# zsyOAOA/ResShift

Measured on NVIDIA B200. Metric: 256x256 x4 SR images/sec (15 steps), denoising hot path, higher is better.
Workload: dtype f16 (fp32 accumulate)

## Files before the change

### include/resshift_b200.h

```cpp
#ifndef RESSHIFT_B200_H
#define RESSHIFT_B200_H

#include <stddef.h>
#include <stdint.h>

#ifdef __cplusplus
extern "C" {
#endif

#define RS_MAX_LEVELS 8

typedef struct rs_unet_config {
  int32_t image_size;
  int32_t in_channels;
  int32_t model_channels;
  int32_t out_channels;
  int32_t n_levels;
  int32_t channel_mult[RS_MAX_LEVELS];
  int32_t num_res_blocks[RS_MAX_LEVELS];
  int32_t n_attn;
  int32_t attention_resolutions[RS_MAX_LEVELS];
  int32_t swin_depth;
  int32_t swin_embed_dim;
  int32_t swin_heads;
  int32_t window_size;
  float mlp_ratio;
  int32_t cond_mask;
  int32_t lq_size;
} rs_unet_config;

typedef struct rs_vq_config {
  int32_t embed_dim;
  int32_t n_embed;
  int32_t z_channels;
  int32_t in_channels;
  int32_t out_ch;
  int32_t ch;
  int32_t n_levels;
  int32_t ch_mult[RS_MAX_LEVELS];
  int32_t num_res_blocks[RS_MAX_LEVELS];
} rs_vq_config;

typedef struct rs_engine rs_engine;
typedef struct rs_plan rs_plan;
typedef struct rs_sampler rs_sampler;

int rs_version(void);
const char* rs_last_error(void);

int rs_unet_create(const rs_unet_config* cfg, rs_engine** out);
void rs_unet_destroy(rs_engine* e);
int rs_unet_param_count(const rs_engine* e);
int rs_unet_param_info(const rs_engine* e, int index, char* name, size_t name_cap, int32_t shape[4],
                       int32_t* ndim, int32_t* is_buffer);
size_t rs_unet_arena_bytes(const rs_engine* e);
int rs_unet_set_arena(rs_engine* e, void* arena_dev);
int rs_unet_load_param(rs_engine* e, const char* name, const float* src_dev, void* stream);

int rs_plan_create(rs_engine* e, int batch, int height, int width, rs_plan** out);
void rs_plan_destroy(rs_plan* p);
size_t rs_plan_workspace_bytes(const rs_plan* p);
int rs_plan_bind(rs_plan* p, void* workspace_dev);
int rs_plan_num_launches(const rs_plan* p);
int rs_plan_forward(rs_plan* p, const float* x, const float* timesteps, const float* lq, const float* mask,
                    float* out, void* stream);
int rs_plan_profile(rs_plan* p, const float* x, const float* timesteps, const float* lq, const float* mask,
                    double* ms_by_kind, double* conv_flops, int32_t* n_conv_launches, void* stream);
int rs_plan_profile_ops(rs_plan* p, const float* x, const float* timesteps, const float* lq, const float* mask,
                        double* ms, char* desc, int desc_stride, int cap, int32_t* n_ops, void* stream);
int rs_plan_probe(rs_plan* p, const char* block, float* dst, int32_t* channels, int32_t* h, int32_t* w,
                  void* stream);

int rs_sampler_create(rs_plan* p, int steps, const double* sqrt_etas_host, double kappa,
                      const int32_t* timestep_map_host, rs_sampler** out);
void rs_sampler_destroy(rs_sampler* s);
int rs_sampler_run(rs_sampler* s, const float* z_y, const float* noises, const float* lq, const float* mask,
                   float* out_latent, int use_graph, void* stream);
int rs_sampler_run_host(rs_sampler* s, const float* z_y_host, const float* noises_host, const float* lq_host,
                        const float* mask_host, float* out_latent_host, void* staging_dev, size_t staging_bytes,
                        int use_graph, void* stream);
size_t rs_sampler_staging_bytes(const rs_sampler* s);
int rs_sampler_set_taps(rs_sampler* s, float* pred_xstart_steps, float* sample_steps);

int rs_vq_create(const rs_vq_config* cfg, rs_engine** out);
int rs_vq_plan_create(rs_engine* e, int batch, int image_h, int image_w, int which, rs_plan** out);
int rs_vq_encode(rs_plan* p, const float* x, float* h_out, void* stream);
int rs_vq_decode(rs_plan* p, const float* h, float* out, int32_t* idx_out, int force_not_quantize, void* stream);
int rs_vq_profile_ops(rs_plan* p, double* ms, char* desc, int desc_stride, int cap, int32_t* n_ops, void* stream);

int rs_op_bicubic_upsample(const float* x, int N, int C, int H, int W, int sf, float* y, void* stream);
int rs_op_ingest_u8(const void* src_u8_nhwc, int N, int H, int W, int C, float* dst_nchw, void* stream);
int rs_op_emit_u8(const float* sr_nchw, const float* lq_nchw_or_null, const float* mask_or_null, int N, int H, int W,
                  int bgr, void* dst_u8_nhwc, void* stream);
int rs_op_tile_gather(const float* tiles, int N, int C, int H, int W, int th, int tw, int nty, int ntx, const int32_t* ys,
                      const int32_t* xs, float* out, void* stream);

int rs_p_sample(const float* x_t, const float* x0_pred, const float* noise, float* x_next, float coef1,
                float coef2, float std, int t_is_zero, long long numel, void* stream);

int rs_op_pack_conv_weight(const float* src_oihw, void* dst_f16, int O, int I, int KH, int KW, int Ipad, void* stream);
int rs_op_conv2d(const void* x, int N, int H, int W, int C, int ld, const void* w_packed, int Ipad, const float* bias,
                 int Cout, int ksize, int stride, const void* residual, int res_ld, void* out, int out_ld,
                 float* out_f32_nchw, int act, int bn, void* stream);
int rs_op_conv2d_stats(const void* x, int N, int H, int W, int C, int ld, const void* w_packed, int Ipad, const float* bias,
                       int Cout, int ksize, int stride, const void* residual, int res_ld, void* out, int out_ld, int act,
                       int bn, float* part, int cstride, int coff, int32_t* slots_out, float* gstat, void* counter,
                       int expected_channels, void* stream);
int rs_op_conv2d_splitk(const void* x, int N, int H, int W, int C, int ld, const void* w_packed, int Ipad, const float* bias,
                        int Cout, int ksize, int stride, const void* residual, int res_ld, void* out, int out_ld, int act,
                        float* part, int cstride, int coff, float* scratch, int32_t* splits_out, float* gstat, void* counter,
                        void* stream);
int rs_op_conv2d_timeline(const void* x, int N, int H, int W, int C, int ld, const void* w_packed, int Ipad, const float* bias,
                          int Cout, int ksize, int stride, void* out, int out_ld, int bn, int iters, void* dbg,
                          int32_t* info, float* splitk_scratch_or_null, void* stream);
int rs_op_groupnorm(const void* x, int N, int H, int W, int C, int ld, const float* gamma, const float* beta,
                    const float* film, long long film_sN, int silu, void* y, int y_ld, float* sums_scratch,
                    void* stream);
long long rs_op_groupnorm_scratch_floats(int N, int H, int W, int C);
int rs_op_groupnorm_apply(const void* x, int N, int H, int W, int C, int ld, const float* gamma, const float* beta,
                          const float* film, long long film_sN, int silu, void* y, int y_ld, const float* gstat,
                          void* stream);
int rs_op_groupnorm_apply_pairs(const void* x, int N, int H, int W, int C, int ld, const float* gamma, const float* beta,
                                const float* film, long long film_sN, int silu, void* y, int y_ld, const float* part,
                                int slots, void* stream);
int rs_op_groupnorm_finalize(const float* part, int N, int slots, int C, int rows_per_slot, float eps, float* gstat, void* stream);
int rs_op_expand_relpos(const float* table_225xh, float* dense_hx64x64, int heads, void* stream);
int rs_op_window_attention(const void* qkv, int N, int H, int W, int heads, int shift, const float* bias_dense,
                           void* out, void* stream);
int rs_op_swin_attn(const void* x, int N, int H, int W, int E, int heads, int shift, const float* gn_part, int gn_slots,
                    const float* gamma, const float* beta, const void* wqkv_packed, const float* bqkv, const float* relbias_dense,
                    const void* wproj_packed, const float* bproj, void* y, float* part_out, float* gstat_out_or_null,
                    uint32_t* counters_or_null, void* stream);
int rs_op_mlp(const void* x, int N, int H, int W, int E, int Hd, const void* w1_packed, const float* b1,
              const void* w2_packed, const float* b2, const void* residual, void* out, void* dbg_timeline_or_null,
              void* stream);
int rs_debug_tile_config(int m_tiles, int cout, int num_kblocks, int32_t* out);
int rs_debug_swin_timeline(void* dev_buf_or_null);
int rs_op_upsample2x(const void* x, int N, int H, int W, int C, void* y, void* stream);

#ifdef __cplusplus
}
#endif
#endif
```

### resshift_b200/_lib.py

```python
from __future__ import annotations

import ctypes as C
import os
from pathlib import Path

_HERE = Path(__file__).resolve().parent
LIB_PATH = Path(os.environ.get("RESSHIFT_B200_LIB", _HERE / "lib" / "librs_b200.so"))

RS_MAX_LEVELS = 8


class RsError(RuntimeError):
    pass


class UNetConfigC(C.Structure):
    _fields_ = [
        ("image_size", C.c_int32), ("in_channels", C.c_int32), ("model_channels", C.c_int32),
        ("out_channels", C.c_int32), ("n_levels", C.c_int32),
        ("channel_mult", C.c_int32 * RS_MAX_LEVELS), ("num_res_blocks", C.c_int32 * RS_MAX_LEVELS),
        ("n_attn", C.c_int32), ("attention_resolutions", C.c_int32 * RS_MAX_LEVELS),
        ("swin_depth", C.c_int32), ("swin_embed_dim", C.c_int32), ("swin_heads", C.c_int32),
        ("window_size", C.c_int32), ("mlp_ratio", C.c_float), ("cond_mask", C.c_int32), ("lq_size", C.c_int32),
    ]


class VQConfigC(C.Structure):
    _fields_ = [
        ("embed_dim", C.c_int32), ("n_embed", C.c_int32), ("z_channels", C.c_int32), ("in_channels", C.c_int32),
        ("out_ch", C.c_int32), ("ch", C.c_int32), ("n_levels", C.c_int32),
        ("ch_mult", C.c_int32 * RS_MAX_LEVELS), ("num_res_blocks", C.c_int32 * RS_MAX_LEVELS),
    ]


_P = C.c_void_p
_SIGNATURES = {
    "rs_version": (C.c_int, []),
    "rs_last_error": (C.c_char_p, []),
    "rs_unet_create": (C.c_int, [C.POINTER(UNetConfigC), C.POINTER(_P)]),
    "rs_unet_destroy": (None, [_P]),
    "rs_unet_param_count": (C.c_int, [_P]),
    "rs_unet_param_info": (C.c_int, [_P, C.c_int, C.c_char_p, C.c_size_t, C.POINTER(C.c_int32), C.POINTER(C.c_int32),
                                     C.POINTER(C.c_int32)]),
    "rs_unet_arena_bytes": (C.c_size_t, [_P]),
    "rs_unet_set_arena": (C.c_int, [_P, _P]),
    "rs_unet_load_param": (C.c_int, [_P, C.c_char_p, _P, _P]),
    "rs_plan_create": (C.c_int, [_P, C.c_int, C.c_int, C.c_int, C.POINTER(_P)]),
    "rs_plan_destroy": (None, [_P]),
    "rs_plan_workspace_bytes": (C.c_size_t, [_P]),
    "rs_plan_bind": (C.c_int, [_P, _P]),
    "rs_plan_num_launches": (C.c_int, [_P]),
    "rs_plan_forward": (C.c_int, [_P, _P, _P, _P, _P, _P, _P]),
    "rs_plan_profile": (C.c_int, [_P, _P, _P, _P, _P, C.POINTER(C.c_double), C.POINTER(C.c_double), C.POINTER(C.c_int32), _P]),
    "rs_plan_profile_ops": (C.c_int, [_P, _P, _P, _P, _P, C.POINTER(C.c_double), C.c_char_p, C.c_int, C.c_int, C.POINTER(C.c_int32), _P]),
    "rs_plan_probe": (C.c_int, [_P, C.c_char_p, _P, C.POINTER(C.c_int32), C.POINTER(C.c_int32), C.POINTER(C.c_int32), _P]),
    "rs_sampler_create": (C.c_int, [_P, C.c_int, C.POINTER(C.c_double), C.c_double, C.POINTER(C.c_int32), C.POINTER(_P)]),
    "rs_sampler_destroy": (None, [_P]),
    "rs_sampler_run": (C.c_int, [_P, _P, _P, _P, _P, _P, C.c_int, _P]),
    "rs_sampler_run_host": (C.c_int, [_P, _P, _P, _P, _P, _P, _P, C.c_size_t, C.c_int, _P]),
    "rs_sampler_staging_bytes": (C.c_size_t, [_P]),
    "rs_sampler_set_taps": (C.c_int, [_P, _P, _P]),
    "rs_p_sample": (C.c_int, [_P, _P, _P, _P, C.c_float, C.c_float, C.c_float, C.c_int, C.c_longlong, _P]),
    "rs_op_pack_conv_weight": (C.c_int, [_P, _P, C.c_int, C.c_int, C.c_int, C.c_int, C.c_int, _P]),
    "rs_op_conv2d": (C.c_int, [_P, C.c_int, C.c_int, C.c_int, C.c_int, C.c_int, _P, C.c_int, _P, C.c_int, C.c_int,
                               C.c_int, _P, C.c_int, _P, C.c_int, _P, C.c_int, C.c_int, _P]),
    "rs_op_conv2d_stats": (C.c_int, [_P, C.c_int, C.c_int, C.c_int, C.c_int, C.c_int, _P, C.c_int, _P, C.c_int, C.c_int,
                                     C.c_int, _P, C.c_int, _P, C.c_int, C.c_int, C.c_int, _P, C.c_int, C.c_int,
                                     C.POINTER(C.c_int32), _P, _P, C.c_int, _P]),
    "rs_op_conv2d_splitk": (C.c_int, [_P, C.c_int, C.c_int, C.c_int, C.c_int, C.c_int, _P, C.c_int, _P, C.c_int, C.c_int,
                                      C.c_int, _P, C.c_int, _P, C.c_int, C.c_int, _P, C.c_int, C.c_int, _P,
                                      C.POINTER(C.c_int32), _P, _P, _P]),
    "rs_op_conv2d_timeline": (C.c_int, [_P, C.c_int, C.c_int, C.c_int, C.c_int, C.c_int, _P, C.c_int, _P, C.c_int, C.c_int,
                                        C.c_int, _P, C.c_int, C.c_int, C.c_int, _P, C.POINTER(C.c_int32), _P, _P]),
    "rs_op_groupnorm": (C.c_int, [_P, C.c_int, C.c_int, C.c_int, C.c_int, C.c_int, _P, _P, _P, C.c_longlong, C.c_int,
                                  _P, C.c_int, _P, _P]),
    "rs_op_groupnorm_scratch_floats": (C.c_longlong, [C.c_int, C.c_int, C.c_int, C.c_int]),
    "rs_op_groupnorm_apply": (C.c_int, [_P, C.c_int, C.c_int, C.c_int, C.c_int, C.c_int, _P, _P, _P, C.c_longlong, C.c_int,
                                        _P, C.c_int, _P, _P]),
    "rs_op_groupnorm_finalize": (C.c_int, [_P, C.c_int, C.c_int, C.c_int, C.c_int, C.c_float, _P, _P]),
    "rs_op_groupnorm_apply_pairs": (C.c_int, [_P, C.c_int, C.c_int, C.c_int, C.c_int, C.c_int, _P, _P, _P, C.c_longlong,
                                              C.c_int, _P, C.c_int, _P, C.c_int, _P]),
    "rs_op_expand_relpos": (C.c_int, [_P, _P, C.c_int, _P]),
    "rs_op_window_attention": (C.c_int, [_P, C.c_int, C.c_int, C.c_int, C.c_int, C.c_int, _P, _P, _P]),
    "rs_op_swin_attn": (C.c_int, [_P, C.c_int, C.c_int, C.c_int, C.c_int, C.c_int, C.c_int, _P, C.c_int, _P, _P, _P, _P, _P, _P, _P,
                                  _P, _P, _P, _P, _P]),
    "rs_op_mlp": (C.c_int, [_P, C.c_int, C.c_int, C.c_int, C.c_int, C.c_int, _P, _P, _P, _P, _P, _P, _P, _P]),
    "rs_debug_tile_config": (C.c_int, [C.c_int, C.c_int, C.c_int, C.POINTER(C.c_int32)]),
    "rs_debug_swin_timeline": (C.c_int, [_P]),
    "rs_op_upsample2x": (C.c_int, [_P, C.c_int, C.c_int, C.c_int, C.c_int, _P, _P]),
    "rs_vq_create": (C.c_int, [C.POINTER(VQConfigC), C.POINTER(_P)]),
    "rs_vq_plan_create": (C.c_int, [_P, C.c_int, C.c_int, C.c_int, C.c_int, C.POINTER(_P)]),
    "rs_vq_encode": (C.c_int, [_P, _P, _P, _P]),
    "rs_vq_decode": (C.c_int, [_P, _P, _P, _P, C.c_int, _P]),
    "rs_vq_profile_ops": (C.c_int, [_P, C.POINTER(C.c_double), C.c_char_p, C.c_int, C.c_int, C.POINTER(C.c_int32), _P]),
    "rs_op_bicubic_upsample": (C.c_int, [_P, C.c_int, C.c_int, C.c_int, C.c_int, C.c_int, _P, _P]),
    "rs_op_ingest_u8": (C.c_int, [_P, C.c_int, C.c_int, C.c_int, C.c_int, _P, _P]),
    "rs_op_emit_u8": (C.c_int, [_P, _P, _P, C.c_int, C.c_int, C.c_int, C.c_int, _P, _P]),
    "rs_op_tile_gather": (C.c_int, [_P, C.c_int, C.c_int, C.c_int, C.c_int, C.c_int, C.c_int, C.c_int, C.c_int, _P, _P, _P, _P]),
}


def _load():
    if not LIB_PATH.exists():
        raise ImportError(
            f"resshift_b200: CUDA library {LIB_PATH} not found. Build it with "
            f"`python -c 'import __graft_entry__ as g; g.build()'` (nvcc, sm_100a). There is no CPU fallback.")
    lib = C.CDLL(str(LIB_PATH))
    for name, (res, args) in _SIGNATURES.items():
        fn = getattr(lib, name)
        fn.restype = res
        fn.argtypes = args
    return lib


lib = _load()


def check(rc: int) -> None:
    if rc != 0:
        msg = lib.rs_last_error()
        raise RsError(f"librs_b200 error {rc}: {msg.decode(errors='replace') if msg else '?'}")


def declared_symbols():
    return sorted(_SIGNATURES)


def ptr(t) -> int:
    return None if t is None else t.data_ptr()


def current_stream() -> int:
    import torch
    return torch.cuda.current_stream().cuda_stream


def make_config(cfg) -> UNetConfigC:
    c = UNetConfigC()
    c.image_size, c.in_channels, c.model_channels, c.out_channels = cfg.image_size, cfg.in_channels, cfg.model_channels, cfg.out_channels
    c.n_levels = len(cfg.channel_mult)
    for i, v in enumerate(cfg.channel_mult):
        c.channel_mult[i] = int(v)
    for i, v in enumerate(cfg.num_res_blocks):
        c.num_res_blocks[i] = int(v)
    c.n_attn = len(cfg.attention_resolutions)
    for i, v in enumerate(cfg.attention_resolutions):
        c.attention_resolutions[i] = int(v)
    c.swin_depth, c.swin_embed_dim, c.swin_heads = cfg.swin_depth, cfg.swin_embed_dim, cfg.swin_heads
    c.window_size, c.mlp_ratio = cfg.window_size, float(cfg.mlp_ratio)
    c.cond_mask, c.lq_size = int(cfg.cond_mask), cfg.lq_size
    return c


def make_vq_config(cfg) -> VQConfigC:
    c = VQConfigC()
    c.embed_dim, c.n_embed, c.z_channels = cfg.embed_dim, cfg.n_embed, cfg.z_channels
    c.in_channels, c.out_ch, c.ch = cfg.in_channels, cfg.out_ch, cfg.ch
    c.n_levels = len(cfg.ch_mult)
    for i, v in enumerate(cfg.ch_mult):
        c.ch_mult[i] = int(v)
    for i, v in enumerate(cfg.num_res_blocks):
        c.num_res_blocks[i] = int(v)
    return c
```

### resshift_b200/csrc/conv_gemm.cuh

```cuda
#pragma once

#include "common.cuh"
#include "gn_stats.cuh"

namespace rs {

constexpr int kConvBM = 128;
constexpr int kConvBK = 64;
constexpr int kConvEpiWarps = 8;
constexpr int kConvThreads = 64 + 32 * kConvEpiWarps;
constexpr int kConvTmaWarp = kConvEpiWarps;
constexpr int kConvMmaWarp = kConvEpiWarps + 1;
constexpr int kMaxTaps = 9;
constexpr int kMaxSrc = 4;

enum ConvAct : int { ACT_NONE = 0, ACT_GELU = 1, ACT_SILU = 2 };

struct ConvParams {
  CUtensorMap tmA[kMaxSrc];
  CUtensorMap tmB;
  int num_taps;
  int tap_src[kMaxTaps];
  int tap_dh[kMaxTaps];
  int tap_dw[kMaxTaps];
  int kchunks;
  int tail_k16;
  int w_tap_stride;
  int bw, bh, bn;
  int tiles_w, tiles_h, tiles_n;
  int Wout, Hout, Nimg;
  int BN, n_tiles, Cout;
  int stages;
  int tmem_cols;
  int cg;
  int splitk;
  float* partial;
  int splitk_cluster;
  int msub;
  const float* bias;
  const __half* residual;
  long long res_sN, res_sH, res_sW;
  __half* out;
  long long out_sN, out_sH, out_sW;
  float* out_f32_nchw;
  int act;
  unsigned long long* dbg;
  CUtensorMap tmOut, tmRes;
  int tma_out;
  int tma_res;
  int epi_bc;
  GnSink sink[2];
  int gn_slots;
  int persist;
  int num_units;
};

#ifdef __CUDACC__

template <int kCG>
__global__ void __launch_bounds__(kConvThreads, 2) conv_gemm_sm100_kernel(const __grid_constant__ ConvParams p) {
  extern __shared__ __align__(1024) uint8_t smem_raw[];
  uint8_t* smem = reinterpret_cast<uint8_t*>((reinterpret_cast<uintptr_t>(smem_raw) + 1023) & ~uintptr_t(1023));
  const int a_bytes = kConvBM * kConvBK * 2;
  const int b_rows = kCG == 2 ? p.BN / 2 : p.BN;
  const int b_bytes = b_rows * kConvBK * 2;
  const int stage_bytes = p.msub * a_bytes + b_bytes;
  uint64_t* full_bar = reinterpret_cast<uint64_t*>(smem + (size_t)p.stages * stage_bytes);
  uint64_t* empty_bar = full_bar + p.stages;
  uint64_t* tmem_full_bar = empty_bar + p.stages;
  uint64_t* res_bar = tmem_full_bar + 1;
  uint32_t* tmem_slot = reinterpret_cast<uint32_t*>(res_bar + 1);
  float* s_bias = reinterpret_cast<float*>(smem + (size_t)p.stages * stage_bytes + 256);

  const int warp = threadIdx.x >> 5;
  const int lane = threadIdx.x & 31;
  unsigned long long* dbg = p.dbg ? p.dbg + (size_t)blockIdx.x * 8 : nullptr;
  if (dbg && threadIdx.x == 0) {
    uint32_t smid;
    asm volatile("mov.u32 %0, %%smid;" : "=r"(smid));
    dbg[0] = global_timer_ns(); dbg[7] = smid;
  }

  const uint32_t crank = kCG == 2 ? cluster_ctarank() : 0;
  const uint32_t rank = crank & 1;
  const uint32_t lead = crank & ~1u;
  const uint16_t pair_mask = (uint16_t)(3u << lead);
  int unit = kCG == 2 ? (blockIdx.x >> 1) : blockIdx.x;
  const int split = unit % p.splitk;
  unit /= p.splitk;
  const int n_tile = unit % p.n_tiles;
  const int mt0 = kCG == 2 ? (unit / p.n_tiles) * 2 + (int)rank : (unit / p.n_tiles) * p.msub;
  const int total_kb = p.num_taps * p.kchunks;
  const int kb_begin = (int)((long long)total_kb * split / p.splitk);
  const int kb_end = (int)((long long)total_kb * (split + 1) / p.splitk);
  const int num_kb = kb_end - kb_begin;
  auto tile_origin = [&](int sub, int& tw_, int& th_, int& w0_, int& h0_, int& n0_) {
    int mt = mt0 + sub;
    tw_ = mt % p.tiles_w; mt /= p.tiles_w;
    th_ = mt % p.tiles_h; mt /= p.tiles_h;
    w0_ = tw_ * p.bw; h0_ = th_ * p.bh; n0_ = mt * p.bn;
  };

  if (warp == kConvTmaWarp && lane == 0) {
    for (int s = 0; s < kMaxSrc; ++s) tma_prefetch_desc(&p.tmA[s]);
    tma_prefetch_desc(&p.tmB);
    if (p.tma_out) tma_prefetch_desc(&p.tmOut);
    if (p.tma_res) tma_prefetch_desc(&p.tmRes);
    for (int s = 0; s < p.stages; ++s) {
      mbar_init(&full_bar[s], 1);
      mbar_init(&empty_bar[s], 1);
    }
    mbar_init(tmem_full_bar, 1);
    mbar_init(res_bar, 1);
    mbar_fence_init();
  }
  if (warp == kConvMmaWarp) {
    if constexpr (kCG == 2) { tmem_alloc_dyn_cg2(tmem_slot, (uint32_t)p.tmem_cols); tmem_relinquish_cg2(); }
    else { tmem_alloc_dyn(tmem_slot, (uint32_t)p.tmem_cols); tmem_relinquish(); }
  }
  tc_fence_before();
  if constexpr (kCG == 2) cluster_sync_all(); else __syncthreads();
  tc_fence_after();
  const uint32_t tmem_base = *tmem_slot;
  pdl_trigger();
  pdl_wait();
  if (dbg && threadIdx.x == 0) dbg[1] = global_timer_ns();

  if (warp == kConvTmaWarp) {
    const bool el = elect_one();
    int stage = 0;
    uint32_t phase = 0;
    int tws[2], ths[2], w0s[2], h0s[2], n0s[2];
    for (int sub = 0; sub < p.msub; ++sub) tile_origin(sub, tws[sub], ths[sub], w0s[sub], h0s[sub], n0s[sub]);
    int tap = kb_begin / p.kchunks;
    int kc = kb_begin - tap * p.kchunks;
    const uint32_t tx_bytes = (uint32_t)(kCG == 2 ? 2 * stage_bytes : stage_bytes);
    for (int kb = 0; kb < num_kb; ++kb) {
      mbar_wait(&empty_bar[stage], phase ^ 1);
      uint8_t* sa = smem + (size_t)stage * stage_bytes;
      uint8_t* sb = sa + p.msub * a_bytes;
      const CUtensorMap* ma = &p.tmA[p.tap_src[tap]];
      const int dw = p.tap_dw[tap], dh = p.tap_dh[tap];
      const int kcol = kc * kConvBK, wcol = tap * p.w_tap_stride + kc * kConvBK;
      if constexpr (kCG == 2) {
        const uint32_t lead_bar = mapa_u32(smem_u32(&full_bar[stage]), lead);
        if (el) {
          if (rank == 0) mbar_arrive_expect_tx(&full_bar[stage], tx_bytes);
          tma_load_4d_cg2(sa, ma, lead_bar, kcol, w0s[0] + dw, h0s[0] + dh, n0s[0]);
          tma_load_2d_cg2(sb, &p.tmB, lead_bar, wcol, n_tile * p.BN + (int)rank * b_rows);
        }
      } else {
        if (el) {
          mbar_arrive_expect_tx(&full_bar[stage], tx_bytes);
          for (int sub = 0; sub < p.msub; ++sub)
            tma_load_4d(sa + sub * a_bytes, ma, &full_bar[stage], kcol, w0s[sub] + dw, h0s[sub] + dh, n0s[sub]);
          tma_load_2d(sb, &p.tmB, &full_bar[stage], wcol, n_tile * p.BN);
        }
      }
      if (++kc == p.kchunks) { kc = 0; ++tap; }
      if (++stage == p.stages) { stage = 0; phase ^= 1; }
    }
  } else if (warp == kConvMmaWarp && rank == 0) {
    const bool el = elect_one();
    const uint32_t idesc = umma_idesc_f16(kCG == 2 ? 2 * kConvBM : kConvBM, p.BN);
    const uint32_t smem0 = smem_u32(smem);
    const uint32_t b_off = (uint32_t)(p.msub * a_bytes);
    int stage = 0;
    uint32_t phase = 0;
    int kc = kb_begin % p.kchunks;
    for (int kb = 0; kb < num_kb; ++kb) {
      mbar_wait(&full_bar[stage], phase);
      tc_fence_after();
      if (dbg && el && kb == 0) dbg[2] = global_timer_ns();
      const uint32_t sa = smem0 + (uint32_t)stage * (uint32_t)stage_bytes;
      const uint64_t adesc = umma_desc_sw128(sa);
      const uint64_t bdesc = umma_desc_sw128(sa + b_off);
      const uint32_t acc0 = kb != 0 ? 1u : 0u;
      const int ksteps = (kc == p.kchunks - 1) ? p.tail_k16 : kConvBK / 16;
      if (++kc == p.kchunks) kc = 0;
      if constexpr (kCG == 2) {
        if (el) {
          umma_f16_cg2(tmem_base, adesc, bdesc, idesc, acc0);
#pragma unroll
          for (int k = 1; k < kConvBK / 16; ++k) if (k < ksteps) umma_f16_cg2(tmem_base, adesc + 2 * k, bdesc + 2 * k, idesc, 1u);
          umma_commit_cg2(&empty_bar[stage], pair_mask);
          if (kb == num_kb - 1) umma_commit_cg2(tmem_full_bar, pair_mask);
        }
      } else {
        if (el) {
          umma_f16(tmem_base, adesc, bdesc, idesc, acc0);
#pragma unroll
          for (int k = 1; k < kConvBK / 16; ++k) if (k < ksteps) umma_f16(tmem_base, adesc + 2 * k, bdesc + 2 * k, idesc, 1u);
          if (p.msub == 2) {
            const uint64_t adesc1 = umma_desc_sw128(sa + a_bytes);
            umma_f16(tmem_base + p.BN, adesc1, bdesc, idesc, acc0);
#pragma unroll
            for (int k = 1; k < kConvBK / 16; ++k) if (k < ksteps) umma_f16(tmem_base + p.BN, adesc1 + 2 * k, bdesc + 2 * k, idesc, 1u);
          }
          umma_commit(&empty_bar[stage]);
          if (kb == num_kb - 1) umma_commit(tmem_full_bar);
        }
      }
      if (++stage == p.stages) { stage = 0; phase ^= 1; }
    }
    if (dbg && el) dbg[3] = global_timer_ns();
// ... 64 lines not shown
          for (int sub = 0; sub < p.msub; ++sub) {
            int tw, th, w0, h0, n0;
            tile_origin(sub, tw, th, w0, h0, n0);
            for (int b = 0; b < nblk; ++b)
              tma_load_4d(smem + (size_t)sub * sub_bytes + (size_t)b * blk_bytes, &p.tmRes, res_bar, col0 + b * bc, w0, h0, n0);
          }
        }
        mbar_wait(res_bar, 0);
      }
      const bool want_stats = p.sink[0].part != nullptr;
      for (int sub = 0; sub < p.msub; ++sub) {
        int tw, th, w0, h0, n0;
        tile_origin(sub, tw, th, w0, h0, n0);
        const uint32_t trow = tmem_base + (static_cast<uint32_t>(quad * 32) << 16) + sub * p.BN;
        uint8_t* sblk = smem + (size_t)sub * sub_bytes;
        uint32_t vn[16];
        if (cpar * 16 < p.BN) tmem_ld16(trow + cpar * 16, vn);
        for (int c = cpar * 16; c < p.BN; c += 32) {
          tmem_ld_wait16(vn);
          float f[16];
#pragma unroll
          for (int j = 0; j < 16; ++j) f[j] = __uint_as_float(vn[j]);
          if (c + 32 < p.BN) tmem_ld16(trow + c + 32, vn);
          {
            const float4* bp = reinterpret_cast<const float4*>(s_bias + c);
#pragma unroll
            for (int j = 0; j < 4; ++j) {
              const float4 b4 = bp[j];
              f[4 * j] += b4.x; f[4 * j + 1] += b4.y; f[4 * j + 2] += b4.z; f[4 * j + 3] += b4.w;
            }
          }
          if (p.act == ACT_GELU) {
#pragma unroll
            for (int j = 0; j < 16; ++j) f[j] = gelu_erf_f(f[j]);
          } else if (p.act == ACT_SILU) {
#pragma unroll
            for (int j = 0; j < 16; ++j) f[j] = silu_f(f[j]);
          }
          uint8_t* brow = sblk + (size_t)(c >> bshift) * blk_bytes + r * (2 * bc);
          const int u0 = (c & (bc - 1)) >> 3;
          uint4* a0 = reinterpret_cast<uint4*>(brow + (((u0) ^ swz) << 4));
          uint4* a1 = reinterpret_cast<uint4*>(brow + (((u0 + 1) ^ swz) << 4));
          if (p.tma_res) {
            const uint4 r0 = *a0, r1 = *a1;
            const __half2* h0p = reinterpret_cast<const __half2*>(&r0);
            const __half2* h1p = reinterpret_cast<const __half2*>(&r1);
#pragma unroll
            for (int j = 0; j < 4; ++j) {
              const float2 x0 = __half22float2(h0p[j]);
              const float2 x1 = __half22float2(h1p[j]);
              f[2 * j] += x0.x; f[2 * j + 1] += x0.y;
              f[8 + 2 * j] += x1.x; f[8 + 2 * j + 1] += x1.y;
            }
          }
          uint4 o0, o1;
          __half2* q0 = reinterpret_cast<__half2*>(&o0);
          __half2* q1 = reinterpret_cast<__half2*>(&o1);
#pragma unroll
          for (int j = 0; j < 4; ++j) {
            q0[j] = __floats2half2_rn(f[2 * j], f[2 * j + 1]);
            q1[j] = __floats2half2_rn(f[8 + 2 * j], f[8 + 2 * j + 1]);
          }
          *a0 = o0; *a1 = o1;
          if (want_stats) warp_chunk_stats(o0, o1, lane, wsum_all + ((size_t)(sub * 4 + quad) * p.BN + c) * 2);
        }
      }
      fence_proxy_async_smem();
      named_bar_sync(1, 32 * kConvEpiWarps);
      if (dbg && etid == 0) dbg[6] = global_timer_ns();
      if (etid == 0) {
        for (int sub = 0; sub < p.msub; ++sub) {
          int tw, th, w0, h0, n0;
          tile_origin(sub, tw, th, w0, h0, n0);
          for (int b = 0; b < nblk; ++b)
            if (col0 + b * bc < p.Cout)
              tma_store_4d(&p.tmOut, smem + (size_t)sub * sub_bytes + (size_t)b * blk_bytes, col0 + b * bc, w0, h0, n0);
        }
        tma_store_commit();
      }
      if (want_stats) {
        int* s_flag = reinterpret_cast<int*>(wsum_all + (size_t)p.msub * 8 * p.BN);
        for (int sub = 0; sub < p.msub; ++sub) {
          int tw, th, w0, h0, n0;
          tile_origin(sub, tw, th, w0, h0, n0);
          const int ncols = min(p.BN, p.Cout - col0);
          const int slot = th * p.tiles_w + tw;
          if (n0 < p.Nimg)
            write_quad_pairs(wsum_all + (size_t)sub * 8 * p.BN, p.BN, ncols, col0, p.bn, n0, p.Nimg, slot, p.gn_slots, p.sink[0], p.sink[1],
                             etid, 32 * kConvEpiWarps);
          if (p.sink[0].gstat || p.sink[1].gstat) {
            const GnSink* const sk[4] = {&p.sink[0], &p.sink[0], p.sink[1].part ? &p.sink[1] : nullptr, p.sink[1].part ? &p.sink[1] : nullptr};
            const int n1 = (p.bn == 2 && n0 + 1 < p.Nimg) ? n0 + 1 : -1;
            const int im[4] = {n0 < p.Nimg ? n0 : -1, n0 < p.Nimg ? n1 : -1, n0 < p.Nimg ? n0 : -1, n0 < p.Nimg ? n1 : -1};
            const unsigned int ad[4] = {(unsigned)ncols, (unsigned)ncols, (unsigned)ncols, (unsigned)ncols};
            gn_arrive<4>(sk, im, ad, p.gn_slots, 128.0f / (float)p.bn, etid, 32 * kConvEpiWarps, 1, s_flag);
          }
        }
      }
      if (etid == 0) tma_store_wait_read();
    } else {
      for (int sub = 0; sub < p.msub; ++sub) {
        int tw, th, w0, h0, n0;
        tile_origin(sub, tw, th, w0, h0, n0);
        const int w = w0 + lw, h = h0 + lh, n = n0 + ln;
        const bool row_ok = (w < p.Wout) && (h < p.Hout) && (n < p.Nimg);
        const uint32_t trow = tmem_base + (static_cast<uint32_t>(quad * 32) << 16) + sub * p.BN;
        __half* orow = p.out ? p.out + n * p.out_sN + h * p.out_sH + w * p.out_sW : nullptr;
        const __half* rrow = p.residual ? p.residual + n * p.res_sN + h * p.res_sH + w * p.res_sW : nullptr;
        for (int c = cpar * 16; c < p.BN; c += 32) {
          uint32_t v[16];
          __syncwarp();
          tmem_ld16(trow + c, v);
          tmem_ld_wait();
          const int col = col0 + c;
          if (!row_ok || col >= p.Cout) continue;
          float f[16];
#pragma unroll
          for (int j = 0; j < 16; ++j) f[j] = __uint_as_float(v[j]);
          if (p.bias) {
#pragma unroll
            for (int j = 0; j < 16; ++j)
              if (col + j < p.Cout) f[j] += __ldg(p.bias + col + j);
          }
          if (p.act == ACT_GELU) {
#pragma unroll
            for (int j = 0; j < 16; ++j) f[j] = gelu_erf_f(f[j]);
          } else if (p.act == ACT_SILU) {
#pragma unroll
            for (int j = 0; j < 16; ++j) f[j] = silu_f(f[j]);
          }
          if (rrow)
            for (int j = 0; j < 16 && col + j < p.Cout; ++j) f[j] += __half2float(rrow[col + j]);
          if (p.out_f32_nchw)
            for (int j = 0; j < 16 && col + j < p.Cout; ++j)
              p.out_f32_nchw[(((long long)n * p.Cout + (col + j)) * p.Hout + h) * p.Wout + w] = f[j];
          if (orow)
            for (int j = 0; j < 16 && col + j < p.Cout; ++j) orow[col + j] = __float2half_rn(f[j]);
        }
      }
    }
  }

  if constexpr (kCG == 2) {
    if (p.splitk > 1 && p.splitk_cluster) {
      cluster_sync_all();
      if (warp < kConvEpiWarps) {
        const int etid = threadIdx.x;
        const int S = p.splitk, cw = p.BN / S, upr = cw >> 3;
        const int pitch = p.BN * 4 + 16;
        const int cbase = split * cw;
        const int col0 = n_tile * p.BN;
        __half* s_out = reinterpret_cast<__half*>(smem + (size_t)kConvBM * pitch);
        float* s_col = reinterpret_cast<float*>(s_out + (size_t)kConvBM * cw);
        int tw, th, w0, h0, n0;
        tile_origin(0, tw, th, w0, h0, n0);
        const uint32_t dump0 = smem_u32(smem);
        for (int u = etid; u < kConvBM * upr; u += 32 * kConvEpiWarps) {
          const int rr = u / upr, cu = u - rr * upr;
          const int ct = cbase + cu * 8;
          float acc[8];
#pragma unroll
          for (int j = 0; j < 8; ++j) acc[j] = 0.f;
          for (int sp = 0; sp < S; ++sp) {
            const uint32_t a = mapa_u32(dump0 + (uint32_t)(rr * pitch + ct * 4), (uint32_t)(sp * 2) + rank);
            const float4 x0 = ld_shared_cluster_f4(a), x1 = ld_shared_cluster_f4(a + 16);
            acc[0] += x0.x; acc[1] += x0.y; acc[2] += x0.z; acc[3] += x0.w;
            acc[4] += x1.x; acc[5] += x1.y; acc[6] += x1.z; acc[7] += x1.w;
          }
          const int lw = rr % p.bw, lh = (rr / p.bw) % p.bh, ln = rr / (p.bw * p.bh);
          const int w = w0 + lw, h = h0 + lh, n = n0 + ln;
          const int col = col0 + ct;
          const bool ok = (w < p.Wout) && (h < p.Hout) && (n < p.Nimg) && (col < p.Cout);
          uint4 o = make_uint4(0, 0, 0, 0);
          if (ok) {
            if (p.bias) {
#pragma unroll
              for (int j = 0; j < 8; ++j) acc[j] += __ldg(p.bias + col + j);
            }
            if (p.act == ACT_GELU) {
#pragma unroll
              for (int j = 0; j < 8; ++j) acc[j] = gelu_erf_f(acc[j]);
            } else if (p.act == ACT_SILU) {
#pragma unroll
              for (int j = 0; j < 8; ++j) acc[j] = silu_f(acc[j]);
            }
            if (p.residual) {
              const uint4 rv = *reinterpret_cast<const uint4*>(p.residual + n * p.res_sN + h * p.res_sH + w * p.res_sW + col);
              const __half2* rh = reinterpret_cast<const __half2*>(&rv);
#pragma unroll
              for (int j = 0; j < 4; ++j) { const float2 f = __half22float2(rh[j]); acc[2 * j] += f.x; acc[2 * j + 1] += f.y; }
            }
            __half2* oh = reinterpret_cast<__half2*>(&o);
#pragma unroll
            for (int j = 0; j < 4; ++j) oh[j] = __floats2half2_rn(acc[2 * j], acc[2 * j + 1]);
            *reinterpret_cast<uint4*>(p.out + n * p.out_sN + h * p.out_sH + w * p.out_sW + col) = o;
          }
          *reinterpret_cast<uint4*>(s_out + (size_t)rr * cw + cu * 8) = o;
        }
        if (p.sink[0].part != nullptr) {
          named_bar_sync(1, 32 * kConvEpiWarps);
          for (int t = etid; t < 2 * cw; t += 32 * kConvEpiWarps) {
            const int half = t / cw, c = t - half * cw;
            const __half* col = s_out + (size_t)(half * 64) * cw + c;
            const float pv = __half2float(col[0]);
            float s1 = 0.f, s2 = 0.f;
            for (int rr = 1; rr < 64; ++rr) {
              const float d = __half2float(col[(size_t)rr * cw]) - pv;
              s1 += d; s2 = fmaf(d, d, s2);
            }
            s_col[(half * cw + c) * 2] = pv + s1 * (1.0f / 64.0f);
            s_col[(half * cw + c) * 2 + 1] = fmaxf(s2 - s1 * s1 * (1.0f / 64.0f), 0.f);
          }
          named_bar_sync(1, 32 * kConvEpiWarps);
          const int slot = th * p.tiles_w + tw;
          const int ncols = max(0, min(cw, p.Cout - (col0 + cbase)));
          if (n0 < p.Nimg)
            write_tile_pairs(s_col, cw, ncols, col0 + cbase, p.bn, n0, p.Nimg, slot, p.gn_slots, p.sink[0], p.sink[1], etid, 32 * kConvEpiWarps);
          if (p.sink[0].gstat || p.sink[1].gstat) {
            int* s_flag = reinterpret_cast<int*>(s_col + 4 * cw);
            const GnSink* const sk[4] = {&p.sink[0], &p.sink[0], p.sink[1].part ? &p.sink[1] : nullptr, p.sink[1].part ? &p.sink[1] : nullptr};
            const int n1 = (p.bn == 2 && n0 + 1 < p.Nimg) ? n0 + 1 : -1;
            const int im[4] = {n0 < p.Nimg ? n0 : -1, n0 < p.Nimg ? n1 : -1, n0 < p.Nimg ? n0 : -1, n0 < p.Nimg ? n1 : -1};
            const unsigned int ad[4] = {(unsigned)ncols, (unsigned)ncols, (unsigned)ncols, (unsigned)ncols};
            gn_arrive<4>(sk, im, ad, p.gn_slots, 128.0f / (float)p.bn, etid, 32 * kConvEpiWarps, 1, s_flag);
          }
        }
      }
    }
  }

  tc_fence_before();
  if constexpr (kCG == 2) cluster_sync_all(); else __syncthreads();
  if (dbg && threadIdx.x == 0) dbg[5] = global_timer_ns();
  if (warp == kConvMmaWarp) {
    tc_fence_after();
    if constexpr (kCG == 2) tmem_dealloc_dyn_cg2(tmem_base, (uint32_t)p.tmem_cols);
    else tmem_dealloc_dyn(tmem_base, (uint32_t)p.tmem_cols);
  }
}

struct ConvSimtSrc {
  const __half* ptr[kMaxSrc];
  long long sN[kMaxSrc], sH[kMaxSrc], sW[kMaxSrc];
  int H[kMaxSrc], W[kMaxSrc];
  int C;
  const __half* wt;
};

__global__ void conv_simt_kernel(const __grid_constant__ ConvParams p, const __grid_constant__ ConvSimtSrc s) {
  pdl_trigger();
  pdl_wait();
  const long long pix = (long long)blockIdx.x * (blockDim.x >> 5) + (threadIdx.x >> 5);
  const int lane = threadIdx.x & 31;
  const long long npix = (long long)p.Nimg * p.Hout * p.Wout;
  if (pix >= npix) return;
  const int w = (int)(pix % p.Wout);
  const int h = (int)((pix / p.Wout) % p.Hout);
  const int n = (int)(pix / ((long long)p.Wout * p.Hout));
  const int ktot = p.num_taps * p.w_tap_stride;
  for (int co = lane; co < p.Cout; co += 32) {
    float acc = 0.f;
    for (int t = 0; t < p.num_taps; ++t) {
      const int src = p.tap_src[t];
      const int hh = h + p.tap_dh[t], ww = w + p.tap_dw[t];
      if (hh < 0 || ww < 0 || hh >= s.H[src] || ww >= s.W[src]) continue;
      const __half* a = s.ptr[src] + n * s.sN[src] + hh * s.sH[src] + ww * s.sW[src];
      const __half* wr = s.wt + (long long)co * ktot + t * p.w_tap_stride;
      for (int c = 0; c < s.C; c += 2) {
        const float2 av = __half22float2(*reinterpret_cast<const __half2*>(a + c));
        const float2 wv = __half22float2(*reinterpret_cast<const __half2*>(wr + c));
        acc = fmaf(av.x, wv.x, acc);
        acc = fmaf(av.y, wv.y, acc);
      }
    }
    if (p.bias) acc += p.bias[co];
    if (p.act == ACT_GELU) acc = gelu_erf_f(acc);
    else if (p.act == ACT_SILU) acc = silu_f(acc);
    if (p.residual) acc += __half2float(p.residual[n * p.res_sN + h * p.res_sH + w * p.res_sW + co]);
    if (p.out_f32_nchw) p.out_f32_nchw[(((long long)n * p.Cout + co) * p.Hout + h) * p.Wout + w] = acc;
    if (p.out) p.out[n * p.out_sN + h * p.out_sH + w * p.out_sW + co] = __float2half_rn(acc);
  }
}

#endif

}
```

### resshift_b200/csrc/engine.cu

```cuda
#include <map>
#include <memory>
#include <string>
#include <vector>

#include "../../include/resshift_b200.h"
#include "launch.cuh"
#include "vq_kernels.cuh"

namespace rs {

static thread_local std::string g_last_error;
void set_error(const std::string& msg) { g_last_error = msg; }
int fail(int code, const std::string& msg) { g_last_error = msg; return code; }

static inline size_t align_up(size_t v, size_t a) { return (v + a - 1) / a * a; }

enum Role { R_CONV3 = 0, R_CONV1, R_LINEAR, R_BIAS, R_GN_W, R_GN_B, R_RELPOS, R_BUF_RELIDX, R_BUF_MASK, R_F32  };

struct Param {
  std::string name;
  std::vector<int> shape;
  int role;
  size_t off = 0;
  size_t bytes = 0;
// ... 113 lines not shown
      add_conv(e, p, L.a, L.b, 3);
    } else if (L.kind == 1) {
      add_gn(e, p + ".in_layers.0", L.a);
      add_conv(e, p + ".in_layers.2", L.a, L.b, 3);
      add_linear(e, p + ".emb_layers.1", e.time_dim(), 2 * L.b);
      add_gn(e, p + ".out_layers.0", L.b);
      add_conv(e, p + ".out_layers.3", L.b, L.b, 3);
      if (L.a != L.b) add_conv(e, p + ".skip_connection", L.a, L.b, 1);
    } else if (L.kind == 2) {
      const int E = c.swin_embed_dim, res = L.b;
      const int win = res <= c.window_size ? res : c.window_size;
      const int shift = res <= c.window_size ? 0 : c.window_size / 2;
      const int hidden = (int)(E * c.mlp_ratio);
      add_conv(e, p + ".patch_embed.proj", L.a, E, 1);
      add_conv(e, p + ".patch_unembed.proj", E, L.a, 1);
      for (int i = 0; i < c.swin_depth; ++i) {
        const std::string b = p + ".blocks." + std::to_string(i);
        if (i % 2 == 1 && shift > 0) {
          const int nw = (res / win) * (res / win);
          add_param(e, b + ".attn_mask", {nw, win * win, win * win}, R_BUF_MASK);
        }
        add_gn(e, b + ".norm1", E);
        add_param(e, b + ".attn.relative_position_bias_table", {(2 * win - 1) * (2 * win - 1), c.swin_heads}, R_RELPOS);
        add_param(e, b + ".attn.relative_position_index", {win * win, win * win}, R_BUF_RELIDX);
        add_linear(e, b + ".attn.qkv", E, 3 * E);
        add_linear(e, b + ".attn.proj", E, E);
        add_gn(e, b + ".norm2", E);
        add_conv(e, b + ".mlp.fc1", E, hidden, 1);
        add_conv(e, b + ".mlp.fc2", hidden, E, 1);
      }
    } else if (L.kind == 3) {
      add_conv(e, p + ".op", L.a, L.a, 3);
    } else if (L.kind == 4) {
      add_conv(e, p + ".conv", L.a, L.a, 3);
    }
  }
}

int build_inventory(rs_engine& e) {
  const rs_unet_config& c = e.cfg;
  add_linear(e, "time_embed.0", c.model_channels, e.time_dim());
  add_linear(e, "time_embed.2", e.time_dim(), e.time_dim());
  int fc = e.lq_in_ch(), bc = 16;
  for (int st = 0; st < e.fe_stages(); ++st) {
    add_conv(e, "feature_extractor." + std::to_string(3 * st), fc, bc, 3);
    add_conv(e, "feature_extractor." + std::to_string(3 * st + 2) + ".op", bc, 2 * bc, 3);
    bc *= 2; fc = bc;
  }
  Topology t = build_topology(e);
  for (size_t i = 0; i < t.input_blocks.size(); ++i) add_layers(e, "input_blocks." + std::to_string(i), t.input_blocks[i]);
  add_layers(e, "middle_block", t.middle);
  for (size_t i = 0; i < t.output_blocks.size(); ++i) add_layers(e, "output_blocks." + std::to_string(i), t.output_blocks[i]);
  add_gn(e, "out.0", c.channel_mult[0] * c.model_channels);
  add_conv(e, "out.2", c.channel_mult[0] * c.model_channels, c.out_channels, 3);

  size_t off = 0;
  const int K = e.time_dim();
  e.film_w_off = off;
  int rows = 0;
  for (Param& p : e.params) {
    if (p.role == R_LINEAR && p.name.find(".emb_layers.1.weight") != std::string::npos) {
      p.ipad = K; p.off = off; p.bytes = (size_t)p.shape[0] * K * 2;
      e.film_row_of[p.name.substr(0, p.name.size() - std::string(".emb_layers.1.weight").size())] = rows;
      rows += p.shape[0];
      off += p.bytes;
    }
  }
  e.film_rows = rows;
  off = align_up(off, 256);
  e.film_b_off = off;
  for (Param& p : e.params) {
    if (p.role == R_BIAS && p.name.find(".emb_layers.1.bias") != std::string::npos) {
      p.off = off; p.bytes = (size_t)p.shape[0] * 4; off += p.bytes;
    }
  }
  off = align_up(off, 256);
  for (Param& p : e.params) {
    if (p.bytes) continue;
    switch (p.role) {
      case R_CONV3: case R_CONV1:
        p.ipad = (p.shape[1] + 7) / 8 * 8;
        p.bytes = (size_t)p.shape[0] * p.shape[2] * p.shape[3] * p.ipad * 2; break;
      case R_LINEAR:
        p.ipad = (p.shape[1] + 7) / 8 * 8;
        p.bytes = (size_t)p.shape[0] * p.ipad * 2; break;
      case R_BIAS: case R_GN_W: case R_GN_B:
        p.bytes = (size_t)p.shape[0] * 4; break;
      case R_RELPOS:
        p.bytes = (size_t)c.swin_heads * 64 * 64 * 4; break;
      default: p.bytes = 0; break;
    }
    if (p.bytes) { p.off = off; off = align_up(off + p.bytes, 256); }
  }
  e.arena_bytes = align_up(off, 256);
  return 0;
}

}

namespace {

enum OpKind { OP_CONV, OP_GN, OP_ATTN, OP_UPSAMPLE, OP_MLP, OP_SOFTMAX, OP_FORK, OP_JOIN, OP_SWIN_ATTN };

struct Tensor {
  size_t bytes = 0;
  int first = 1 << 30, last = -1;
  size_t off = 0;
  bool persistent = false;
};

struct Op {
  OpKind kind;
  ConvDesc conv;
  GnDesc gn;
  View a_in, a_out; const float* a_bias = nullptr; int a_shift = 0;
  View u_in, u_out;
  View s_view; float s_scale = 1.f;
  View w_view; bool w_is_view = false;
  std::string in_param;
  MlpDesc mlp;
  SwinAttnDesc swin;
  std::string blk_name;
  std::string w2_name, b2_name;
  std::string w_name, b_name, g_name;
  size_t stats_off = 0;
  int gn_index = -1;
  bool to_f32 = false;
  int split_tens = -1;
  int stream = 0;
  struct StatDst { int list; int op; int coff; int img_off; };
  std::vector<StatDst> stat_dst;
};

}

struct rs_plan {
  rs_engine* e = nullptr;
  int B = 0, H = 0, W = 0, lqH = 0, lqW = 0;
  std::vector<Tensor> tensors;
  std::vector<Op> fe_ops, ops;
  std::map<std::string, View> block_out;
  size_t off_emb_sin = 0, off_emb_mid = 0, off_emb_vec = 0, off_film = 0, off_tsteps = 0, off_tables = 0;
  size_t off_stats = 0, stats_bytes = 0, off_state = 0, off_temps = 0, temps_bytes = 0;
  size_t off_gstat = 0, off_counters = 0;
  int n_gn = 0;
  size_t workspace_bytes = 0;
  int max_rows = 0;
  uint8_t* ws = nullptr;
  View xin, lq_feat, fe_in;
  int cin_pad = 0, fe_cpad = 0;
  float* out_f32 = nullptr;
  bool bound = false;
  int launches = 0;
  int branches = 1;
  std::vector<cudaStream_t> side;
  std::vector<cudaEvent_t> ev;
  std::vector<std::pair<int, int>> sections;
  ~rs_plan() {
    for (cudaStream_t s : side) cudaStreamDestroy(s);
    for (cudaEvent_t e : ev) cudaEventDestroy(e);
  }
  int vq_which = -1;
  int imgH = 0, imgW = 0;
  const void* table_owner = nullptr;
  unsigned long long table_epoch = ~0ull;

  int new_tensor(size_t bytes, bool persistent = false) {
    Tensor t; t.bytes = align_up(bytes, 256); t.persistent = persistent;
    tensors.push_back(t);
    return (int)tensors.size() - 1;
  }
  View make_view(int N, int Hh, int Ww, int C, bool persistent = false) {
    View v; v.N = N; v.H = Hh; v.W = Ww; v.C = C; v.ld = C; v.off = 0;
    v.tens = new_tensor((size_t)N * Hh * Ww * C * 2, persistent);
    return v;
  }
  static View slice(const View& base, int c0, int C) {
    View v = base; v.off = base.off + c0; v.c0 = base.c0 + c0; v.C = C; return v;
  }
  static View batch(const View& base, int n0, int n) {
    View v = base; v.off = base.off + (long long)n0 * base.sN(); v.n0 = base.n0 + n0; v.N = n; return v;
  }
  void touch(const View& v, int opi) {
    if (v.tens < 0) return;
    Tensor& t = tensors[v.tens];
    t.first = std::min(t.first, opi); t.last = std::max(t.last, opi);
  }
};

namespace {

struct Builder {
  rs_plan& P;
  rs_engine& E;
  std::vector<Op>* cur;
  size_t stats_off = 0;
  int n_gn = 0;
  struct Writer { int c0; int C; int n0; int N; int list; int op; int win_slots; };
  std::map<int, std::vector<Writer>> writers;
  int cur_stream = 0;
  int cur_batch0 = 0;
  static bool overlaps(const Writer& w, const View& v, int C) {
    return w.c0 < v.c0 + C && v.c0 < w.c0 + w.C && w.n0 < v.n0 + v.N && v.n0 < w.n0 + w.N;
  }
  static bool inside(const Writer& w, const View& v) {
    return w.c0 >= v.c0 && w.c0 + w.C <= v.c0 + v.C && w.n0 >= v.n0 && w.n0 + w.N <= v.n0 + v.N;
  }
  void note_writer(const View& out, int C, int win_slots = 0) {
    auto& ws = writers[out.tens];
    ws.erase(std::remove_if(ws.begin(), ws.end(), [&](const Writer& w) { return overlaps(w, out, C); }), ws.end());
    ws.push_back({out.c0, C, out.n0, out.N, list_id(), (int)cur->size() - 1, win_slots});
  }
  std::vector<Writer> covering_writers(const View& in) {
    bool fusable = false;
    conv_tile_slots(in.H, in.W, &fusable);
    std::vector<Writer> prod;
    if (fuse_stats && fusable) {
      long long covered = 0;
      auto it = writers.find(in.tens);
      if (it != writers.end())
        for (const Writer& w : it->second)
          if (inside(w, in)) { prod.push_back(w); covered += (long long)w.C * w.N; }
      bool ok = covered == (long long)in.C * in.N;
      for (const Writer& w : prod) ok = ok && list(w.list)[w.op].stat_dst.size() < 2 && w.win_slots == prod[0].win_slots;
      if (!ok) prod.clear();
    }
    return prod;
  }
  const bool fuse_mlp = env_int("RS_MLP_FUSE", 1) && !env_is("RS_CONV_IMPL", "simt");
  const bool fuse_mlp_norm = env_int("RS_MLP_NORM_FUSE", 0) != 0;
  const bool fuse_swin_attn = env_int("RS_SWIN_FUSE", 1) != 0 && !env_is("RS_CONV_IMPL", "simt") && !env_is("RS_ATTN_IMPL", "simt");
  const int fuse_swin_min_pairs = env_int("RS_SWIN_FUSE_MIN_PAIRS", 96);
  const bool fuse_stats = env_int("RS_GN_FUSE", 1) && !env_is("RS_CONV_EPI", "direct") && !env_is("RS_CONV_IMPL", "simt");
  Builder(rs_plan& p) : P(p), E(*p.e), cur(&p.ops) {}
  int list_id() const { return cur == &P.fe_ops ? 0 : 1; }
  std::vector<Op>& list(int id) { return id == 0 ? P.fe_ops : P.ops; }

  int opi() const { return (int)(P.fe_ops.size() + P.ops.size()); }

  void conv(const View& in, const std::string& name, int ksize, int stride, int cout, const View* out,
            const View* res, int act, bool out_f32 = false, int pad_lo = 1) {
    Op op; op.kind = OP_CONV;
    op.conv.in = in; op.conv.ksize = ksize; op.conv.stride = stride; op.conv.Cout = cout; op.conv.act = act;
    op.conv.pad_lo = pad_lo;
    if (out) { op.conv.out = *out; op.conv.has_out = true; } else op.conv.has_out = false;
    if (res) { op.conv.res = *res; op.conv.has_res = true; }
    op.w_name = name + ".weight"; op.b_name = name + ".bias";
    op.to_f32 = out_f32;
    if (out && !out_f32 && env_int("RS_CONV_SPLITK", 0) != 1) {
      const TileConfig tc = conv_preview_config(in.N, in.H, in.W, in.C, cout, ksize, stride, true);
      if (tc.splitk > 1) op.conv.allow_split = true;
      if (tc.splitk > 1 && !tc.cluster_split) {
        const size_t bytes = (size_t)tc.splitk * in.N * (in.H / stride) * (in.W / stride) * cout * sizeof(float);
        op.split_tens = P.new_tensor(bytes);
        Tensor& tz = P.tensors[op.split_tens];
        tz.first = tz.last = opi();
      }
    }
    const int i = opi();
    P.touch(in, i); if (out) P.touch(*out, i); if (res) P.touch(*res, i);
    op.stream = cur_stream;
    cur->push_back(op);
    if (out && !out_f32 && out->tens >= 0) note_writer(*out, cout);
  }
  void gn(const View& in, const std::string& name, const View& out, int silu, int film_off, float eps = 1e-5f) {
    Op op; op.kind = OP_GN;
    op.gn.in = in; op.gn.out = out; op.gn.silu = silu; op.gn.film_off = film_off; op.gn.eps = eps;
    op.gn.film_n0 = cur_batch0;
    op.g_name = name;
    std::vector<Writer> prod = covering_writers(in);
    op.gn.win_slots = !prod.empty() && prod[0].win_slots;
    const int tile_slots = op.gn.win_slots ? (in.H / 8) * (in.W / 8) : conv_tile_slots(in.H, in.W);
    int chunks, rows;
    gn_chunks(in.H * in.W, in.N, &chunks, &rows);
    op.gn.fused = !prod.empty();
    op.gn.slots = op.gn.fused ? tile_slots : chunks;
    op.stats_off = stats_off;
    op.gn_index = n_gn++;
    stats_off += align_up((size_t)in.N * op.gn.slots * in.C * 2 * sizeof(float), 256);
    const int i = opi();
    P.touch(in, i); P.touch(out, i);
    op.stream = cur_stream;
    cur->push_back(op);
    for (const Writer& w : prod)
      list(w.list)[w.op].stat_dst.push_back({list_id(), (int)cur->size() - 1, w.c0 - in.c0, w.n0 - in.n0});
  }
  void attn(const View& qkv, const View& out, const std::string& blk, int shift) {
    Op op; op.kind = OP_ATTN; op.a_in = qkv; op.a_out = out; op.a_shift = shift;
    op.w_name = blk + ".attn.relative_position_bias_table";
    const int i = opi();
    P.touch(qkv, i); P.touch(out, i);
    op.stream = cur_stream;
    cur->push_back(op);
  }
  bool mlp(const View& in, const std::string& name, int E, int Hd, const View& out, const View& res,
           const std::string& norm_name = std::string()) {
    Op op; op.kind = OP_MLP;
    op.mlp.in = in; op.mlp.out = out; op.mlp.res = res; op.mlp.has_res = true; op.mlp.E = E; op.mlp.Hd = Hd;
    op.w_name = name + ".fc1.weight"; op.b_name = name + ".fc1.bias";
    op.w2_name = name + ".fc2.weight"; op.b2_name = name + ".fc2.bias";
    std::vector<Writer> prod;
    if (!norm_name.empty()) {
      prod = covering_writers(in);
      if (prod.empty() || Hd < 4 * E) return false;
      op.g_name = norm_name;
      op.gn.win_slots = prod[0].win_slots;
      op.gn.in = in; op.gn.fused = true; op.gn.slots = op.gn.win_slots ? (in.H / 8) * (in.W / 8) : conv_tile_slots(in.H, in.W);
      op.stats_off = stats_off;
      op.gn_index = n_gn++;
      stats_off += align_up((size_t)in.N * op.gn.slots * in.C * 2 * sizeof(float), 256);
    }
    const int i = opi();
    P.touch(in, i); P.touch(out, i); P.touch(res, i);
    op.stream = cur_stream;
    cur->push_back(op);
    for (const Writer& w : prod)
      list(w.list)[w.op].stat_dst.push_back({list_id(), (int)cur->size() - 1, w.c0 - in.c0, w.n0 - in.n0});
    if (out.tens >= 0) note_writer(out, E);
    return true;
  }
  bool swin_attn(const View& x, const std::string& blk, int heads, int shift) {
    std::vector<Writer> prod = covering_writers(x);
    if (prod.empty()) return false;
    Op op; op.kind = OP_SWIN_ATTN;
    op.swin.x = x; op.swin.y = x; op.swin.heads = heads; op.swin.shift = shift;
    op.blk_name = blk;
    op.g_name = blk + ".norm1";
    op.gn.win_slots = prod[0].win_slots;
    op.gn.in = x; op.gn.fused = true; op.gn.slots = op.gn.win_slots ? (x.H / 8) * (x.W / 8) : conv_tile_slots(x.H, x.W);
    op.stats_off = stats_off;
    op.gn_index = n_gn++;
    stats_off += align_up((size_t)x.N * op.gn.slots * x.C * 2 * sizeof(float), 256);
    const int i = opi();
    P.touch(x, i);
    op.stream = cur_stream;
    cur->push_back(op);
    for (const Writer& w : prod)
      list(w.list)[w.op].stat_dst.push_back({list_id(), (int)cur->size() - 1, w.c0 - x.c0, w.n0 - x.n0});
    if (x.tens >= 0) note_writer(x, x.C, 1);
    return true;
  }
  void upsample(const View& in, const View& out) {
    Op op; op.kind = OP_UPSAMPLE; op.u_in = in; op.u_out = out;
    const int i = opi();
    P.touch(in, i); P.touch(out, i);
    op.stream = cur_stream;
    cur->push_back(op);
  }
  void marker(OpKind k) { Op op; op.kind = k; cur->push_back(op); }

  void res_block(const View& x, const std::string& p, int cout, const View& out) {
    View t1 = P.make_view(x.N, x.H, x.W, x.C);
    gn(x, p + ".in_layers.0", t1, 1, -1);
    View h1 = P.make_view(x.N, x.H, x.W, cout);
    conv(t1, p + ".in_layers.2", 3, 1, cout, &h1, nullptr, ACT_NONE);
    View t2 = P.make_view(x.N, x.H, x.W, cout);
    gn(h1, p + ".out_layers.0", t2, 1, E.film_row_of.at(p));
    if (x.C != cout) {
      conv(x, p + ".skip_connection", 1, 1, cout, &out, nullptr, ACT_NONE);
      conv(t2, p + ".out_layers.3", 3, 1, cout, &out, &out, ACT_NONE);
    } else {
      conv(t2, p + ".out_layers.3", 3, 1, cout, &out, &x, ACT_NONE);
    }
  }
  int basic_layer(const View& x, const std::string& p, int ctor_res, const View& out) {
    const rs_unet_config& c = E.cfg;
    const int Ed = c.swin_embed_dim, hidden = (int)(Ed * c.mlp_ratio);
    const int win = ctor_res <= c.window_size ? ctor_res : c.window_size;
    RS_CHECK(win == 8 && x.H % 8 == 0 && x.W % 8 == 0, "the window-attention kernel covers 8x8 windows only");
    const int shift_odd = ctor_res <= c.window_size ? 0 : c.window_size / 2;
    View e = P.make_view(x.N, x.H, x.W, Ed);
    conv(x, p + ".patch_embed.proj", 1, 1, Ed, &e, nullptr, ACT_NONE);
    for (int i = 0; i < c.swin_depth; ++i) {
      const std::string b = p + ".blocks." + std::to_string(i);
      const int win_pairs = (x.N * (x.H / 8) * (x.W / 8) + 1) / 2;
      if (!(fuse_swin_attn && win_pairs >= fuse_swin_min_pairs && swin_attn_supported(Ed, c.swin_heads, x.H, x.W) &&
            swin_attn(e, b, c.swin_heads, (i % 2) ? shift_odd : 0))) {
        View n1 = P.make_view(x.N, x.H, x.W, Ed);
        gn(e, b + ".norm1", n1, 0, -1);
        View qkv = P.make_view(x.N, x.H, x.W, 3 * Ed);
        conv(n1, b + ".attn.qkv", 1, 1, 3 * Ed, &qkv, nullptr, ACT_NONE);
        View a = P.make_view(x.N, x.H, x.W, Ed);
        attn(qkv, a, b, (i % 2) ? shift_odd : 0);
        conv(a, b + ".attn.proj", 1, 1, Ed, &e, &e, ACT_NONE);
      }
      const bool mlp_ok = fuse_mlp && mlp_supported(Ed, hidden, x.H, x.W, x.N);
      if (mlp_ok && fuse_mlp_norm && mlp(e, b + ".mlp", Ed, hidden, e, e, b + ".norm2")) continue;
      View n2 = P.make_view(x.N, x.H, x.W, Ed);
      gn(e, b + ".norm2", n2, 0, -1);
      if (mlp_ok) {
        mlp(n2, b + ".mlp", Ed, hidden, e, e);
      } else {
        View f = P.make_view(x.N, x.H, x.W, hidden);
        conv(n2, b + ".mlp.fc1", 1, 1, hidden, &f, nullptr, ACT_GELU);
        conv(f, b + ".mlp.fc2", 1, 1, Ed, &e, &e, ACT_NONE);
      }
    }
    conv(e, p + ".patch_unembed.proj", 1, 1, x.C, &out, nullptr, ACT_NONE);
    return 0;
  }

  int run_block(View h, const std::string& prefix, const std::vector<Layer>& layers, const View& dest, View* result) {
    for (size_t j = 0; j < layers.size(); ++j) {
      const Layer& L = layers[j];
      const std::string p = prefix + "." + std::to_string(j);
      const bool last = (j + 1 == layers.size());
      View out;
      if (L.kind == 0) {
        out = last ? dest : P.make_view(h.N, h.H, h.W, L.b);
        conv(h, p, 3, 1, L.b, &out, nullptr, ACT_NONE);
      } else if (L.kind == 1) {
        out = last ? dest : P.make_view(h.N, h.H, h.W, L.b);
        res_block(h, p, L.b, out);
      } else if (L.kind == 2) {
        out = last ? dest : P.make_view(h.N, h.H, h.W, h.C);
        int rc = basic_layer(h, p, L.b, out); if (rc) return rc;
      } else if (L.kind == 3) {
        out = dest;
        conv(h, p + ".op", 3, 2, L.a, &out, nullptr, ACT_NONE);
      } else {
        View u = P.make_view(h.N, 2 * h.H, 2 * h.W, h.C);
        upsample(h, u);
        out = dest;
        conv(u, p + ".conv", 3, 1, L.a, &out, nullptr, ACT_NONE);
      }
      h = out;
    }
    *result = h;
    return 0;
  }
};

int finish_layout(rs_plan& P, Builder& b, size_t state_bytes, bool unet) {
  rs_engine& E = *P.e;
  const rs_unet_config& c = E.cfg;
  const int B = P.B;
  P.max_rows = std::max(B, 64);
  size_t off = 0;
  auto region = [&](size_t bytes) { size_t o = off; off = align_up(off + bytes, 256); return o; };
  if (unet) {
    P.off_tables = region(4 * 1024 * sizeof(float));
    P.off_tsteps = region((size_t)P.max_rows * sizeof(float));
    P.off_emb_sin = region((size_t)P.max_rows * c.model_channels * sizeof(float));
    P.off_emb_mid = region((size_t)P.max_rows * E.time_dim() * sizeof(float));
    P.off_emb_vec = region((size_t)P.max_rows * E.time_dim() * sizeof(float));
    P.off_film = region((size_t)P.max_rows * E.film_rows * sizeof(float));
  }
  P.stats_bytes = b.stats_off;
  P.off_stats = region(P.stats_bytes);
  P.n_gn = b.n_gn;
  P.off_gstat = region((size_t)P.n_gn * B * 32 * 2 * sizeof(float));
  P.off_counters = region((size_t)P.n_gn * B * sizeof(unsigned int));
  const size_t lat = state_bytes;
  P.off_state = region(2 * align_up(lat, 256));
  for (const auto& sec : P.sections)
    for (Tensor& tz : P.tensors) {
      if (tz.last < 0) continue;
      if (tz.first >= sec.first && tz.first <= sec.second) tz.first = sec.first;
      if (tz.last >= sec.first && tz.last <= sec.second) tz.last = sec.second;
    }
  if (env_int("RS_NO_REUSE", 0)) for (Tensor& tz : P.tensors) tz.persistent = true;
  for (Tensor& tz : P.tensors) if (tz.persistent) tz.off = region(tz.bytes);
  P.off_temps = off;
  {
    struct Live { size_t off, bytes; int last; };
    std::vector<Live> live;
    std::vector<int> order;
    for (int i = 0; i < (int)P.tensors.size(); ++i) if (!P.tensors[i].persistent && P.tensors[i].last >= 0) order.push_back(i);
    std::stable_sort(order.begin(), order.end(), [&](int a, int bb) { return P.tensors[a].first < P.tensors[bb].first; });
    size_t high = 0;
    for (int id : order) {
      Tensor& tz = P.tensors[id];
      live.erase(std::remove_if(live.begin(), live.end(), [&](const Live& l) { return l.last < tz.first; }), live.end());
      std::sort(live.begin(), live.end(), [](const Live& a, const Live& bb) { return a.off < bb.off; });
      size_t pos = 0;
      for (const Live& l : live) {
        if (pos + tz.bytes <= l.off) break;
        pos = std::max(pos, l.off + l.bytes);
      }
      tz.off = P.off_temps + pos;
      live.push_back({pos, tz.bytes, tz.last});
      high = std::max(high, pos + tz.bytes);
    }
    P.temps_bytes = high;
  }
  P.workspace_bytes = align_up(P.off_temps + P.temps_bytes, 256);
  return 0;
}

int build_plan(rs_plan& P) {
  rs_engine& E = *P.e;
  const rs_unet_config& c = E.cfg;
  Topology topo = build_topology(E);
  Builder b(P);
  const int B = P.B;

  const int fes = E.fe_stages();
  P.lqH = P.H << fes; P.lqW = P.W << fes;
  if (fes > 0) {
    b.cur = &P.fe_ops;
    P.fe_cpad = 8;
    P.fe_in = P.make_view(B, P.lqH, P.lqW, P.fe_cpad, true);
    View cur = P.fe_in;
    int bc = 16;
    for (int st = 0; st < fes; ++st) {
      View a = P.make_view(B, cur.H, cur.W, bc, true);
      b.conv(cur, "feature_extractor." + std::to_string(3 * st), 3, 1, bc, &a, nullptr, ACT_SILU);
      View d = P.make_view(B, cur.H / 2, cur.W / 2, 2 * bc, true);
      b.conv(a, "feature_extractor." + std::to_string(3 * st + 2) + ".op", 3, 2, 2 * bc, &d, nullptr, ACT_NONE);
      cur = d; bc *= 2;
// ... 3 lines not shown
  }

  const int cin = c.in_channels + E.lq_feat_ch();
  P.cin_pad = (cin + 7) / 8 * 8;
  P.xin = P.make_view(B, P.H, P.W, P.cin_pad, true);

  const int n_in = (int)topo.input_blocks.size();
  const int n_out = (int)topo.output_blocks.size();
  RS_CHECK(n_in == n_out, "encoder/decoder block counts differ");
  std::vector<int> in_h(n_in), in_w(n_in);
  {
    int hh = P.H, ww = P.W;
    for (int i = 0; i < n_in; ++i) {
      for (const Layer& L : topo.input_blocks[i]) if (L.kind == 3) { hh /= 2; ww /= 2; }
      in_h[i] = hh; in_w[i] = ww;
    }
  }
  std::vector<View> cat(n_out);
  for (int j = 0; j < n_out; ++j) {
    const int k = n_in - 1 - j;
    const int ctot = topo.output_blocks[j][0].a;
    cat[j] = P.make_view(B, in_h[k], in_w[k], ctot);
  }
  {
    int nb = env_int("RS_LOWRES_STREAMS", 1);
    if (nb < 1) nb = 1;
    while (nb > 1 && (B % nb != 0 || B / nb < 1)) --nb;
    P.branches = nb;
  }
  const long long low_tiles = env_int("RS_LOWRES_TILES", 64);
  auto is_low = [&](int hh, int ww) { return (long long)B * hh * ww / 128 <= low_tiles; };
  bool in_sec = false;
  int sec_first = 0;
  auto leave = [&]() {
    if (!in_sec) return;
    const int last = b.opi() - 1;
    b.marker(OP_JOIN);
    P.sections.push_back({sec_first, last});
    in_sec = false;
  };
  auto run = [&](const View& hin, const std::string& prefix, const std::vector<Layer>& layers, const View& dest, View* hout) -> int {
    bool low = P.branches > 1 && is_low(hin.H, hin.W);
    if (P.branches > 1 && !low && layers.size() == 1 && layers[0].kind == 3) low = is_low(hin.H / 2, hin.W / 2);
    if (!low) {
      leave();
      return b.run_block(hin, prefix, layers, dest, hout);
    }
    if (!in_sec) { b.marker(OP_FORK); sec_first = b.opi(); in_sec = true; }
    const int per = B / P.branches;
    for (int k = 0; k < P.branches; ++k) {
      View tmp;
      b.cur_stream = k; b.cur_batch0 = k * per;
      int rc = b.run_block(rs_plan::batch(hin, k * per, per), prefix, layers, rs_plan::batch(dest, k * per, per), &tmp);
      b.cur_stream = 0; b.cur_batch0 = 0;
      if (rc) return rc;
    }
    *hout = dest;
    return 0;
  };
  View h = P.xin;
  for (int i = 0; i < n_in; ++i) {
    const int j = n_in - 1 - i;
    const int ich = topo.in_block_ch[i];
    View dest = rs_plan::slice(cat[j], cat[j].C - ich, ich);
    View hin = h;
    int rc = run(hin, "input_blocks." + std::to_string(i), topo.input_blocks[i], dest, &h);
    if (rc) return rc;
    P.block_out["input_blocks." + std::to_string(i)] = h;
  }
  {
    View dest = rs_plan::slice(cat[0], 0, cat[0].C - topo.in_block_ch[n_in - 1]);
    int rc = run(h, "middle_block", topo.middle, dest, &h); if (rc) return rc;
    P.block_out["middle_block"] = h;
  }
  View final_h;
  for (int j = 0; j < n_out; ++j) {
    View dest;
    if (j + 1 < n_out) {
      const int ich_next = topo.in_block_ch[n_in - 2 - j];
      dest = rs_plan::slice(cat[j + 1], 0, cat[j + 1].C - ich_next);
    } else {
      const Layer& L0 = topo.output_blocks[j][0];
      dest = P.make_view(B, cat[j].H, cat[j].W, L0.b);
    }
    int rc = run(cat[j], "output_blocks." + std::to_string(j), topo.output_blocks[j], dest, &h);
    if (rc) return rc;
    P.block_out["output_blocks." + std::to_string(j)] = h;
    final_h = h;
  }
  leave();
  View t = P.make_view(B, final_h.H, final_h.W, final_h.C);
  b.gn(final_h, "out.0", t, 1, -1);
  b.conv(t, "out.2", 3, 1, c.out_channels, nullptr, nullptr, ACT_NONE, true);

  return finish_layout(P, b, (size_t)B * std::max(c.in_channels, c.out_channels) * P.H * P.W * sizeof(float), true);
}

void resolve(rs_plan& P, View& v) {
  if (v.tens >= 0) v.ptr = reinterpret_cast<__half*>(P.ws + P.tensors[v.tens].off) + v.off;
}

bool gn_finalizes(const Op& g) {
  static const int thr = env_int("RS_GN_FINALIZE_SLOTS", 64);
  return g.gn.slots > thr && !g.gn.win_slots;
}
bool gn_producer_finalizes(const Op& g) {
  static const int on = env_int("RS_GN_PRODUCER_FINALIZE", 0);
  static const int swin_fin = env_int("RS_SWIN_FINALIZE", 0);
  if (g.gn.win_slots) return swin_fin != 0 && swin_attn_uses_tc();
  return gn_finalizes(g) && (on != 0 || !g.gn.fused);
}
GnSink make_sink(rs_plan& P, const Op& g, int coff, int img_off = 0, bool consumer = false) {
  GnSink s{};
  s.part = reinterpret_cast<float*>(P.ws + P.off_stats + g.stats_off) + (size_t)img_off * g.gn.slots * g.gn.in.C * 2;
  if (gn_producer_finalizes(g) || (consumer && gn_finalizes(g))) {
    s.gstat = reinterpret_cast<float*>(P.ws + P.off_gstat) + (size_t)g.gn_index * P.B * 64 + (size_t)img_off * 64;
    s.counter = reinterpret_cast<unsigned int*>(P.ws + P.off_counters) + (size_t)g.gn_index * P.B + img_off;
  }
  s.cstride = g.gn.in.C; s.coff = coff; s.expected = (unsigned)(g.gn.slots * g.gn.in.C); s.eps = g.gn.eps;
  return s;
}

int bind_ops(rs_plan& P, std::vector<Op>& ops) {
  rs_engine& E = *P.e;
  for (Op& op : ops) {
    if (op.kind == OP_CONV) {
      for (int i = 0; i < 2; ++i) {
        op.conv.sink[i] = GnSink{};
        if (i < (int)op.stat_dst.size()) {
          const Op::StatDst& sd = op.stat_dst[i];
          op.conv.sink[i] = make_sink(P, (sd.list == 0 ? P.fe_ops : P.ops)[sd.op], sd.coff, sd.img_off);
        }
      }
      ConvDesc& d = op.conv;
      resolve(P, d.in); if (d.has_out) resolve(P, d.out); if (d.has_res) resolve(P, d.res);
      if (!op.in_param.empty()) {
        const Param* wp = E.find(op.in_param);
        RS_CHECK(wp != nullptr && wp->ipad == d.in.ld, "missing / mismatching parameter " + op.in_param);
        d.in.ptr = E.at<__half>(op.in_param);
      }
      if (op.w_is_view) {
        resolve(P, op.w_view);
        d.wt = op.w_view.ptr; d.ipad = op.w_view.ld;
        d.bias = op.b_name.empty() ? nullptr : E.at<float>(op.b_name);
      } else {
        const Param* w = E.find(op.w_name);
        RS_CHECK(w != nullptr, "missing parameter " + op.w_name);
        d.wt = E.at<__half>(op.w_name); d.ipad = w->ipad; d.bias = E.at<float>(op.b_name);
      }
      d.out_f32 = op.to_f32 ? P.out_f32 : nullptr;
      d.partial = op.split_tens >= 0 ? reinterpret_cast<float*>(P.ws + P.tensors[op.split_tens].off) : nullptr;
      if (d.in.C < d.ipad && d.in.ld >= d.ipad && d.in.tens == P.xin.tens) d.in.C = d.ipad;
      if (d.in.C < d.ipad && P.fe_in.tens >= 0 && d.in.tens == P.fe_in.tens) d.in.C = d.ipad;
      int rc = conv_finalize(d); if (rc) return rc;
      P.launches += (d.prm.splitk > 1 && !d.prm.splitk_cluster) ? 2 : 1;
    } else if (op.kind == OP_GN) {
      resolve(P, op.gn.in); resolve(P, op.gn.out);
      op.gn.gamma = E.at<float>(op.g_name + ".weight"); op.gn.beta = E.at<float>(op.g_name + ".bias");
      RS_CHECK(op.gn.gamma && op.gn.beta, "missing GroupNorm parameters " + op.g_name);
      {
        const GnSink sk = make_sink(P, op, 0, 0, true);
        op.gn.part = sk.part; op.gn.gstat = sk.gstat; op.gn.counter = sk.counter;
        op.gn.finalize_kernel = op.gn.fused && gn_finalizes(op) && !gn_producer_finalizes(op);
      }
      P.launches += (op.gn.fused ? 1 : 2) + (op.gn.finalize_kernel ? 1 : 0);
    } else if (op.kind == OP_MLP) {
      MlpDesc& m = op.mlp;
      resolve(P, m.in); resolve(P, m.out); resolve(P, m.res);
      m.w1 = E.at<__half>(op.w_name); m.b1 = E.at<float>(op.b_name);
      m.w2 = E.at<__half>(op.w2_name); m.b2 = E.at<float>(op.b2_name);
      RS_CHECK(m.w1 && m.w2 && m.b1 && m.b2, "missing MLP parameters " + op.w_name);
      const Param* w1p = E.find(op.w_name); const Param* w2p = E.find(op.w2_name);
      RS_CHECK(w1p->ipad == m.E && w2p->ipad == m.Hd, "MLP weight padding");
      if (!op.g_name.empty()) {
        const GnSink sk = make_sink(P, op, 0);
        m.gn_in_gstat = sk.gstat; m.gn_in_part = sk.part; m.gn_in_slots = op.gn.slots;
        m.gn_in_gamma = E.at<float>(op.g_name + ".weight"); m.gn_in_beta = E.at<float>(op.g_name + ".bias");
        RS_CHECK(m.gn_in_gamma && m.gn_in_beta, "missing GroupNorm parameters " + op.g_name);
      }
      for (int i = 0; i < 2; ++i) {
        m.sink[i] = GnSink{};
        if (i < (int)op.stat_dst.size()) {
          const Op::StatDst& sd = op.stat_dst[i];
          m.sink[i] = make_sink(P, (sd.list == 0 ? P.fe_ops : P.ops)[sd.op], sd.coff, sd.img_off);
        }
      }
      int rc = mlp_finalize(m); if (rc) return rc;
      ++P.launches;
    } else if (op.kind == OP_ATTN) {
      resolve(P, op.a_in); resolve(P, op.a_out);
      op.a_bias = E.at<float>(op.w_name);
      RS_CHECK(op.a_bias != nullptr, "missing " + op.w_name);
      ++P.launches;
    } else if (op.kind == OP_SWIN_ATTN) {
      SwinAttnDesc& w = op.swin;
      resolve(P, w.x); resolve(P, w.y);
      const std::string& b = op.blk_name;
      const Param* wq = E.find(b + ".attn.qkv.weight"); const Param* wp = E.find(b + ".attn.proj.weight");
      RS_CHECK(wq && wp, "missing attention parameters of " + b);
      w.wqkv = E.at<__half>(b + ".attn.qkv.weight"); w.wqkv_ld = wq->ipad; w.bqkv = E.at<float>(b + ".attn.qkv.bias");
      w.wproj = E.at<__half>(b + ".attn.proj.weight"); w.wproj_ld = wp->ipad; w.bproj = E.at<float>(b + ".attn.proj.bias");
      w.relbias = E.at<float>(b + ".attn.relative_position_bias_table");
      w.gamma = E.at<float>(b + ".norm1.weight"); w.beta = E.at<float>(b + ".norm1.bias");
      RS_CHECK(w.bqkv && w.bproj && w.relbias && w.gamma && w.beta, "missing attention parameters of " + b);
      {
        const GnSink sk = make_sink(P, op, 0);
        w.gn_part = sk.part; w.gn_slots = op.gn.slots; w.gn_gstat = sk.gstat;
      }
      for (int i = 0; i < 2; ++i) {
        w.sink[i] = GnSink{};
        if (i < (int)op.stat_dst.size()) {
          const Op::StatDst& sd = op.stat_dst[i];
          w.sink[i] = make_sink(P, (sd.list == 0 ? P.fe_ops : P.ops)[sd.op], sd.coff, sd.img_off);
        }
      }
      int rc = swin_attn_finalize(w); if (rc) return rc;
      ++P.launches;
    } else if (op.kind == OP_FORK || op.kind == OP_JOIN) {
    } else if (op.kind == OP_SOFTMAX) {
      resolve(P, op.s_view);
      RS_CHECK(op.s_view.C % 8 == 0 && op.s_view.C <= 8192 && op.s_view.ld % 8 == 0, "softmax row length");
      ++P.launches;
    } else {
      resolve(P, op.u_in); resolve(P, op.u_out);
      ++P.launches;
    }
  }
  return 0;
}

struct Prof {
  std::vector<cudaEvent_t> ev;
  std::vector<int> kind;
  int used = 0;
  cudaEvent_t get() {
    if (used == (int)ev.size()) { cudaEvent_t e; cudaEventCreate(&e); ev.push_back(e); }
    return ev[used++];
  }
  ~Prof() { for (cudaEvent_t e : ev) cudaEventDestroy(e); }
};

inline bool op_skipped(const Op& op) {
  static const int skip = env_int("RS_SKIP_KINDS", 0);
  if (!skip) return false;
  switch (op.kind) {
    case OP_CONV: return (skip >> (op.conv.ksize == 3 ? 0 : 1)) & 1;
    case OP_GN: return (skip >> 2) & 1;
    case OP_ATTN: return (skip >> 3) & 1;
    case OP_UPSAMPLE: return (skip >> 4) & 1;
    case OP_MLP: return (skip >> 5) & 1;
    case OP_SWIN_ATTN: return (skip >> 3) & 1;
    case OP_SOFTMAX: case OP_FORK: case OP_JOIN: return false;
  }
  return false;
}

int run_ops(rs_plan& P, const std::vector<Op>& ops, const float* film_base, long long film_sN, cudaStream_t st0,
            Prof* prof = nullptr) {
  const bool multi = prof == nullptr && !P.side.empty();
  for (const Op& op : ops) {
    int rc = 0;
    if (op.kind == OP_FORK || op.kind == OP_JOIN) {
      if (multi) {
        if (op.kind == OP_FORK) {
          RS_CUDA_OK(cudaEventRecord(P.ev[0], st0));
          for (cudaStream_t s : P.side) RS_CUDA_OK(cudaStreamWaitEvent(s, P.ev[0], 0));
        } else {
          for (size_t k = 0; k < P.side.size(); ++k) {
            RS_CUDA_OK(cudaEventRecord(P.ev[k + 1], P.side[k]));
            RS_CUDA_OK(cudaStreamWaitEvent(st0, P.ev[k + 1], 0));
          }
        }
      }
      if (prof) { cudaEventRecord(prof->get(), st0); prof->kind.push_back((int)OP_UPSAMPLE); cudaEventRecord(prof->get(), st0); }
      continue;
    }
    cudaStream_t st = (multi && op.stream > 0 && op.stream <= (int)P.side.size()) ? P.side[op.stream - 1] : st0;
    if (op_skipped(op)) { if (prof) { cudaEventRecord(prof->get(), st); prof->kind.push_back((int)op.kind); cudaEventRecord(prof->get(), st); } continue; }
    if (prof) { cudaEventRecord(prof->get(), st); prof->kind.push_back((int)op.kind); }
    switch (op.kind) {
      case OP_CONV: rc = conv_launch(op.conv, st); break;
      case OP_GN: {
        GnDesc g = op.gn;
        if (g.film_off >= 0) { g.film = film_base + g.film_off + (long long)g.film_n0 * film_sN; g.film_sN = film_sN; }
        rc = gn_launch(g, st);
        break;
      }
      case OP_MLP: rc = mlp_launch(op.mlp, st); break;
      case OP_SWIN_ATTN: rc = swin_attn_launch(op.swin, st); break;
      case OP_ATTN:
        rc = attn_launch(op.a_in, op.a_out, op.a_bias, P.e->cfg.swin_heads, P.e->cfg.swin_embed_dim, op.a_shift, st);
        break;
      case OP_SOFTMAX: {
        SoftmaxParams sp{op.s_view.ptr, (long long)op.s_view.ld, op.s_view.N * op.s_view.H * op.s_view.W, op.s_view.C, op.s_scale};
        (void)launch_k(softmax_rows_kernel, dim3((unsigned)sp.rows), dim3(256), (size_t)0, st, sp);
        if (cudaGetLastError() != cudaSuccess) rc = fail(-2, "softmax launch failed");
        break;
      }
      case OP_UPSAMPLE: {
        UpsampleParams u{op.u_in.ptr, op.u_in.sN(), op.u_in.ld, op.u_out.ptr, op.u_in.N, op.u_in.H, op.u_in.W, op.u_in.C};
        const long long total = (long long)u.N * 4 * u.H * u.W * (u.C / 8);
        (void)launch_k(upsample2x_kernel, dim3((unsigned)std::min<long long>((total + 255) / 256, 148 * 16)), dim3(256), (size_t)(0), st, u);
        if (cudaGetLastError() != cudaSuccess) rc = fail(-2, "upsample launch failed");
        break;
      }
    }
    if (prof) cudaEventRecord(prof->get(), st);
    if (rc) return rc;
  }
  return 0;
}

int run_embedding(rs_plan& P, const float* tsteps, int rows, cudaStream_t st) {
  rs_engine& E = *P.e;
  const int mc = E.cfg.model_channels, K = E.time_dim();
  float* sinb = reinterpret_cast<float*>(P.ws + P.off_emb_sin);
  float* mid = reinterpret_cast<float*>(P.ws + P.off_emb_mid);
  float* vec = reinterpret_cast<float*>(P.ws + P.off_emb_vec);
  float* film = reinterpret_cast<float*>(P.ws + P.off_film);
  const int half = mc / 2;
  (void)launch_k(timestep_embedding_kernel, dim3((rows * half + 127) / 128), dim3(128), (size_t)(0), st, tsteps, sinb, rows, mc);
  auto lin = [&](const float* x, const __half* W, const float* bias, float* out, int Kin, int O, int si, int so) {
    const long long warps = (long long)rows * O;
    (void)launch_k(linear_small_kernel, dim3((unsigned)((warps * 32 + 255) / 256)), dim3(256), (size_t)(0), st, x, W, bias, out, rows, Kin, O, si, so);
  };
  const Param* w0 = E.find("time_embed.0.weight");
  RS_CHECK(w0 && w0->ipad == mc, "time_embed.0 layout");
  lin(sinb, E.at<__half>("time_embed.0.weight"), E.at<float>("time_embed.0.bias"), mid, mc, K, 0, 1);
  lin(mid, E.at<__half>("time_embed.2.weight"), E.at<float>("time_embed.2.bias"), vec, K, K, 0, 0);
  lin(vec, reinterpret_cast<__half*>(E.arena + E.film_w_off), reinterpret_cast<float*>(E.arena + E.film_b_off), film,
      K, E.film_rows, 1, 0);
  RS_CUDA_OK(cudaGetLastError());
  return 0;
}

int pack_lq_and_input(rs_plan& P, const float* x, const float* lq, const float* mask, const float* scale_tab,
                      int scale_idx, cudaStream_t st) {
  rs_engine& E = *P.e;
  const rs_unet_config& c = E.cfg;
  const long long npix = (long long)P.B * P.H * P.W;
  PackInputParams pp{};
  pp.x = x; pp.Cx = c.in_channels; pp.scale_tab = scale_tab; pp.scale_idx = scale_idx;
  pp.out = P.xin.ptr; pp.Cpad = P.cin_pad; pp.N = P.B; pp.HW = P.H * P.W;
  pp.zero_ptr = reinterpret_cast<unsigned int*>(P.ws + P.off_counters); pp.zero_n = P.n_gn * P.B;
  if (E.fe_stages() > 0) {
    RS_CHECK(!c.cond_mask || mask != nullptr, "this model is mask-conditioned: mask must be given");
    PackImageParams ip{lq, 3, c.cond_mask ? mask : nullptr, c.cond_mask ? 1 : 0, P.fe_in.ptr, P.fe_cpad, P.B, P.lqH * P.lqW};
    const long long lpix = (long long)P.B * P.lqH * P.lqW;
    (void)launch_k(pack_image_kernel, dim3((unsigned)((lpix + 255) / 256)), dim3(256), (size_t)(0), st, ip);
    int rc = run_ops(P, P.fe_ops, nullptr, 0, st); if (rc) return rc;
    pp.lq_nhwc = P.lq_feat.ptr; pp.lq_ld = P.lq_feat.ld; pp.Cl = P.lq_feat.C;
  } else {
    RS_CHECK(!c.cond_mask, "cond_mask with lq_size == image_size is not covered");
    pp.lq_nchw = lq; pp.Cl = 3;
  }
  (void)launch_k(pack_input_kernel, dim3((unsigned)((npix + 255) / 256)), dim3(256), (size_t)(0), st, pp);
  RS_CUDA_OK(cudaGetLastError());
  return 0;
}

}

extern "C" {

int rs_version(void) { return 100; }
const char* rs_last_error(void) { return g_last_error.c_str(); }

int rs_unet_create(const rs_unet_config* cfg, rs_engine** out) {
  RS_CHECK(cfg && out, "null argument");
  RS_CHECK(cfg->n_levels >= 1 && cfg->n_levels <= RS_MAX_LEVELS, "n_levels");
  RS_CHECK(cfg->swin_embed_dim == cfg->swin_heads * 32, "head_dim must be 32 (num_head_channels: 32 in every shipped yaml)");
  RS_CHECK(cfg->model_channels % 32 == 0 && cfg->swin_embed_dim % 32 == 0, "GroupNorm32 needs channels % 32 == 0");
  RS_CHECK(cfg->lq_size >= cfg->image_size, "lq_size < image_size is not covered");
  auto e = std::make_unique<rs_engine>();
  e->cfg = *cfg;
  int rc = build_inventory(*e); if (rc) return rc;
  *out = e.release();
  return 0;
}
void rs_unet_destroy(rs_engine* e) { delete e; }
int rs_unet_param_count(const rs_engine* e) { return e ? (int)e->params.size() : 0; }
int rs_unet_param_info(const rs_engine* e, int index, char* name, size_t name_cap, int32_t shape[4], int32_t* ndim,
                       int32_t* is_buffer) {
  RS_CHECK(e && index >= 0 && index < (int)e->params.size(), "index out of range");
  const Param& p = e->params[index];
  if (name && name_cap) { std::strncpy(name, p.name.c_str(), name_cap - 1); name[name_cap - 1] = 0; }
  for (int i = 0; i < 4; ++i) shape[i] = i < (int)p.shape.size() ? p.shape[i] : 1;
  if (ndim) *ndim = (int)p.shape.size();
  if (is_buffer) *is_buffer = (p.role == R_BUF_RELIDX || p.role == R_BUF_MASK) ? 1 : 0;
  return 0;
}
size_t rs_unet_arena_bytes(const rs_engine* e) { return e ? e->arena_bytes : 0; }
int rs_unet_set_arena(rs_engine* e, void* arena_dev) {
  RS_CHECK(e && arena_dev && (reinterpret_cast<uintptr_t>(arena_dev) & 255) == 0, "arena must be 256-byte aligned");
  e->arena = static_cast<uint8_t*>(arena_dev);
  return 0;
}
int rs_unet_load_param(rs_engine* e, const char* name, const float* src, void* stream) {
  RS_CHECK(e && name && src, "null argument");
  RS_CHECK(e->arena != nullptr, "rs_unet_set_arena first");
  const Param* p = e->find(name);
  RS_CHECK(p != nullptr, std::string("unknown parameter ") + name);
  cudaStream_t st = static_cast<cudaStream_t>(stream);
  ++e->weights_epoch;
  if (p->bytes == 0) return 0;
  if (p->role == R_CONV3 || p->role == R_CONV1 || p->role == R_LINEAR) {
    const int O = p->shape[0], I = p->shape[1];
    const int KH = p->shape.size() == 4 ? p->shape[2] : 1, KW = p->shape.size() == 4 ? p->shape[3] : 1;
    const long long total = (long long)O * KH * KW * p->ipad;
    (void)launch_k(pack_conv_weight_kernel, dim3((unsigned)std::min<long long>((total + 255) / 256, 4096)), dim3(256), (size_t)(0), st, 
        src, reinterpret_cast<__half*>(e->arena + p->off), O, I, KH, KW, p->ipad);
  } else if (p->role == R_RELPOS) {
    RS_CHECK(p->shape[0] == 225, "relative position table must be 15x15 (window 8)");
    (void)launch_k(expand_relpos_kernel, dim3((e->cfg.swin_heads * 4096 + 255) / 256), dim3(256), (size_t)(0), st,
        src, reinterpret_cast<float*>(e->arena + p->off), e->cfg.swin_heads);
  } else {
    long long n = 1;
    for (int v : p->shape) n *= v;
    (void)launch_k(copy_f32_kernel, dim3((unsigned)((n + 255) / 256)), dim3(256), (size_t)(0), st, src, reinterpret_cast<float*>(e->arena + p->off), n);
  }
  RS_CUDA_OK(cudaGetLastError());
  return 0;
}

int rs_plan_create(rs_engine* e, int batch, int height, int width, rs_plan** out) {
  RS_CHECK(e && out && batch > 0, "bad argument");
  RS_CHECK(e->kind == 0, "this engine is a VQ-GAN first stage: use rs_vq_plan_create");
  const int down = 1 << (e->cfg.n_levels - 1);
  RS_CHECK(height % (8 * down) == 0 && width % (8 * down) == 0,
           "latent H and W must be multiples of window_size * 2^(levels-1) (64 for the shipped configs)");
  auto p = std::make_unique<rs_plan>();
  p->e = e; p->B = batch; p->H = height; p->W = width;
  int rc = build_plan(*p); if (rc) return rc;
  *out = p.release();
  return 0;
}
void rs_plan_destroy(rs_plan* p) { delete p; }
size_t rs_plan_workspace_bytes(const rs_plan* p) { return p ? p->workspace_bytes : 0; }
int rs_plan_num_launches(const rs_plan* p) { return p ? p->launches : 0; }

int rs_plan_bind(rs_plan* p, void* workspace_dev) {
  RS_CHECK(p && workspace_dev && (reinterpret_cast<uintptr_t>(workspace_dev) & 255) == 0, "workspace must be 256-byte aligned");
  RS_CHECK(p->e->arena != nullptr, "rs_unet_set_arena before binding a plan");
  p->ws = static_cast<uint8_t*>(workspace_dev);
  if (p->vq_which >= 0) {
    p->out_f32 = reinterpret_cast<float*>(p->ws + p->off_state);
  } else {
    const size_t lat = align_up((size_t)p->B * std::max(p->e->cfg.in_channels, p->e->cfg.out_channels) * p->H * p->W * 4, 256);
    p->out_f32 = reinterpret_cast<float*>(p->ws + p->off_state + lat);
  }
  resolve(*p, p->xin);
  if (p->fe_in.tens >= 0) { resolve(*p, p->fe_in); resolve(*p, p->lq_feat); }
  for (auto& kv : p->block_out) resolve(*p, kv.second);
  p->launches = 0;
  if (p->branches > 1 && p->side.empty() && !p->sections.empty()) {
    for (int k = 1; k < p->branches; ++k) {
      cudaStream_t s = nullptr;
      RS_CUDA_OK(cudaStreamCreateWithFlags(&s, cudaStreamNonBlocking));
      p->side.push_back(s);
    }
    for (int k = 0; k < p->branches; ++k) {
      cudaEvent_t e = nullptr;
      RS_CUDA_OK(cudaEventCreateWithFlags(&e, cudaEventDisableTiming));
      p->ev.push_back(e);
    }
  }
  int rc = conv_init(); if (rc) return rc;
  rc = bind_ops(*p, p->fe_ops); if (rc) return rc;
  rc = bind_ops(*p, p->ops); if (rc) return rc;
  p->launches += p->vq_which >= 0 ? 3 : 6;
  p->bound = true;
  return 0;
}

int rs_plan_forward(rs_plan* p, const float* x, const float* timesteps, const float* lq, const float* mask, float* out,
                    void* stream) {
  RS_CHECK(p && p->bound, "plan is not bound");
  RS_CHECK(p->vq_which < 0, "this is a VQ-GAN plan: use rs_vq_encode / rs_vq_decode");
  RS_CHECK(x && timesteps && lq && out, "null tensor");
  cudaStream_t st = static_cast<cudaStream_t>(stream);
  p->table_owner = nullptr;
  int rc = run_embedding(*p, timesteps, p->B, st); if (rc) return rc;
  rc = pack_lq_and_input(*p, x, lq, mask, nullptr, 0, st); if (rc) return rc;
  const float* film = reinterpret_cast<const float*>(p->ws + p->off_film);
  rc = run_ops(*p, p->ops, film, p->e->film_rows, st); if (rc) return rc;
  const long long n = (long long)p->B * p->e->cfg.out_channels * p->H * p->W;
  (void)launch_k(copy_f32_kernel, dim3((unsigned)((n + 255) / 256)), dim3(256), (size_t)(0), st, p->out_f32, out, n);
  RS_CUDA_OK(cudaGetLastError());
  return 0;
}

int rs_plan_profile(rs_plan* p, const float* x, const float* timesteps, const float* lq, const float* mask,
                    double* ms_by_kind, double* conv_flops, int32_t* n_conv_launches, void* stream) {
  RS_CHECK(p && p->bound && ms_by_kind && p->vq_which < 0, "bad argument (needs a bound denoiser plan)");
  cudaStream_t st = static_cast<cudaStream_t>(stream);
  p->table_owner = nullptr;
  int rc = run_embedding(*p, timesteps, p->B, st); if (rc) return rc;
  rc = pack_lq_and_input(*p, x, lq, mask, nullptr, 0, st); if (rc) return rc;
  Prof prof;
  const float* film = reinterpret_cast<const float*>(p->ws + p->off_film);
  rc = run_ops(*p, p->ops, film, p->e->film_rows, st, &prof); if (rc) return rc;
  RS_CUDA_OK(cudaStreamSynchronize(st));
  for (int k = 0; k < 4; ++k) ms_by_kind[k] = 0.0;
  for (size_t i = 0; i < prof.kind.size(); ++i) {
    float ms = 0.f;
    cudaEventElapsedTime(&ms, prof.ev[2 * i], prof.ev[2 * i + 1]);
    const int kd = prof.kind[i];
    ms_by_kind[(kd == (int)OP_MLP || kd == (int)OP_SWIN_ATTN) ? 0 : kd] += ms;
  }
  double fl = 0.0; int nc = 0;
  for (const Op& op : p->ops) if (op.kind == OP_MLP) {
    fl += 4.0 * (double)op.mlp.in.N * op.mlp.in.H * op.mlp.in.W * op.mlp.E * (double)op.mlp.Hd;
    ++nc;
  } else if (op.kind == OP_CONV) {
    const ConvParams& c = op.conv.prm;
    const int cin_real = op.conv.in.tens == p->xin.tens ? p->e->cfg.in_channels + p->e->lq_feat_ch() : op.conv.in.C;
    fl += 2.0 * (double)c.Nimg * c.Hout * c.Wout * c.Cout * (double)c.num_taps * cin_real;
    ++nc;
  } else if (op.kind == OP_SWIN_ATTN) {
    const double M = (double)op.swin.x.N * op.swin.x.H * op.swin.x.W, Ed = (double)op.swin.x.C;
    fl += M * (8.0 * Ed * Ed + 256.0 * Ed);
    ++nc;
  }
  if (conv_flops) *conv_flops = fl;
  if (n_conv_launches) *n_conv_launches = nc;
  return 0;
}

static void collect_profile(const rs_plan& P, const Prof& prof, double* ms, char* desc, int desc_stride, int cap, int32_t* n_ops) {
  const rs_plan* p = &P;
  const int n = std::min<int>((int)p->ops.size(), cap);
  *n_ops = n;
  for (int i = 0; i < n; ++i) {
    float t = 0.f;
    cudaEventElapsedTime(&t, prof.ev[2 * i], prof.ev[2 * i + 1]);
    ms[i] = t;
    const Op& op = p->ops[i];
    char* d = desc + (size_t)i * desc_stride;
    if (op.kind == OP_CONV) {
      const ConvParams& c = op.conv.prm;
      snprintf(d, desc_stride, "conv%dx%d s%d %dx%d Cin=%d Cout=%d grid=%d BN=%d st=%d %s", op.conv.ksize, op.conv.ksize,
               op.conv.stride, c.Hout, c.Wout, op.conv.in.C, c.Cout, op.conv.grid, c.BN, c.stages, op.w_name.c_str());
    } else if (op.kind == OP_GN) {
      snprintf(d, desc_stride, "gn %dx%d C=%d fused=%d %s", op.gn.in.H, op.gn.in.W, op.gn.in.C, (int)op.gn.fused, op.g_name.c_str());
    } else if (op.kind == OP_MLP) {
      snprintf(d, desc_stride, "mlp %dx%d E=%d Hd=%d grid=%d", op.mlp.in.H, op.mlp.in.W, op.mlp.E, op.mlp.Hd, op.mlp.grid);
    } else if (op.kind == OP_ATTN) {
      snprintf(d, desc_stride, "attn %dx%d shift=%d", op.a_in.H, op.a_in.W, op.a_shift);
    } else if (op.kind == OP_SWIN_ATTN) {
      snprintf(d, desc_stride, "swin_attn %dx%d shift=%d grid=%d", op.swin.x.H, op.swin.x.W, op.swin.shift, op.swin.grid);
    } else if (op.kind == OP_FORK || op.kind == OP_JOIN) {
      snprintf(d, desc_stride, "%s", op.kind == OP_FORK ? "fork" : "join");
    } else if (op.kind == OP_SOFTMAX) {
      snprintf(d, desc_stride, "softmax %d", op.s_view.C);
    } else {
      snprintf(d, desc_stride, "upsample %dx%d C=%d", op.u_in.H, op.u_in.W, op.u_in.C);
    }
  }
}

int rs_plan_profile_ops(rs_plan* p, const float* x, const float* timesteps, const float* lq, const float* mask,
                        double* ms, char* desc, int desc_stride, int cap, int32_t* n_ops, void* stream) {
  RS_CHECK(p && p->bound && ms && desc && n_ops, "bad argument");
  cudaStream_t st = static_cast<cudaStream_t>(stream);
  p->table_owner = nullptr;
  int rc = run_embedding(*p, timesteps, p->B, st); if (rc) return rc;
  rc = pack_lq_and_input(*p, x, lq, mask, nullptr, 0, st); if (rc) return rc;
  Prof prof;
  const float* film = reinterpret_cast<const float*>(p->ws + p->off_film);
  rc = run_ops(*p, p->ops, film, p->e->film_rows, st, &prof); if (rc) return rc;
  RS_CUDA_OK(cudaStreamSynchronize(st));
  collect_profile(*p, prof, ms, desc, desc_stride, cap, n_ops);
  return 0;
}

__global__ void probe_kernel(const __half* src, long long sN, int ld, float* dst, int N, int HW, int C) {
  pdl_trigger();
  pdl_wait();
  const long long i = (long long)blockIdx.x * blockDim.x + threadIdx.x;
  if (i >= (long long)N * C * HW) return;
  const int hw = (int)(i % HW); const int c = (int)((i / HW) % C); const int n = (int)(i / ((long long)HW * C));
  dst[i] = __half2float(src[n * sN + (long long)hw * ld + c]);
}

int rs_plan_probe(rs_plan* p, const char* block, float* dst, int32_t* channels, int32_t* h, int32_t* w, void* stream) {
  RS_CHECK(p && p->bound && block, "bad argument");
  auto it = p->block_out.find(block);
  RS_CHECK(it != p->block_out.end(), std::string("unknown block ") + block);
  const View& v = it->second;
  if (channels) *channels = v.C; if (h) *h = v.H; if (w) *w = v.W;
  if (dst) {
    const long long n = (long long)v.N * v.C * v.H * v.W;
    (void)launch_k(probe_kernel, dim3((unsigned)((n + 255) / 256)), dim3(256), (size_t)(0), static_cast<cudaStream_t>(stream), v.ptr, v.sN(), v.ld, dst, v.N, v.H * v.W, v.C);
    RS_CUDA_OK(cudaGetLastError());
  }
  return 0;
}

}

struct rs_sampler {
  rs_plan* p = nullptr;
  int T = 0;
  double kappa = 0;
  std::vector<float> coef1, coef2, stdv, in_scale, tsteps;
  float prior_coef = 0;
  float* tap_pred = nullptr; float* tap_sample = nullptr;
  cudaGraphExec_t graph = nullptr;
  cudaStream_t cap_stream = nullptr;
  const void* g_zy = nullptr; const void* g_noise = nullptr; const void* g_lq = nullptr; const void* g_mask = nullptr;
  void* g_out = nullptr;
};

namespace {

int sampler_enqueue(rs_sampler& S, const float* z_y, const float* noises, const float* lq, const float* mask,
                    float* out_latent, cudaStream_t st) {
  rs_plan& P = *S.p;
  const rs_unet_config& c = P.e->cfg;
  RS_CHECK(c.in_channels == c.out_channels, "predict_type xstart needs out_channels == in_channels");
  const long long numel = (long long)P.B * c.in_channels * P.H * P.W;
  const size_t lat = align_up((size_t)numel * 4, 256);
  float* x_t = reinterpret_cast<float*>(P.ws + P.off_state);
  float* tab = reinterpret_cast<float*>(P.ws + P.off_tables);
  const float* coef1 = tab, *coef2 = tab + 1024, *stdv = tab + 2048, *in_scale = tab + 3072;
  (void)lat;
  (void)launch_k(prior_sample_kernel, dim3((unsigned)((numel + 255) / 256)), dim3(256), (size_t)(0), st, z_y, noises, x_t, S.prior_coef, numel);
  int rc = pack_lq_and_input(P, x_t, lq, mask, in_scale, S.T - 1, st); if (rc) return rc;
  const float* film_all = reinterpret_cast<const float*>(P.ws + P.off_film);
  for (int k = 0; k < S.T; ++k) {
    const int t = S.T - 1 - k;
    rc = run_ops(P, P.ops, film_all + (long long)t * P.e->film_rows, 0, st); if (rc) return rc;
    PSampleParams pp{};
    pp.x_t = x_t; pp.x0 = P.out_f32; pp.noise = noises + (long long)(k + 1) * numel;
    pp.x_next = (t == 0) ? out_latent : x_t;
    pp.coef1 = coef1; pp.coef2 = coef2; pp.stdv = stdv; pp.in_scale = in_scale; pp.t = t;
    pp.N = P.B; pp.C = c.in_channels; pp.HW = P.H * P.W;
    pp.next_in = P.xin.ptr; pp.next_cpad = P.cin_pad;
    pp.zero_ptr = reinterpret_cast<unsigned int*>(P.ws + P.off_counters); pp.zero_n = P.n_gn * P.B;
    if (S.tap_pred) RS_CUDA_OK(cudaMemcpyAsync(S.tap_pred + (long long)k * numel, P.out_f32, numel * 4, cudaMemcpyDeviceToDevice, st));
    (void)launch_k(p_sample_kernel, dim3((unsigned)((numel + 255) / 256)), dim3(256), (size_t)(0), st, pp);
    if (S.tap_sample) RS_CUDA_OK(cudaMemcpyAsync(S.tap_sample + (long long)k * numel, pp.x_next, numel * 4, cudaMemcpyDeviceToDevice, st));
  }
  RS_CUDA_OK(cudaGetLastError());
  return 0;
}

int sampler_prepare(rs_sampler& S, cudaStream_t st) {
  rs_plan& P = *S.p;
  if (P.table_owner == &S && P.table_epoch == P.e->weights_epoch) return 0;
  float* tab = reinterpret_cast<float*>(P.ws + P.off_tables);
  RS_CUDA_OK(cudaMemcpyAsync(tab, S.coef1.data(), S.T * 4, cudaMemcpyHostToDevice, st));
  RS_CUDA_OK(cudaMemcpyAsync(tab + 1024, S.coef2.data(), S.T * 4, cudaMemcpyHostToDevice, st));
  RS_CUDA_OK(cudaMemcpyAsync(tab + 2048, S.stdv.data(), S.T * 4, cudaMemcpyHostToDevice, st));
  RS_CUDA_OK(cudaMemcpyAsync(tab + 3072, S.in_scale.data(), S.T * 4, cudaMemcpyHostToDevice, st));
  float* ts = reinterpret_cast<float*>(P.ws + P.off_tsteps);
  RS_CUDA_OK(cudaMemcpyAsync(ts, S.tsteps.data(), S.T * 4, cudaMemcpyHostToDevice, st));
  int rc = run_embedding(P, ts, S.T, st); if (rc) return rc;
  RS_CUDA_OK(cudaStreamSynchronize(st));
  P.table_owner = &S; P.table_epoch = P.e->weights_epoch;
  return 0;
}

}

extern "C" {

int rs_sampler_create(rs_plan* p, int steps, const double* sqrt_etas, double kappa, const int32_t* tmap, rs_sampler** out) {
  RS_CHECK(p && p->bound && sqrt_etas && out, "bad argument (plan must be bound)");
  RS_CHECK(p->vq_which < 0, "samplers are built on denoiser plans");
  RS_CHECK(steps >= 2 && steps <= p->max_rows && steps <= 1024, "steps out of range for this plan");
  auto s = std::make_unique<rs_sampler>();
  s->p = p; s->T = steps; s->kappa = kappa;
  std::vector<double> etas(steps), prev(steps), alpha(steps), pv(steps);
  for (int i = 0; i < steps; ++i) etas[i] = sqrt_etas[i] * sqrt_etas[i];
  for (int i = 0; i < steps; ++i) { prev[i] = i ? etas[i - 1] : 0.0; alpha[i] = etas[i] - prev[i]; pv[i] = kappa * kappa * prev[i] / etas[i] * alpha[i]; }
  s->coef1.resize(steps); s->coef2.resize(steps); s->stdv.resize(steps); s->in_scale.resize(steps); s->tsteps.resize(steps);
  for (int i = 0; i < steps; ++i) {
    const double pvc = pv[i == 0 ? 1 : i];
    s->coef1[i] = (float)(prev[i] / etas[i]);
    s->coef2[i] = (float)(alpha[i] / etas[i]);
    const float logv = (float)std::log(pvc);
    s->stdv[i] = std::exp(0.5f * logv);
    const float e32 = (float)etas[i];
    s->in_scale[i] = 1.0f / std::sqrt(e32 * (float)(kappa * kappa) + 1.0f);
    s->tsteps[i] = (float)(tmap ? tmap[i] : i);
  }
  s->prior_coef = (float)(kappa * sqrt_etas[steps - 1]);
  *out = s.release();
  return 0;
}
void rs_sampler_destroy(rs_sampler* s) {
  if (s && s->p && s->p->table_owner == s) s->p->table_owner = nullptr;
  if (s && s->graph) cudaGraphExecDestroy(s->graph);
  if (s && s->cap_stream) cudaStreamDestroy(s->cap_stream);
// ... 95 lines not shown
```

### resshift_b200/csrc/gn_stats.cuh

```cuda
#pragma once

#include "common.cuh"

namespace rs {

struct GnSink {
  float* part;
  float* gstat;
  unsigned int* counter;
  int cstride;
  int coff;
  unsigned int expected;
  float eps;
};

#ifdef __CUDACC__

__device__ __forceinline__ float2 ldcg_f2(const float* p) {
  float2 v;
  asm volatile("ld.global.cg.v2.f32 {%0, %1}, [%2];" : "=f"(v.x), "=f"(v.y) : "l"(p) : "memory");
  return v;
}

__device__ __forceinline__ unsigned int atom_add_acq_rel_gpu(unsigned int* p, unsigned int v) {
// ... 55 lines not shown
    }
    const int g = g0 + q * gstep;
    const float invK = 1.0f / (float)K;
    const float dm = a * invK;
    const float m2 = fmaxf(b - ns * (float)K * dm * dm, 0.f);
    const float var = m2 * invK / ns;
    if (lane == 0 && g < 32) {
      gstat[((size_t)n * 32 + g) * 2] = pivot[q] + dm;
      gstat[((size_t)n * 32 + g) * 2 + 1] = rsqrtf(var + eps);
    }
  }
}

template <int kMax>
__device__ __forceinline__ void gn_arrive(const GnSink* const (&sink)[kMax], const int (&img)[kMax], const unsigned int (&add)[kMax],
                                          int slots, float ns, int tid, int nthreads, int bar_id, int* s_flag ) {
  named_bar_sync(bar_id, nthreads);
  if (tid < kMax) {
    int last = 0;
    if (sink[tid] != nullptr && img[tid] >= 0 && sink[tid]->gstat != nullptr) {
      const unsigned int old = atom_add_acq_rel_gpu(sink[tid]->counter + img[tid], add[tid]);
      last = (old + add[tid] == sink[tid]->expected) ? 1 : 0;
    }
    s_flag[tid] = last;
  }
  named_bar_sync(bar_id, nthreads);
  const int warp = tid >> 5, lane = tid & 31, nwarps = nthreads >> 5;
#pragma unroll
  for (int i = 0; i < kMax; ++i) {
    if (!s_flag[i]) continue;
    const GnSink& s = *sink[i];
    const int cpg = s.cstride / 32;
    for (int g = warp; g < 32; g += 4 * nwarps) gn_finalize_groups<4>(s.part, img[i], slots, s.cstride, g, nwarps, cpg, ns, s.eps, s.gstat, lane);
  }
  named_bar_sync(bar_id, nthreads);
}

constexpr int kGnListCap = 64;
struct GnArriveList {
  int cnt;
  int over;
  short sink[kGnListCap];
  short img[kGnListCap];
  unsigned int add[kGnListCap];
  int flag[kGnListCap];
};
__device__ __forceinline__ void gn_list_add(GnArriveList* L, int d, int img, unsigned int add) {
  for (int j = 0; j < L->cnt; ++j)
    if (L->sink[j] == d && L->img[j] == img) { L->add[j] += add; return; }
  const int j = L->cnt++;
  L->sink[j] = (short)d; L->img[j] = (short)img; L->add[j] = add;
}
__device__ __forceinline__ void gn_list_arrive(GnArriveList* L, const GnSink& s0, const GnSink& s1, int slots, float ns, int tid,
                                               int nthreads, int bar_id) {
  named_bar_sync(bar_id, nthreads);
  const int cnt = L->cnt;
  for (int j = tid; j < cnt; j += nthreads) {
    const GnSink& s = L->sink[j] == 0 ? s0 : s1;
    const unsigned int old = atom_add_acq_rel_gpu(s.counter + L->img[j], L->add[j]);
    L->flag[j] = (old + L->add[j] == s.expected) ? 1 : 0;
  }
  named_bar_sync(bar_id, nthreads);
  const int warp = tid >> 5, lane = tid & 31, nwarps = nthreads >> 5;
  for (int j = 0; j < cnt; ++j) {
    if (!L->flag[j]) continue;
    const GnSink& s = L->sink[j] == 0 ? s0 : s1;
    const int cpg = s.cstride / 32;
    for (int g = warp; g < 32; g += 4 * nwarps) gn_finalize_groups<4>(s.part, L->img[j], slots, s.cstride, g, nwarps, cpg, ns, s.eps, s.gstat, lane);
  }
  named_bar_sync(bar_id, nthreads);
  if (tid == 0) L->cnt = 0;
}

template <typename Ld>
__device__ __forceinline__ void pivot_stats2(Ld ld, int rows, float2& mean, float2& m2) {
  const float2 p = ld(0);
  float2 s1 = make_float2(0.f, 0.f), s2 = make_float2(0.f, 0.f);
  for (int r = 1; r < rows; ++r) {
    const float2 v = ld(r);
    const float dx = v.x - p.x, dy = v.y - p.y;
    s1.x += dx; s1.y += dy;
    s2.x = fmaf(dx, dx, s2.x); s2.y = fmaf(dy, dy, s2.y);
  }
  const float inv = 1.0f / (float)rows;
  mean = make_float2(p.x + s1.x * inv, p.y + s1.y * inv);
  m2 = make_float2(fmaxf(s2.x - s1.x * s1.x * inv, 0.f), fmaxf(s2.y - s1.y * s1.y * inv, 0.f));
}

__device__ __forceinline__ void warp_chunk_stats(const uint4& o0, const uint4& o1, int lane, float* dst) {
  float sv[16], sq[16];
  const __half2* q0 = reinterpret_cast<const __half2*>(&o0);
  const __half2* q1 = reinterpret_cast<const __half2*>(&o1);
#pragma unroll
  for (int j = 0; j < 4; ++j) {
    const float2 x0 = __half22float2(q0[j]);
    const float2 x1 = __half22float2(q1[j]);
    sv[2 * j] = x0.x; sv[2 * j + 1] = x0.y; sv[8 + 2 * j] = x1.x; sv[8 + 2 * j + 1] = x1.y;
  }
#pragma unroll
  for (int j = 0; j < 16; ++j) sq[j] = sv[j] * sv[j];
#pragma unroll
  for (int half = 8, bit = 16; half >= 1; half >>= 1, bit >>= 1) {
    const bool upper = (lane & bit) != 0;
#pragma unroll
    for (int j = 0; j < half; ++j) {
      const float send_s = upper ? sv[j] : sv[j + half];
      const float keep_s = upper ? sv[j + half] : sv[j];
      sv[j] = keep_s + __shfl_xor_sync(0xffffffffu, send_s, bit);
      const float send_q = upper ? sq[j] : sq[j + half];
      const float keep_q = upper ? sq[j + half] : sq[j];
      sq[j] = keep_q + __shfl_xor_sync(0xffffffffu, send_q, bit);
    }
  }
  sv[0] += __shfl_xor_sync(0xffffffffu, sv[0], 1);
  sq[0] += __shfl_xor_sync(0xffffffffu, sq[0], 1);
  if ((lane & 1) == 0) {
    const int cidx = ((lane >> 4) & 1) * 8 + ((lane >> 3) & 1) * 4 + ((lane >> 2) & 1) * 2 + ((lane >> 1) & 1);
    const float mean = sv[0] * (1.0f / 32.0f);
    dst[cidx * 2] = mean;
    dst[cidx * 2 + 1] = fmaxf(sq[0] - sv[0] * mean, 0.f);
  }
}

__device__ __forceinline__ void write_quad_pairs(const float* wq, int BN, int ncols, int col0, int bn, int n0, int Nimg, int slot,
                                                 int slots, const GnSink& s0, const GnSink& s1, int tid, int nthreads) {
  for (int cc = tid; cc < ncols; cc += nthreads) {
    float m[4], q[4];
#pragma unroll
    for (int k = 0; k < 4; ++k) { m[k] = wq[((size_t)k * BN + cc) * 2]; q[k] = wq[((size_t)k * BN + cc) * 2 + 1]; }
    float ma, qa, mb, qb;
    chan_merge_equal(32.f, m[0], q[0], m[1], q[1], ma, qa);
    chan_merge_equal(32.f, m[2], q[2], m[3], q[3], mb, qb);
#pragma unroll
    for (int d = 0; d < 2; ++d) {
      const GnSink& s = d == 0 ? s0 : s1;
      if (!s.part) continue;
      const size_t ch = (size_t)s.coff + col0 + cc;
      float* dst = s.part + (((size_t)n0 * slots + slot) * s.cstride + ch) * 2;
      if (bn == 1) {
        float mm, qq;
        chan_merge_equal(64.f, ma, qa, mb, qb, mm, qq);
        dst[0] = mm; dst[1] = qq;
      } else {
        dst[0] = ma; dst[1] = qa;
        if (n0 + 1 < Nimg) {
          float* dst1 = s.part + (((size_t)(n0 + 1) * slots + slot) * s.cstride + ch) * 2;
          dst1[0] = mb; dst1[1] = qb;
        }
      }
    }
  }
}

__device__ __forceinline__ void write_tile_pairs(const float* wstat, int BN, int ncols, int col0, int bn, int n0, int Nimg, int slot,
                                                 int slots, const GnSink& s0, const GnSink& s1, int tid, int nthreads) {
  for (int cc = tid; cc < ncols; cc += nthreads) {
    const float m0 = wstat[((size_t)0 * BN + cc) * 2], q0 = wstat[((size_t)0 * BN + cc) * 2 + 1];
    const float m1 = wstat[((size_t)1 * BN + cc) * 2], q1 = wstat[((size_t)1 * BN + cc) * 2 + 1];
#pragma unroll
    for (int d = 0; d < 2; ++d) {
      const GnSink& s = d == 0 ? s0 : s1;
      if (!s.part) continue;
      const size_t ch = (size_t)s.coff + col0 + cc;
      float* dst = s.part + (((size_t)n0 * slots + slot) * s.cstride + ch) * 2;
      if (bn == 1) {
        float m, q;
        chan_merge_equal(64.f, m0, q0, m1, q1, m, q);
        dst[0] = m; dst[1] = q;
      } else {
        dst[0] = m0; dst[1] = q0;
        if (n0 + 1 < Nimg) {
          float* dst1 = s.part + (((size_t)(n0 + 1) * slots + slot) * s.cstride + ch) * 2;
          dst1[0] = m1; dst1[1] = q1;
        }
      }
    }
  }
}

__device__ __forceinline__ float2 gn_channel_from_pairs(const float* part_nc , int slots, int C, float ns) {
  const float pivot = reinterpret_cast<const float2*>(part_nc)->x;
  float s1 = 0.f, s2 = 0.f;
  int sl = 0;
  for (; sl + 16 <= slots; sl += 16) {
    float2 e[16];
#pragma unroll
    for (int u = 0; u < 16; ++u) e[u] = *reinterpret_cast<const float2*>(part_nc + (size_t)(sl + u) * C * 2);
#pragma unroll
    for (int u = 0; u < 16; ++u) { const float d = e[u].x - pivot; s1 += d; s2 += fmaf(ns * d, d, e[u].y); }
  }
  for (; sl + 4 <= slots; sl += 4) {
    float2 e[4];
#pragma unroll
    for (int u = 0; u < 4; ++u) e[u] = *reinterpret_cast<const float2*>(part_nc + (size_t)(sl + u) * C * 2);
#pragma unroll
    for (int u = 0; u < 4; ++u) { const float d = e[u].x - pivot; s1 += d; s2 += fmaf(ns * d, d, e[u].y); }
  }
  for (; sl < slots; ++sl) {
    const float2 e = *reinterpret_cast<const float2*>(part_nc + (size_t)sl * C * 2);
    const float d = e.x - pivot; s1 += d; s2 += fmaf(ns * d, d, e.y);
  }
  const float dm = s1 / (float)slots;
  return make_float2(pivot + dm, fmaxf(s2 - ns * (float)slots * dm * dm, 0.f));
}
__device__ __forceinline__ float2 gn_group_from_channels(const float* ch_pairs , int cpg, float cnt, float eps) {
  const float pivot = ch_pairs[0];
  float s1 = 0.f, s2 = 0.f;
  for (int j = 0; j < cpg; ++j) { const float d = ch_pairs[2 * j] - pivot; s1 += d; s2 += fmaf(cnt * d, d, ch_pairs[2 * j + 1]); }
  const float dm = s1 / (float)cpg;
  const float m2 = fmaxf(s2 - cnt * (float)cpg * dm * dm, 0.f);
  return make_float2(pivot + dm, rsqrtf(m2 / (cnt * (float)cpg) + eps));
}

#endif
}
```

### resshift_b200/csrc/launch.cuh

```cuda
#pragma once

#include <algorithm>
#include <cstdlib>
#include <cmath>
#include <cstring>
#include <utility>
#include <vector>

#include "common.cuh"
#include "conv_gemm.cuh"
#include "conv_persist.cuh"
#include "elementwise.cuh"
#include "mlp_fused.cuh"
#include "norm_act.cuh"
#include "window_attn.cuh"
#include "swin_attn_fused.cuh"
#include "swin_attn_tc.cuh"

namespace rs {

typedef CUresult (*PFN_encodeTiled)(CUtensorMap*, CUtensorMapDataType, cuuint32_t, void*, const cuuint64_t*,
                                    const cuuint64_t*, const cuuint32_t*, const cuuint32_t*, CUtensorMapInterleave,
                                    CUtensorMapSwizzle, CUtensorMapL2promotion, CUtensorMapFloatOOBfill);

inline PFN_encodeTiled get_encode_tiled() {
  static PFN_encodeTiled fn = nullptr;
  if (!fn) {
    void* p = nullptr;
    cudaDriverEntryPointQueryResult q;
    if (cudaGetDriverEntryPoint("cuTensorMapEncodeTiled", &p, cudaEnableDefault, &q) == cudaSuccess &&
        q == cudaDriverEntryPointSuccess)
      fn = reinterpret_cast<PFN_encodeTiled>(p);
  }
  return fn;
}

struct View {
  __half* ptr = nullptr;
  int tens = -1;
  long long off = 0;
  int c0 = 0, n0 = 0;
  int N = 0, H = 0, W = 0, C = 0, ld = 0;
  long long sW() const { return ld; }
  long long sH() const { return (long long)W * ld; }
  long long sN() const { return (long long)H * W * ld; }
};

inline int encode_act_map(CUtensorMap* m, const __half* base, int C, int W, int H, int N, long long sW,
                          long long sH, long long sN, int bw, int bh, int bn, int box_c = kConvBK) {
  PFN_encodeTiled enc = get_encode_tiled();
  RS_CHECK(enc != nullptr, "cuTensorMapEncodeTiled entry point not available (no CUDA driver?)");
  cuuint64_t dims[4] = {(cuuint64_t)C, (cuuint64_t)W, (cuuint64_t)H, (cuuint64_t)N};
  cuuint64_t strides[3] = {(cuuint64_t)sW * 2, (cuuint64_t)sH * 2, (cuuint64_t)sN * 2};
  cuuint32_t box[4] = {(cuuint32_t)box_c, (cuuint32_t)bw, (cuuint32_t)bh, (cuuint32_t)bn};
  const CUtensorMapSwizzle swz = box_c == 64 ? CU_TENSOR_MAP_SWIZZLE_128B
                                 : (box_c == 32 ? CU_TENSOR_MAP_SWIZZLE_64B : CU_TENSOR_MAP_SWIZZLE_32B);
  RS_CHECK(box_c == 64 || box_c == 32 || box_c == 16, "activation box width");
  cuuint32_t estr[4] = {1, 1, 1, 1};
  RS_CHECK((reinterpret_cast<uintptr_t>(base) & 15) == 0, "activation base must be 16-byte aligned");
  RS_CHECK(sW % 8 == 0 && sH % 8 == 0 && sN % 8 == 0, "activation strides must be multiples of 16 bytes");
  CUresult r = enc(m, CU_TENSOR_MAP_DATA_TYPE_FLOAT16, 4, const_cast<__half*>(base), dims, strides, box, estr,
                   CU_TENSOR_MAP_INTERLEAVE_NONE, swz, CU_TENSOR_MAP_L2_PROMOTION_L2_128B,
                   CU_TENSOR_MAP_FLOAT_OOB_FILL_NONE);
  RS_CHECK(r == CUDA_SUCCESS, "cuTensorMapEncodeTiled(activation) failed with CUresult " + std::to_string((int)r));
  return 0;
}
inline int encode_weight_map(CUtensorMap* m, const __half* base, int Ktot, int Cout, int BN) {
  PFN_encodeTiled enc = get_encode_tiled();
  RS_CHECK(enc != nullptr, "cuTensorMapEncodeTiled entry point not available (no CUDA driver?)");
  cuuint64_t dims[2] = {(cuuint64_t)Ktot, (cuuint64_t)Cout};
  cuuint64_t strides[1] = {(cuuint64_t)Ktot * 2};
  cuuint32_t box[2] = {(cuuint32_t)kConvBK, (cuuint32_t)BN};
  cuuint32_t estr[2] = {1, 1};
  RS_CHECK((reinterpret_cast<uintptr_t>(base) & 15) == 0 && Ktot % 8 == 0, "weight matrix must be 16-byte aligned");
  CUresult r = enc(m, CU_TENSOR_MAP_DATA_TYPE_FLOAT16, 2, const_cast<__half*>(base), dims, strides, box, estr,
                   CU_TENSOR_MAP_INTERLEAVE_NONE, CU_TENSOR_MAP_SWIZZLE_128B, CU_TENSOR_MAP_L2_PROMOTION_L2_256B,
                   CU_TENSOR_MAP_FLOAT_OOB_FILL_NONE);
  RS_CHECK(r == CUDA_SUCCESS, "cuTensorMapEncodeTiled(weights) failed with CUresult " + std::to_string((int)r));
  return 0;
}

inline int env_int(const char* name, int dflt) {
  const char* v = std::getenv(name);
  return v ? std::atoi(v) : dflt;
}
inline bool env_is(const char* name, const char* val) {
  const char* v = std::getenv(name);
  return v && std::strcmp(v, val) == 0;
}

template <typename... KArgs, typename... Args>
inline cudaError_t launch_kc(void (*kernel)(KArgs...), dim3 grid, dim3 block, size_t smem, cudaStream_t st,
                             int cluster_x, Args&&... args) {
  static const int use_pdl = env_int("RS_PDL", 1);
  cudaLaunchConfig_t cfg{};
  cfg.gridDim = grid; cfg.blockDim = block; cfg.dynamicSmemBytes = smem; cfg.stream = st;
  cudaLaunchAttribute attr[2];
  int n = 0;
  if (use_pdl) {
    attr[n].id = cudaLaunchAttributeProgrammaticStreamSerialization;
    attr[n].val.programmaticStreamSerializationAllowed = 1;
    ++n;
  }
  if (cluster_x > 1) {
    attr[n].id = cudaLaunchAttributeClusterDimension;
    attr[n].val.clusterDim.x = cluster_x; attr[n].val.clusterDim.y = 1; attr[n].val.clusterDim.z = 1;
    ++n;
  }
  cfg.attrs = attr; cfg.numAttrs = n;
  return cudaLaunchKernelEx(&cfg, kernel, std::forward<Args>(args)...);
}
template <typename... KArgs, typename... Args>
inline cudaError_t launch_k(void (*kernel)(KArgs...), dim3 grid, dim3 block, size_t smem, cudaStream_t st,
                            Args&&... args) {
  return launch_kc(kernel, grid, block, smem, st, 1, std::forward<Args>(args)...);
}

inline int pow2_floor_div(int x, int cap) {
  int p = 1;
  while (p * 2 <= cap && x % (p * 2) == 0) p *= 2;
  return p;
}

struct ConvDesc {
  View in;
  int ksize = 1, stride = 1;
  int pad_lo = 1;
  const __half* wt = nullptr;
  int ipad = 0;
  const float* bias = nullptr;
  int Cout = 0;
  View out;
  bool has_out = true;
  View res; bool has_res = false;
  float* out_f32 = nullptr;
  int act = ACT_NONE;
  int bn_override = 0;
  unsigned long long* dbg = nullptr;
  float* partial = nullptr;
  bool allow_split = false;
  SplitKReduceParams red;
  int red_grid_x = 0, red_grid_z = 1; size_t red_smem = 0;
  GnSink sink[2] = {};
  ConvParams prm;
  ConvSimtSrc simt;
  int grid = 0; size_t smem = 0;
};

struct TileConfig { int BN = 0, msub = 1, stages = 2, occ = 1, cg = 1, splitk = 1, persist = 0, cluster_split = 0; double est_cycles = 1e30; };

inline TileConfig pick_tile_config(int m_tiles, int cout16, int num_kb, int f_bn, bool allow_split = false, bool allow_persist = false,
                                   bool allow_cluster_split = false) {
  const int f_msub = env_int("RS_CONV_MSUB", 0), f_occ = env_int("RS_CONV_OCC", 0), f_stages = env_int("RS_CONV_STAGES", 0);
  const int f_cg = env_int("RS_CONV_CG", 0);
  TileConfig best, bestp;
  double best_real = 1e30;
  for (int cand = std::min(cout16, 256); cand >= 16; cand -= 16) {
    if (f_bn ? (cand != std::min(f_bn, std::min(cout16, 256))) : (cout16 % cand != 0)) continue;
    const int n_tiles = (cout16 + cand - 1) / cand;
    for (int cg = 1; cg <= 2; ++cg) {
      if (f_cg && cg != f_cg && !(f_cg == 2 && m_tiles < 2)) continue;
      if (cg == 2 && (cand % 16 != 0 || m_tiles < 2)) continue;
      if (allow_persist && 2 * cand <= 512) {
        const long long units_p = (long long)((m_tiles + cg - 1) / cg) * n_tiles;
        const int workers = cg == 2 ? 74 : 148;
        const int sbytes_p = kConvBM * kConvBK * 2 + (cand / cg) * kConvBK * 2;
        const size_t extra = (size_t)2 * cand * kConvBM * 2 + (size_t)cand * 40 + 1280 + sizeof(GnArriveList);
        const int st_p = (int)std::min<size_t>(8, ((size_t)227 * 1024 - extra) / (size_t)sbytes_p);
        if ((m_tiles + cg - 1) / cg >= 2 * workers && st_p >= 2) {
          const double kb_p = std::max(std::max(2.0 * cand, 2.0 * sbytes_p / 128.0), 2600.0 / st_p);
          const double epi_p = 5000.0 + 3.0 * cand;
          const double rounds = std::ceil((double)units_p / workers);
          const double total = rounds * std::max(num_kb * kb_p, epi_p) + epi_p + 3000.0;
          if (total < bestp.est_cycles) {
            bestp.est_cycles = total; bestp.BN = cand; bestp.msub = 1; bestp.stages = std::min(st_p, std::max(2, num_kb));
            bestp.occ = 1; bestp.cg = cg; bestp.splitk = 1; bestp.persist = 1;
          }
        }
      }
      for (int ms = 1; ms <= 2; ++ms) {
        if (ms == 2 && (f_msub != 2 || cg == 2 || m_tiles % 2 || 2 * cand > 512)) continue;
        const int sbytes = ms * kConvBM * kConvBK * 2 + (cand / cg) * kConvBK * 2;
        for (int occ = 1; occ <= 2; ++occ) {
          if (f_occ && occ != f_occ) continue;
          if (occ == 2 && ms * cand > 256) continue;
          const int budget = (occ == 2 ? 111 : 222) * 1024 - 2048;
          int st = std::min(std::min(8, std::max(2, num_kb)), budget / sbytes);
          {
            const int st_need = (int)(((size_t)ms * ((size_t)cand * kConvBM * 2 + (size_t)4 * cand * 2 * sizeof(float)) + 16 + sbytes - 1) / sbytes);
            if (st_need > budget / sbytes) continue;
            st = std::max(st, st_need);
          }
          if (f_stages) st = f_stages;
          if (st < 2 || (size_t)st * sbytes + 2304 > (size_t)(occ == 2 ? 113 : 227) * 1024) continue;
          const double smem_cycles = (sbytes + ms * (kConvBM * kConvBK * 2.0 + (cand / cg) * kConvBK * 2.0)) / 128.0;
          const double load_lat = m_tiles >= 64 ? 3000.0 : 7500.0;
          const double kb_cycles = std::max(occ * std::max(ms * 2.0 * cand, smem_cycles), load_lat / st);
          const double epi = 18.0 * cand * ms + 3000.0 + (cg == 2 ? 2500.0 : 0.0);
          const long long units = (long long)((m_tiles + cg * ms - 1) / (cg * ms)) * n_tiles;
          const double slots = (cg == 2 ? 74.0 : 148.0) * occ;
          const int f_split = env_int("RS_CONV_SPLITK", 0);
          const int kSplits[6] = {1, 2, 3, 4, 6, 8};
          const char* f_mode = std::getenv("RS_CONV_SPLITK_MODE");
          for (int mode = 0; mode < 2; ++mode)
          for (int si = 0; si < 6; ++si) {
            const int S = kSplits[si];
            if (mode == 1 && (S != 2 || !allow_cluster_split || cg != 2 || occ != 1 || (cand / S) % 8 != 0)) continue;
            if (mode == 1 && f_mode && std::strcmp(f_mode, "global") == 0) continue;
            if (mode == 0 && S > 1 && f_mode && std::strcmp(f_mode, "cluster") == 0) continue;
            if (mode == 1 && (size_t)kConvBM * (cand * 4 + 16) + (size_t)kConvBM * (cand / S) * 2 + (size_t)4 * (cand / S) * 4 + 16 > (size_t)st * sbytes) continue;
            if (S > 1 && ((mode == 0 && !allow_split) || ms != 1 || num_kb / S < 6)) continue;
            if (f_split && (allow_split || allow_cluster_split) && ms == 1 && num_kb / f_split >= 6 && S != f_split) continue;
            const double waves = std::ceil((double)units * S / slots);
            const double kbs = std::ceil((double)num_kb / S);
            const double round = kbs * kb_cycles + (occ == 2 ? 0.5 * epi : epi);
            const double part_bytes = 4.0 * m_tiles * 128.0 * cout16 * S;
            const double total = waves * round + (S == 1 ? 0.0 : mode == 1 ? 6000.0 : 19000.0 + 2.0 * part_bytes / 2048.0);
            if (total < best.est_cycles) {
              best.est_cycles = total; best.BN = cand; best.msub = ms;
              best.stages = std::max(std::min(st, (int)std::max(2.0, kbs)), std::min(st, (int)(((size_t)ms * ((size_t)cand * kConvBM * 2 + (size_t)4 * cand * 2 * sizeof(float)) + 16 + sbytes - 1) / sbytes)));
              best.occ = occ; best.cg = cg; best.splitk = S; best.persist = 0; best.cluster_split = (S > 1 && mode == 1) ? 1 : 0;
              best_real = waves * (kbs * kb_cycles + epi + 5000.0) + (S == 1 ? 0.0 : mode == 1 ? 6000.0 : 19000.0 + 2.0 * part_bytes / 2048.0);
            }
          }
        }
      }
    }
  }
  if (bestp.BN && 0.85 * bestp.est_cycles < best_real) return bestp;
  return best;
}

inline TileConfig conv_preview_config(int N, int Hin, int Win, int Cin, int Cout, int ksize, int stride, bool allow_split) {
  const int Hout = Hin / stride, Wout = Win / stride;
  const int bw = pow2_floor_div(Wout, kConvBM);
  const int bh = pow2_floor_div(Hout, kConvBM / bw);
  const int bn = kConvBM / (bw * bh);
  const int m_tiles = (Wout / bw) * (Hout / bh) * ((N + bn - 1) / bn);
  const bool contiguous = (bw == Wout) || (bh == 1);
  const int num_kb = ksize * ksize * ((Cin + kConvBK - 1) / kConvBK);
  const bool sp = allow_split && contiguous && bn <= 2;
  return pick_tile_config(m_tiles, (Cout + 15) / 16 * 16, num_kb, env_int("RS_CONV_BN", 0), sp, false, sp && Cout % 8 == 0);
}

inline int conv_finalize(ConvDesc& d) {
  ConvParams& p = d.prm;
  std::memset(&p, 0, sizeof(p));
  const int Hin = d.in.H, Win = d.in.W;
  RS_CHECK(d.ksize == 1 || d.ksize == 3, "kernel size must be 1 or 3");
  RS_CHECK(d.stride == 1 || (d.stride == 2 && d.ksize == 3 && Hin % 2 == 0 && Win % 2 == 0), "unsupported stride");
  const int Hout = Hin / d.stride, Wout = Win / d.stride, N = d.in.N;
  p.Hout = Hout; p.Wout = Wout; p.Nimg = N; p.Cout = d.Cout;
  p.num_taps = d.ksize * d.ksize;
  p.kchunks = (d.in.C + kConvBK - 1) / kConvBK;
  {
    const int tail = d.in.C - (p.kchunks - 1) * kConvBK;
    p.tail_k16 = env_int("RS_CONV_TAILSKIP", 1) ? (tail + 15) / 16 : kConvBK / 16;
  }
  p.w_tap_stride = d.ipad;
  RS_CHECK(d.ipad % 8 == 0 && d.ipad >= d.in.C, "weight channel padding");
  p.bw = pow2_floor_div(Wout, kConvBM);
  p.bh = pow2_floor_div(Hout, kConvBM / p.bw);
  p.bn = kConvBM / (p.bw * p.bh);
  p.tiles_w = Wout / p.bw; p.tiles_h = Hout / p.bh; p.tiles_n = (N + p.bn - 1) / p.bn;
  const int m_tiles = p.tiles_w * p.tiles_h * p.tiles_n;
  const int cout16 = (d.Cout + 15) / 16 * 16;
  const int num_kb = p.num_taps * p.kchunks;
  const bool contiguous_tiles = (p.bw == Wout) || (p.bh == 1);
  const bool can_split = d.allow_split && d.partial != nullptr && contiguous_tiles && p.bn <= 2 && d.has_out && !d.out_f32;
  const int want_persist = env_int("RS_CONV_PERSIST", -1);
  const bool persist_ok = d.has_out && !d.out_f32 && want_persist != 0 && !env_is("RS_CONV_EPI", "direct") &&
                          !env_is("RS_CONV_IMPL", "simt") && env_int("RS_CONV_MSUB", 0) != 2 &&
                          (!(d.sink[0].part || d.sink[1].part) || 2 * N <= kGnListCap);
  const bool can_cluster_split = d.allow_split && contiguous_tiles && p.bn <= 2 && d.has_out && !d.out_f32 && d.Cout % 8 == 0;
  const TileConfig tc = pick_tile_config(m_tiles, cout16, num_kb, d.bn_override ? d.bn_override : env_int("RS_CONV_BN", 0), can_split,
                                         persist_ok && want_persist != 1, can_cluster_split);
  const int BN = tc.BN, msub = tc.msub, stages = tc.stages, cg = tc.cg;
  p.cg = cg;
  p.splitk = tc.splitk; p.partial = d.partial; p.splitk_cluster = tc.cluster_split;
  RS_CHECK(BN >= 16 && BN <= 256 && BN % 16 == 0, "no valid tile configuration");
  p.BN = BN; p.n_tiles = (cout16 + BN - 1) / BN;
  p.msub = msub;
  int cols = 32; while (cols < msub * BN) cols *= 2;
  p.tmem_cols = cols;
  const int stage_bytes = msub * kConvBM * kConvBK * 2 + (BN / cg) * kConvBK * 2;
  p.stages = stages;
  d.smem = (size_t)stages * stage_bytes + 1024 + 256 + 1024;
  RS_CHECK(d.smem <= 227 * 1024, "shared memory budget exceeded");
  d.grid = (cg == 2 ? ((m_tiles + 1) / 2) * p.n_tiles * 2 : (m_tiles / msub) * p.n_tiles) * p.splitk;
  if (d.stride == 1) {
    int t = 0;
    for (int ky = 0; ky < d.ksize; ++ky)
      for (int kx = 0; kx < d.ksize; ++kx, ++t) {
        p.tap_src[t] = 0; p.tap_dh[t] = ky - d.ksize / 2; p.tap_dw[t] = kx - d.ksize / 2;
      }
  } else {
    int t = 0;
    for (int ky = 0; ky < 3; ++ky)
      for (int kx = 0; kx < 3; ++kx, ++t) {
        if (d.pad_lo == 1) {
          const int hp = (ky == 1) ? 0 : 1, wp = (kx == 1) ? 0 : 1;
          p.tap_src[t] = hp * 2 + wp; p.tap_dh[t] = (ky == 0) ? -1 : 0; p.tap_dw[t] = (kx == 0) ? -1 : 0;
        } else {
          const int hp = (ky == 1) ? 1 : 0, wp = (kx == 1) ? 1 : 0;
          p.tap_src[t] = hp * 2 + wp; p.tap_dh[t] = (ky == 2) ? 1 : 0; p.tap_dw[t] = (kx == 2) ? 1 : 0;
        }
      }
  }
  p.bias = d.bias; p.act = d.act;
  if (d.has_res) {
    RS_CHECK(d.res.H == Hout && d.res.W == Wout && d.res.N == N && d.res.C >= d.Cout, "residual geometry");
    p.residual = d.res.ptr; p.res_sN = d.res.sN(); p.res_sH = d.res.sH(); p.res_sW = d.res.sW();
  }
  if (d.has_out) {
    RS_CHECK(d.out.H == Hout && d.out.W == Wout && d.out.N == N, "output geometry");
    p.out = d.out.ptr; p.out_sN = d.out.sN(); p.out_sH = d.out.sH(); p.out_sW = d.out.sW();
    RS_CHECK(d.out.ld % 8 == 0 && (reinterpret_cast<uintptr_t>(d.out.ptr) & 15) == 0, "output alignment");
  }
  p.out_f32_nchw = d.out_f32;
  p.dbg = d.dbg;
  p.tma_out = (d.has_out && !d.out_f32 && p.splitk == 1 && !env_is("RS_CONV_EPI", "direct") && !env_is("RS_CONV_IMPL", "simt")) ? 1 : 0;
  p.tma_res = (p.tma_out && d.has_res) ? 1 : 0;
  p.epi_bc = (BN % 64 == 0) ? 64 : (BN % 32 == 0 ? 32 : 16);
  if (p.tma_out) {
    int rc = encode_act_map(&p.tmOut, d.out.ptr, d.Cout, Wout, Hout, N, d.out.sW(), d.out.sH(), d.out.sN(), p.bw, p.bh, p.bn, p.epi_bc);
    if (rc) return rc;
    if (p.tma_res) {
      rc = encode_act_map(&p.tmRes, d.res.ptr, d.Cout, Wout, Hout, N, d.res.sW(), d.res.sH(), d.res.sN(), p.bw, p.bh, p.bn, p.epi_bc);
      if (rc) return rc;
    }
    const size_t need = (size_t)msub * ((size_t)BN * kConvBM * 2 + (size_t)4 * BN * 2 * sizeof(float)) + 16;
    RS_CHECK(tc.persist || need <= (size_t)stages * stage_bytes, "epilogue staging does not fit in the pipeline shared memory");
  }
  {
    const int units = (cg == 2 ? (m_tiles + 1) / 2 : m_tiles) * p.n_tiles;
    const int workers = cg == 2 ? 74 : 148;
    const bool eligible = persist_ok && p.tma_out && p.splitk == 1 && msub == 1 && 2 * BN <= 512;
    p.persist = (eligible && (tc.persist || want_persist == 1)) ? 1 : 0;
    RS_CHECK(!tc.persist || p.persist, "persistent configuration chosen for an ineligible layer");
    p.num_units = units;
    if (p.persist) {
      const size_t extra = (size_t)2 * BN * kConvBM * 2 + (size_t)4 * BN * 2 * sizeof(float) + (size_t)2 * BN * sizeof(float) + 256 + 1024 + sizeof(GnArriveList);
      const int st = (int)std::min<size_t>(8, ((size_t)227 * 1024 - extra) / (size_t)stage_bytes);
      RS_CHECK(st >= 2, "persistent conv: shared memory budget");
      p.stages = std::min(st, std::max(2, num_kb));
      d.smem = (size_t)p.stages * stage_bytes + extra;
      int cols2 = 32; while (cols2 < 2 * BN) cols2 *= 2;
      p.tmem_cols = cols2;
      d.grid = cg * std::min(units, workers);
    }
  }
  p.gn_slots = p.tiles_w * p.tiles_h;
  RS_CHECK(!(d.sink[0].part || d.sink[1].part) || p.bn <= 2, "fused GroupNorm statistics need tiles of at most two images");
  auto fill_sinks = [&](GnSink* dst) {
    int k = 0;
    for (int i = 0; i < 2; ++i) {
      dst[i] = GnSink{};
      if (!d.sink[i].part) continue;
      dst[k] = d.sink[i];
      if (dst[k].expected == 0) dst[k].expected = (unsigned)(p.gn_slots * dst[k].cstride);
      if (dst[k].eps == 0.f) dst[k].eps = 1e-5f;
      ++k;
    }
  };
  {
    GnSink none[2] = {};
    if (p.tma_out) fill_sinks(p.sink); else { p.sink[0] = none[0]; p.sink[1] = none[1]; }
  }
  if (p.splitk > 1 && p.splitk_cluster) {
    fill_sinks(p.sink);
    RS_CHECK(cg == 2 && d.Cout % 8 == 0 && (BN / p.splitk) % 8 == 0, "cluster split-K configuration");
  } else if (p.splitk > 1) {
    SplitKReduceParams& r = d.red;
    std::memset(&r, 0, sizeof(r));
    r.partial = d.partial; r.S = p.splitk; r.N = N; r.HW = Hout * Wout; r.C = d.Cout;
    r.bias = d.bias; r.act = d.act;
    if (d.has_res) { r.residual = d.res.ptr; r.res_sN = d.res.sN(); r.res_ld = d.res.ld; }
    r.out = d.out.ptr; r.out_sN = d.out.sN(); r.out_ld = d.out.ld;
    r.rows_per_slot = p.bw * p.bh; r.slots = p.tiles_w * p.tiles_h;
    fill_sinks(r.sink);
    RS_CHECK(d.Cout % 8 == 0 && d.Cout <= 2048, "split-K reduce needs Cout % 8 == 0");
    p.bias = nullptr; p.residual = nullptr; p.act = ACT_NONE; p.sink[0] = GnSink{}; p.sink[1] = GnSink{};
    d.red_grid_x = r.slots;
    int cpc = d.Cout;
    while (cpc > 64 && cpc % 16 == 0 && (long long)r.slots * N * (d.Cout / cpc) < 2 * 148) cpc /= 2;
    r.cols_per_cta = cpc;
    d.red_grid_z = (d.Cout + cpc - 1) / cpc;
    const int lanes = 256 / std::max(1, cpc / 8);
    d.red_smem = (size_t)std::max(1, lanes) * cpc * 3 * sizeof(float) + 16;
  }
  ConvSimtSrc& s = d.simt;
  std::memset(&s, 0, sizeof(s));
  s.C = d.in.C; s.wt = d.wt;
  const int nsrc = d.stride == 1 ? 1 : 4;
  for (int i = 0; i < kMaxSrc; ++i) {
    const int j = i < nsrc ? i : 0;
    const int hp = d.stride == 2 ? (j >> 1) : 0, wp = d.stride == 2 ? (j & 1) : 0;
    const __half* base = d.in.ptr + (long long)hp * d.in.sH() + (long long)wp * d.in.sW();
    const long long sW = d.in.sW() * d.stride, sH = d.in.sH() * d.stride, sN = d.in.sN();
    s.ptr[i] = base; s.sN[i] = sN; s.sH[i] = sH; s.sW[i] = sW; s.H[i] = Hout; s.W[i] = Wout;
    if (!env_is("RS_CONV_IMPL", "simt")) {
      int rc = encode_act_map(&p.tmA[i], base, d.in.C, Wout, Hout, N, sW, sH, sN, p.bw, p.bh, p.bn);
      if (rc) return rc;
    }
  }
  if (!env_is("RS_CONV_IMPL", "simt")) {
    int rc = encode_weight_map(&p.tmB, d.wt, p.num_taps * d.ipad, d.Cout, BN / cg);
    if (rc) return rc;
  }
  return 0;
}

inline int conv_init() {
  static bool attr_set = false;
  if (!attr_set) {
    RS_CUDA_OK(cudaFuncSetAttribute(conv_gemm_sm100_kernel<1>, cudaFuncAttributeMaxDynamicSharedMemorySize, 227 * 1024));
    RS_CUDA_OK(cudaFuncSetAttribute(conv_gemm_sm100_kernel<2>, cudaFuncAttributeMaxDynamicSharedMemorySize, 227 * 1024));
    RS_CUDA_OK(cudaFuncSetAttribute(conv_gemm_persist_sm100_kernel<1>, cudaFuncAttributeMaxDynamicSharedMemorySize, 227 * 1024));
    RS_CUDA_OK(cudaFuncSetAttribute(conv_gemm_persist_sm100_kernel<2>, cudaFuncAttributeMaxDynamicSharedMemorySize, 227 * 1024));
    RS_CUDA_OK(cudaFuncSetAttribute(window_attn_kernel, cudaFuncAttributeMaxDynamicSharedMemorySize, 160 * 1024));
    RS_CUDA_OK(cudaFuncSetAttribute(mlp_fused_sm100_kernel, cudaFuncAttributeMaxDynamicSharedMemorySize, 227 * 1024));
    RS_CUDA_OK(cudaFuncSetAttribute(swin_attn_fused_kernel<192>, cudaFuncAttributeMaxDynamicSharedMemorySize, (int)SwinSmem<192>::total));
    RS_CUDA_OK(cudaFuncSetAttribute(swin_attn_fused_kernel<64>, cudaFuncAttributeMaxDynamicSharedMemorySize, (int)SwinSmem<64>::total));
    RS_CUDA_OK(cudaFuncSetAttribute(swin_attn_tc_kernel<192>, cudaFuncAttributeMaxDynamicSharedMemorySize, (int)SwinTcSmem<192>::total));
    RS_CUDA_OK(cudaFuncSetAttribute(swin_attn_tc_kernel<64>, cudaFuncAttributeMaxDynamicSharedMemorySize, (int)SwinTcSmem<64>::total));
    attr_set = true;
  }
  return 0;
}

inline int conv_launch(const ConvDesc& d, cudaStream_t st) {
  if (env_is("RS_CONV_IMPL", "simt")) {
    const long long npix = (long long)d.prm.Nimg * d.prm.Hout * d.prm.Wout;
    const int warps = 8;
    (void)launch_k(conv_simt_kernel, dim3((unsigned)((npix + warps - 1) / warps)), dim3(warps * 32), (size_t)(0), st, d.prm, d.simt);
  } else {
    if (d.prm.persist && d.prm.cg == 2)
      (void)launch_kc(conv_gemm_persist_sm100_kernel<2>, dim3(d.grid), dim3(kConvThreads), (size_t)(d.smem), st, 2, d.prm);
    else if (d.prm.persist)
      (void)launch_kc(conv_gemm_persist_sm100_kernel<1>, dim3(d.grid), dim3(kConvThreads), (size_t)(d.smem), st, 1, d.prm);
    else if (d.prm.cg == 2)
      (void)launch_kc(conv_gemm_sm100_kernel<2>, dim3(d.grid), dim3(kConvThreads), (size_t)(d.smem), st,
                      d.prm.splitk_cluster ? 2 * d.prm.splitk : 2, d.prm);
    else
      (void)launch_kc(conv_gemm_sm100_kernel<1>, dim3(d.grid), dim3(kConvThreads), (size_t)(d.smem), st, 1, d.prm);
    if (d.prm.splitk > 1 && !d.prm.splitk_cluster)
      (void)launch_k(splitk_reduce_kernel, dim3(d.red_grid_x, d.prm.Nimg, d.red_grid_z), dim3(256), d.red_smem, st, d.red);
  }
  RS_CUDA_OK(cudaGetLastError());
  return 0;
}

inline int conv_tile_slots(int H, int W, bool* fusable = nullptr) {
  const int bw = pow2_floor_div(W, kConvBM);
  const int bh = pow2_floor_div(H, kConvBM / bw);
  if (fusable) *fusable = (kConvBM / (bw * bh)) <= 2;
  return (W / bw) * (H / bh);
}

struct GnDesc {
  View in, out;
  const float* gamma = nullptr; const float* beta = nullptr;
  const float* film = nullptr; long long film_sN = 0;
  int film_off = -1;
  int film_n0 = 0;
  int silu = 0;
  float* part = nullptr;
  float* gstat = nullptr;
  unsigned int* counter = nullptr;
  float eps = 1e-5f;
  int slots = 0;
  bool fused = false;
  bool win_slots = false;
  bool finalize_kernel = false;
};

inline void gn_chunks(int HW, int N, int* chunks, int* rows) {
  int c = std::max(1, std::min((HW + 31) / 32, (148 * 4 + N - 1) / N));
  while (c > 1 && HW % c != 0) --c;
  *chunks = c; *rows = HW / c;
}

inline int gn_launch(const GnDesc& g, cudaStream_t st) {
  const int C = g.in.C, HW = g.in.H * g.in.W, N = g.in.N;
  RS_CHECK(C % 32 == 0 && C % 8 == 0 && C <= 2048, "GroupNorm channel count");
  RS_CHECK(g.in.ld % 8 == 0 && g.out.ld % 8 == 0, "GroupNorm view alignment");
  int chunks, rows;
  gn_chunks(HW, N, &chunks, &rows);
  int slots = g.slots;
  RS_CHECK(g.gstat != nullptr || g.part != nullptr, "GroupNorm needs a statistics buffer");
  if (!g.fused) {
    slots = chunks;
    const int lanes = 256 / (C / 8);
    RS_CHECK(g.part != nullptr && (g.gstat == nullptr || g.counter != nullptr), "GroupNorm statistics buffers");
    GnStatsParams sp{};
    sp.x = g.in.ptr; sp.sN = g.in.sN(); sp.ld = g.in.ld; sp.C = C; sp.HW = HW; sp.N = N;
    sp.sink.part = g.part; sp.sink.gstat = g.gstat; sp.sink.counter = g.counter; sp.sink.cstride = C; sp.sink.coff = 0;
    sp.sink.expected = (unsigned)(slots * C); sp.sink.eps = g.eps;
    sp.slots = slots; sp.rows_per_slot = rows;
    (void)launch_k(gn_stats_kernel, dim3(chunks, N), dim3(256), (size_t)lanes * C * 3 * sizeof(float) + 16, st, sp);
    RS_CUDA_OK(cudaGetLastError());
  }
  if (g.fused && g.finalize_kernel) {
    RS_CHECK(g.part != nullptr && g.gstat != nullptr && slots > 0 && HW % slots == 0, "GroupNorm finalisation buffers");
    GnFinalizeParams fp{g.part, g.gstat, slots, C, (float)(HW / slots), g.eps};
    (void)launch_k(gn_finalize_kernel, dim3(32, N), dim3(256), (size_t)0, st, fp);
    RS_CUDA_OK(cudaGetLastError());
  }
  int actas = std::max(1, std::min((HW + 15) / 16, (148 * 4 + N - 1) / N));
  const int arows = (HW + actas - 1) / actas;
  actas = (HW + arows - 1) / arows;
  int csplit = 1;
  {
    const int cpg = C / 32;
    int unit = cpg; while (unit % 8) unit += cpg;
    for (int cs = 2; actas * N * csplit < 222 && cs <= C / unit; ++cs)
      if (C % cs == 0 && (C / cs) % unit == 0) csplit = cs;
  }
  GnApplyParams ap{g.in.ptr, g.in.sN(), g.in.ld, g.out.ptr, g.out.sN(), g.out.ld, C, HW, N, g.gstat, g.part, slots, g.eps,
                   g.gamma, g.beta, g.film, g.film_sN, g.silu, arows, C / csplit};
  (void)launch_k(gn_apply_kernel, dim3(actas, N, csplit), dim3(256), (size_t)(4 * (C / csplit) + 64) * sizeof(float), st, ap);
  RS_CUDA_OK(cudaGetLastError());
  return 0;
}

// ... 191 lines not shown
```

### resshift_b200/csrc/norm_act.cuh

```cuda
#pragma once

#include "common.cuh"
#include "gn_stats.cuh"

namespace rs {

struct GnStatsParams {
  const __half* x;
  long long sN;
  int ld, C, HW, N;
  GnSink sink;
  int slots;
  int rows_per_slot;
};

struct GnApplyParams {
  const __half* x; long long x_sN; int x_ld;
  __half* y; long long y_sN; int y_ld;
  int C, HW, N;
  const float* gstat;
  const float* part;
  int slots;
  float eps;
  const float* gamma;
// ... 35 lines not shown
      } else {
#pragma unroll
        for (int j = 0; j < 8; ++j) { const float d = st[j] - pv[j]; s1[j] += d; s2[j] = fmaf(d, d, s2[j]); }
      }
      ++cnt;
    };
    int r = r0 + rl;
    for (; r + 3 * lanes < r1; r += 4 * lanes) {
      uint4 raw[4];
#pragma unroll
      for (int u = 0; u < 4; ++u) raw[u] = *reinterpret_cast<const uint4*>(base + (long long)(r + u * lanes) * p.ld);
#pragma unroll
      for (int u = 0; u < 4; ++u) acc(raw[u]);
    }
    for (; r < r1; r += lanes) acc(*reinterpret_cast<const uint4*>(base + (long long)r * p.ld));
    float* dst = s_red + ((size_t)rl * p.C + vec * 8) * 3;
    const float inv = cnt ? 1.0f / (float)cnt : 0.f;
#pragma unroll
    for (int j = 0; j < 8; ++j) {
      dst[3 * j] = (float)cnt;
      dst[3 * j + 1] = pv[j] + s1[j] * inv;
      dst[3 * j + 2] = fmaxf(s2[j] - s1[j] * s1[j] * inv, 0.f);
    }
  }
  __syncthreads();
  for (int i = threadIdx.x; i < p.C; i += blockDim.x) {
    float cn = 0.f, mean = 0.f, m2 = 0.f;
    for (int l = 0; l < lanes; ++l) {
      const float* e = s_red + ((size_t)l * p.C + i) * 3;
      const float nb = e[0];
      if (nb == 0.f) continue;
      const float tot = cn + nb, d = e[1] - mean;
      mean += d * (nb / tot);
      m2 += e[2] + d * d * (cn * nb / tot);
      cn = tot;
    }
    float* dst = p.sink.part + (((size_t)n * p.slots + slot) * p.C + i) * 2;
    dst[0] = mean; dst[1] = m2;
  }
  if (!p.sink.gstat) return;
  int* s_flag = reinterpret_cast<int*>(s_red + (size_t)lanes * p.C * 3);
  const GnSink* const sk[1] = {&p.sink};
  const int im[1] = {n};
  const unsigned int ad[1] = {(unsigned)p.C};
  gn_arrive<1>(sk, im, ad, p.slots, (float)p.rows_per_slot, threadIdx.x, blockDim.x, 1, s_flag);
}

struct GnFinalizeParams {
  const float* part;
  float* gstat;
  int slots, C;
  float ns, eps;
};

__global__ void __launch_bounds__(256) gn_finalize_kernel(const GnFinalizeParams p) {
  pdl_trigger();
  pdl_wait();
  __shared__ float s_w[8][2];
  const int g = blockIdx.x, n = blockIdx.y;
  const int cpg = p.C >> 5;
  const int K = p.slots * cpg;
  const float* base = p.part + (size_t)n * p.slots * p.C * 2 + (size_t)g * cpg * 2;
  const float pivot = ldcg_f2(base).x;
  float s1 = 0.f, s2 = 0.f;
  auto item = [&](int i) -> float2 {
    const int sl = i / cpg, c = i - sl * cpg;
    return ldcg_f2(base + ((size_t)sl * p.C + c) * 2);
  };
  int i = threadIdx.x;
  for (; i + 3 * 256 < K; i += 4 * 256) {
    float2 e[4];
#pragma unroll
    for (int u = 0; u < 4; ++u) e[u] = item(i + u * 256);
#pragma unroll
    for (int u = 0; u < 4; ++u) { const float d = e[u].x - pivot; s1 += d; s2 += fmaf(p.ns * d, d, e[u].y); }
  }
  for (; i < K; i += 256) { const float2 e = item(i); const float d = e.x - pivot; s1 += d; s2 += fmaf(p.ns * d, d, e.y); }
#pragma unroll
  for (int off = 16; off; off >>= 1) {
    s1 += __shfl_xor_sync(0xffffffffu, s1, off);
    s2 += __shfl_xor_sync(0xffffffffu, s2, off);
  }
  const int warp = threadIdx.x >> 5, lane = threadIdx.x & 31;
  if (lane == 0) { s_w[warp][0] = s1; s_w[warp][1] = s2; }
  __syncthreads();
  if (threadIdx.x == 0) {
    float a = 0.f, b = 0.f;
#pragma unroll
    for (int w = 0; w < 8; ++w) { a += s_w[w][0]; b += s_w[w][1]; }
    const float invK = 1.0f / (float)K;
    const float dm = a * invK;
    const float m2 = fmaxf(b - p.ns * (float)K * dm * dm, 0.f);
    p.gstat[((size_t)n * 32 + g) * 2] = pivot + dm;
    p.gstat[((size_t)n * 32 + g) * 2 + 1] = rsqrtf(m2 * invK / p.ns + p.eps);
  }
}

__global__ void __launch_bounds__(256, 4) gn_apply_kernel(const GnApplyParams p) {
  pdl_trigger();
  extern __shared__ float s_ab[];
  const int Cs = p.Cs;
  const int c0 = blockIdx.z * Cs;
  float* s_a = s_ab;
  float* s_b = s_ab + Cs;
  float* s_g = s_ab + 2 * Cs;
  float* s_be = s_ab + 3 * Cs;
  float* s_mean = s_ab + 4 * Cs;
  float* s_rstd = s_mean + 32;
  const int n = blockIdx.y;
  const int cpg = p.C / 32;
  for (int c = threadIdx.x; c < Cs; c += blockDim.x) { s_g[c] = __ldg(p.gamma + c0 + c); s_be[c] = __ldg(p.beta + c0 + c); }
  pdl_wait();
  const int vecs = Cs >> 3;
  const int lanes = blockDim.x / vecs;
  const int vec = threadIdx.x % vecs, rl = threadIdx.x / vecs;
  const bool active = rl < lanes;
  const int c = vec * 8;
  const int r0 = blockIdx.x * p.rows_per_cta;
  const int r1 = min(r0 + p.rows_per_cta, p.HW);
  const __half* xb = p.x + n * p.x_sN + c0 + c;
  __half* yb = p.y + n * p.y_sN + c0 + c;
  int r = r0 + rl;
  constexpr int kPre = 4;
  uint4 pre[kPre];
#pragma unroll
  for (int u = 0; u < kPre; ++u)
    if (active && r + u * lanes < r1) pre[u] = *reinterpret_cast<const uint4*>(xb + (long long)(r + u * lanes) * p.x_ld);
  if (p.gstat) {
    if (threadIdx.x < Cs / cpg) {
      const float2 mr = ldcg_f2(p.gstat + ((size_t)n * 32 + c0 / cpg + threadIdx.x) * 2);
      s_mean[threadIdx.x] = mr.x; s_rstd[threadIdx.x] = mr.y;
    }
  } else {
    const float ns = (float)p.HW / (float)p.slots;
    const float* part = p.part + (size_t)n * p.slots * p.C * 2 + (size_t)c0 * 2;
    for (int cc = threadIdx.x; cc < Cs; cc += blockDim.x) {
      const float2 mq = gn_channel_from_pairs(part + (size_t)cc * 2, p.slots, p.C, ns);
      s_a[cc] = mq.x; s_b[cc] = mq.y;
    }
    __syncthreads();
    if (threadIdx.x < Cs / cpg) {
      const int g = threadIdx.x;
      float chp[2 * 64];
      for (int j = 0; j < cpg; ++j) { chp[2 * j] = s_a[g * cpg + j]; chp[2 * j + 1] = s_b[g * cpg + j]; }
      const float2 mr = gn_group_from_channels(chp, cpg, (float)p.HW, p.eps);
      s_mean[g] = mr.x; s_rstd[g] = mr.y;
    }
  }
  __syncthreads();
  {
    const float* f = p.film ? p.film + n * p.film_sN + c0 : nullptr;
    for (int cc = threadIdx.x; cc < Cs; cc += blockDim.x) {
      const int g = cc / cpg;
      float a = s_rstd[g] * s_g[cc];
      float b = s_be[cc] - s_mean[g] * a;
      if (f) { const float sc = 1.0f + f[cc]; a *= sc; b = b * sc + f[p.C + cc]; }
      s_a[cc] = a; s_b[cc] = b;
    }
  }
  __syncthreads();
  if (!active) return;
  float a[8], b[8];
#pragma unroll
  for (int j = 0; j < 8; ++j) { a[j] = s_a[c + j]; b[j] = s_b[c + j]; }
  auto one = [&](const uint4& raw) {
    const __half2* h = reinterpret_cast<const __half2*>(&raw);
    uint4 o;
    __half2* oh = reinterpret_cast<__half2*>(&o);
#pragma unroll
    for (int j = 0; j < 4; ++j) {
      float2 f = __half22float2(h[j]);
      f.x = fmaf(f.x, a[2 * j], b[2 * j]);
      f.y = fmaf(f.y, a[2 * j + 1], b[2 * j + 1]);
      if (p.silu) { f.x = silu_f(f.x); f.y = silu_f(f.y); }
      oh[j] = __floats2half2_rn(f.x, f.y);
    }
    return o;
  };
#pragma unroll
  for (int u = 0; u < kPre; ++u)
    if (r + u * lanes < r1) *reinterpret_cast<uint4*>(yb + (long long)(r + u * lanes) * p.y_ld) = one(pre[u]);
  r += kPre * lanes;
  for (; r + 7 * lanes < r1; r += 8 * lanes) {
    uint4 raw[8];
#pragma unroll
    for (int u = 0; u < 8; ++u) raw[u] = *reinterpret_cast<const uint4*>(xb + (long long)(r + u * lanes) * p.x_ld);
#pragma unroll
    for (int u = 0; u < 8; ++u) *reinterpret_cast<uint4*>(yb + (long long)(r + u * lanes) * p.y_ld) = one(raw[u]);
  }
  for (; r + 3 * lanes < r1; r += 4 * lanes) {
    uint4 raw[4];
#pragma unroll
    for (int u = 0; u < 4; ++u) raw[u] = *reinterpret_cast<const uint4*>(xb + (long long)(r + u * lanes) * p.x_ld);
#pragma unroll
    for (int u = 0; u < 4; ++u) *reinterpret_cast<uint4*>(yb + (long long)(r + u * lanes) * p.y_ld) = one(raw[u]);
  }
  for (; r < r1; r += lanes) {
    const uint4 raw = *reinterpret_cast<const uint4*>(xb + (long long)r * p.x_ld);
    *reinterpret_cast<uint4*>(yb + (long long)r * p.y_ld) = one(raw);
  }
}

#endif
}
```

### resshift_b200/models/unet.py

```python
from __future__ import annotations

import ctypes as C
from typing import Dict, Optional, Tuple

import torch
import torch.nn as nn

from .. import _lib
from ..arch import unet_param_spec, relative_position_index, shifted_window_mask
from ..config import UNetConfig
from ..weights import random_state_dict


class _Node(nn.Module):
    """Anonymous container; only there so that ``state_dict`` keys match the reference's."""


class UNetModelSwin(nn.Module):
    def __init__(self, image_size, in_channels, model_channels, out_channels, num_res_blocks,
                 attention_resolutions, dropout=0, channel_mult=(1, 2, 4, 8), conv_resample=True, dims=2,
                 use_fp16=False, num_heads=1, num_head_channels=-1, use_scale_shift_norm=False,
                 resblock_updown=False, swin_depth=2, swin_embed_dim=96, window_size=8, mlp_ratio=2.0,
                 patch_norm=False, cond_lq=True, cond_mask=False, lq_size=256):
        super().__init__()
        self.cfg = UNetConfig(
            image_size=image_size, in_channels=in_channels, model_channels=model_channels,
            out_channels=out_channels, num_res_blocks=num_res_blocks,
            attention_resolutions=tuple(attention_resolutions), dropout=dropout, channel_mult=tuple(channel_mult),
            conv_resample=conv_resample, dims=dims, use_fp16=use_fp16, num_heads=num_heads,
            num_head_channels=num_head_channels, use_scale_shift_norm=use_scale_shift_norm,
            resblock_updown=resblock_updown, swin_depth=swin_depth, swin_embed_dim=swin_embed_dim,
            window_size=window_size, mlp_ratio=mlp_ratio, patch_norm=patch_norm, cond_lq=cond_lq,
            cond_mask=cond_mask, lq_size=lq_size)
        self.image_size, self.in_channels, self.model_channels = image_size, in_channels, model_channels
        self.out_channels, self.cond_lq, self.cond_mask = out_channels, cond_lq, cond_mask
        self.dtype = torch.float32

        self._spec = unet_param_spec(self.cfg)
        init = random_state_dict(self.cfg, seed=0)
        for name, shape, role in self._spec:
            *path, leaf = name.split(".")
            node = self
            for part in path:
                if not hasattr(node, part):
                    node.add_module(part, _Node())
                node = getattr(node, part)
            value = init[name]
            if role.startswith("buf_"):
                node.register_buffer(leaf, value)
            else:
                if name.endswith("out_layers.3.weight") or name.endswith("out_layers.3.bias"):
                    value = torch.zeros_like(value)
                node.register_parameter(leaf, nn.Parameter(value))

        self._engine = None
        self._arena: Optional[torch.Tensor] = None
        self._packed_versions: Optional[Tuple] = None
        self._plans: Dict[Tuple[int, int, int], "_Plan"] = {}

    def _ensure_engine(self, device: torch.device):
        if device.type != "cuda":
            raise RuntimeError("resshift_b200.UNetModelSwin runs on CUDA only (no CPU fallback); call .cuda() first")
        if self._engine is None:
            h = C.c_void_p()
            cfgc = _lib.make_config(self.cfg)
            _lib.check(_lib.lib.rs_unet_create(C.byref(cfgc), C.byref(h)))
            self._engine = h
            n = _lib.lib.rs_unet_param_count(h)
            mine = sorted(name for name, _, _ in self._spec)
            theirs = []
            buf = C.create_string_buffer(256)
            shape = (C.c_int32 * 4)()
            nd, isb = C.c_int32(), C.c_int32()
            for i in range(n):
                _lib.check(_lib.lib.rs_unet_param_info(h, i, buf, 256, shape, C.byref(nd), C.byref(isb)))
                theirs.append(buf.value.decode())
            if sorted(theirs) != mine:
                raise _lib.RsError("parameter inventory of librs_b200 does not match resshift_b200.arch")
        if self._arena is None or self._arena.device != device:
            nbytes = _lib.lib.rs_unet_arena_bytes(self._engine)
            self._arena = torch.zeros(nbytes + 256, dtype=torch.uint8, device=device)
            base = self._arena.data_ptr()
            self._arena_ptr = (base + 255) // 256 * 256
            _lib.check(_lib.lib.rs_unet_set_arena(self._engine, self._arena_ptr))
            self._packed_versions = None
            self._plans.clear()
        return self._engine

    def pack_weights(self, force: bool = False):
        params = dict(self.named_parameters())
        self._ensure_engine(next(iter(params.values())).device)
        versions = tuple((p._version, p.data_ptr()) for p in params.values())
        if not force and versions == self._packed_versions:
            return
        stream = _lib.current_stream()
        for name, p in params.items():
            if p.device.type != "cuda":
                raise RuntimeError(f"parameter {name} is not on a CUDA device")
            src = p.detach()
            if src.dtype != torch.float32 or not src.is_contiguous():
                src = src.float().contiguous()
            _lib.check(_lib.lib.rs_unet_load_param(self._engine, name.encode(), src.data_ptr(), stream))
            del src
        torch.cuda.current_stream().synchronize()
        self._packed_versions = versions

    def plan(self, batch: int, height: int, width: int) -> "_Plan":
        device = next(self.parameters()).device
        self._ensure_engine(device)
        self.pack_weights()
        key = (batch, height, width)
        if key not in self._plans:
            self._plans[key] = _Plan(self, batch, height, width, device)
        return self._plans[key]

    def num_launches(self, batch, height, width) -> int:
        return _lib.lib.rs_plan_num_launches(self.plan(batch, height, width).handle)

    @torch.no_grad()
    def forward(self, x, timesteps, lq=None, mask=None):
        if lq is None:
            raise ValueError("UNetModelSwin is LQ-conditioned (cond_lq=True in every shipped config): pass lq=")
        if x.device.type != "cuda":
            raise RuntimeError("resshift_b200.UNetModelSwin.forward needs CUDA tensors (no CPU fallback)")
        n, _, h, w = x.shape
        plan = self.plan(n, h, w)
        xf = x.detach().float().contiguous()
        tf = timesteps.detach().to(device=x.device, dtype=torch.float32).contiguous()
        lqf = lq.detach().float().contiguous()
        mf = mask.detach().float().contiguous() if mask is not None else None
        exp_lq = (n, 3, h << self.cfg.fe_stages, w << self.cfg.fe_stages)
        if tuple(lqf.shape) != exp_lq:
            raise ValueError(f"lq must have shape {exp_lq}, got {tuple(lqf.shape)}")
        out = torch.empty(n, self.cfg.out_channels, h, w, dtype=torch.float32, device=x.device)
        _lib.check(_lib.lib.rs_plan_forward(plan.handle, xf.data_ptr(), tf.data_ptr(), lqf.data_ptr(),
                                            _lib.ptr(mf), out.data_ptr(), _lib.current_stream()))
        return out

    def probe(self, batch, height, width, block: str) -> torch.Tensor:
        plan = self.plan(batch, height, width)
        c, hh, ww = C.c_int32(), C.c_int32(), C.c_int32()
        _lib.check(_lib.lib.rs_plan_probe(plan.handle, block.encode(), None, C.byref(c), C.byref(hh), C.byref(ww), None))
        out = torch.empty(batch, c.value, hh.value, ww.value, dtype=torch.float32, device=plan.workspace.device)
        _lib.check(_lib.lib.rs_plan_probe(plan.handle, block.encode(), out.data_ptr(), C.byref(c), C.byref(hh),
                                          C.byref(ww), _lib.current_stream()))
        return out

    def convert_to_fp16(self):
        return self

    def convert_to_fp32(self):
        return self

    def __del__(self):
        try:
            self._plans.clear()
            if self._engine is not None:
                _lib.lib.rs_unet_destroy(self._engine)
        except Exception:
            pass


class _Plan:

    def __init__(self, model: UNetModelSwin, batch: int, height: int, width: int, device):
        self.model = model
        h = C.c_void_p()
        _lib.check(_lib.lib.rs_plan_create(model._engine, batch, height, width, C.byref(h)))
        self.handle = h
        nbytes = _lib.lib.rs_plan_workspace_bytes(h)
        self.workspace = torch.empty(nbytes + 256, dtype=torch.uint8, device=device)
        self.workspace_ptr = (self.workspace.data_ptr() + 255) // 256 * 256
        _lib.check(_lib.lib.rs_plan_bind(h, self.workspace_ptr))
        self.batch, self.height, self.width = batch, height, width
        self.samplers = {}

    def __del__(self):
        try:
            for s in self.samplers.values():
                _lib.lib.rs_sampler_destroy(s)
            _lib.lib.rs_plan_destroy(self.handle)
        except Exception:
            pass
```

Before: 280.3.

## Fold GroupNorm apply into cluster split-K conv epilogue when tile holds whole images

When a conv's output tile covers whole images and full groups, which holds for cluster split-K with two images per tile or two slots per image, the GroupNorm that follows it is computed inside the conv epilogue. Tile statistics are exchanged across the cluster via distributed shared memory, and the normalized, FiLM-modulated, SiLU output is written directly. If the raw conv output is dead it is never written. This removes a separate GroupNorm launch and a full read/write pass of the activation, at the cost of extra shared memory, a cluster sync and more epilogue work, and it applies only to eligible tile configurations.

```diff
diff --git a/include/resshift_b200.h b/include/resshift_b200.h
--- a/include/resshift_b200.h
+++ b/include/resshift_b200.h
@@ -62,6 +62,7 @@
 size_t rs_plan_workspace_bytes(const rs_plan* p);
 int rs_plan_bind(rs_plan* p, void* workspace_dev);
 int rs_plan_num_launches(const rs_plan* p);
+int rs_plan_num_gn_folded(const rs_plan* p);
 int rs_plan_forward(rs_plan* p, const float* x, const float* timesteps, const float* lq, const float* mask,
                     float* out, void* stream);
 int rs_plan_profile(rs_plan* p, const float* x, const float* timesteps, const float* lq, const float* mask,
diff --git a/resshift_b200/_lib.py b/resshift_b200/_lib.py
--- a/resshift_b200/_lib.py
+++ b/resshift_b200/_lib.py
@@ -50,6 +50,7 @@
     "rs_plan_workspace_bytes": (C.c_size_t, [_P]),
     "rs_plan_bind": (C.c_int, [_P, _P]),
     "rs_plan_num_launches": (C.c_int, [_P]),
+    "rs_plan_num_gn_folded": (C.c_int, [_P]),
     "rs_plan_forward": (C.c_int, [_P, _P, _P, _P, _P, _P, _P]),
     "rs_plan_profile": (C.c_int, [_P, _P, _P, _P, _P, C.POINTER(C.c_double), C.POINTER(C.c_double), C.POINTER(C.c_int32), _P]),
     "rs_plan_profile_ops": (C.c_int, [_P, _P, _P, _P, _P, C.POINTER(C.c_double), C.c_char_p, C.c_int, C.c_int, C.POINTER(C.c_int32), _P]),
diff --git a/resshift_b200/csrc/conv_gemm.cuh b/resshift_b200/csrc/conv_gemm.cuh
--- a/resshift_b200/csrc/conv_gemm.cuh
+++ b/resshift_b200/csrc/conv_gemm.cuh
@@ -51,6 +51,13 @@
   int epi_bc;
   GnSink sink[2];
   int gn_slots;
+  int gn_fold, gn_raw, gn_silu, gn_C;
+  float gn_eps;
+  const float* gn_gamma; const float* gn_beta;
+  const float* gn_film;
+  long long gn_film_sN;
+  __half* gn_out;
+  long long gn_sN, gn_sH, gn_sW;
   int persist;
   int num_units;
 };
@@ -421,6 +428,7 @@
         const int col0 = n_tile * p.BN;
         __half* s_out = reinterpret_cast<__half*>(smem + (size_t)kConvBM * pitch);
         float* s_col = reinterpret_cast<float*>(s_out + (size_t)kConvBM * cw);
+        float* s_slot = s_col + 4 * cw + 16;
         int tw, th, w0, h0, n0;
         tile_origin(0, tw, th, w0, h0, n0);
         const uint32_t dump0 = smem_u32(smem);
@@ -462,11 +470,12 @@
             __half2* oh = reinterpret_cast<__half2*>(&o);
 #pragma unroll
             for (int j = 0; j < 4; ++j) oh[j] = __floats2half2_rn(acc[2 * j], acc[2 * j + 1]);
-            *reinterpret_cast<uint4*>(p.out + n * p.out_sN + h * p.out_sH + w * p.out_sW + col) = o;
+            if (!p.gn_fold || p.gn_raw)
+              *reinterpret_cast<uint4*>(p.out + n * p.out_sN + h * p.out_sH + w * p.out_sW + col) = o;
           }
           *reinterpret_cast<uint4*>(s_out + (size_t)rr * cw + cu * 8) = o;
         }
-        if (p.sink[0].part != nullptr) {
+        if (p.sink[0].part != nullptr || p.gn_fold) {
           named_bar_sync(1, 32 * kConvEpiWarps);
           for (int t = etid; t < 2 * cw; t += 32 * kConvEpiWarps) {
             const int half = t / cw, c = t - half * cw;
@@ -483,7 +492,14 @@
           named_bar_sync(1, 32 * kConvEpiWarps);
           const int slot = th * p.tiles_w + tw;
           const int ncols = max(0, min(cw, p.Cout - (col0 + cbase)));
-          if (n0 < p.Nimg)
+          if (p.gn_fold)
+            for (int t = etid; t < p.bn * cw; t += 32 * kConvEpiWarps) {
+              const int j = t / cw, c = t - j * cw;
+              const int k = p.bn == 1 ? slot : j;
+              const float2 q = tile_pair(s_col, cw, c, p.bn, j);
+              s_slot[(k * cw + c) * 2] = q.x; s_slot[(k * cw + c) * 2 + 1] = q.y;
+            }
+          if (p.sink[0].part != nullptr && n0 < p.Nimg)
             write_tile_pairs(s_col, cw, ncols, col0 + cbase, p.bn, n0, p.Nimg, slot, p.gn_slots, p.sink[0], p.sink[1], etid, 32 * kConvEpiWarps);
           if (p.sink[0].gstat || p.sink[1].gstat) {
             int* s_flag = reinterpret_cast<int*>(s_col + 4 * cw);
@@ -492,6 +508,71 @@
             const int im[4] = {n0 < p.Nimg ? n0 : -1, n0 < p.Nimg ? n1 : -1, n0 < p.Nimg ? n0 : -1, n0 < p.Nimg ? n1 : -1};
             const unsigned int ad[4] = {(unsigned)ncols, (unsigned)ncols, (unsigned)ncols, (unsigned)ncols};
             gn_arrive<4>(sk, im, ad, p.gn_slots, 128.0f / (float)p.bn, etid, 32 * kConvEpiWarps, 1, s_flag);
+          }
+        }
+      }
+      if (p.gn_fold) {
+        const int S = p.splitk, cw = p.BN / S;
+        const int pitch = p.BN * 4 + 16;
+        const int cbase = split * cw;
+        const int col0 = n_tile * p.BN;
+        const int nthr = 32 * kConvEpiWarps;
+        const __half* s_out = reinterpret_cast<const __half*>(smem + (size_t)kConvBM * pitch);
+        float* s_slot = reinterpret_cast<float*>(smem + (size_t)kConvBM * pitch + (size_t)kConvBM * cw * 2) + 4 * cw + 16;
+        float* s_ch = s_slot + 4 * cw;
+        float* s_ab = s_ch + 4 * cw;
+        int tw, th, w0, h0, n0;
+        tile_origin(0, tw, th, w0, h0, n0);
+        const int HW = p.Hout * p.Wout;
+        if (p.bn == 1) {
+          cluster_sync_all();
+          if (warp < kConvEpiWarps) {
+            const int other = 1 - (th * p.tiles_w + tw);
+            const uint32_t src = mapa_u32(smem_u32(s_slot + (size_t)other * cw * 2), crank ^ 1u);
+            for (int c = threadIdx.x; c < cw / 2; c += nthr) {
+              const float4 v = ld_shared_cluster_f4(src + (uint32_t)(c * 16));
+              float* d = s_slot + ((size_t)other * cw + 2 * c) * 2;
+              d[0] = v.x; d[1] = v.y; d[2] = v.z; d[3] = v.w;
+            }
+          }
+        }
+        if (warp < kConvEpiWarps) {
+          const int etid = threadIdx.x;
+          const int nimg = p.bn;
+          for (int t = etid; t < nimg * cw; t += nthr) {
+            const int j = t / cw, c = t - j * cw;
+            const float2 mq = p.bn == 1 ? gn_channel_from_pairs(s_slot + (size_t)c * 2, 2, cw, (float)HW / 2.0f)
+                                        : gn_channel_from_pairs(s_slot + (size_t)(j * cw + c) * 2, 1, cw, (float)HW);
+            s_ch[(j * cw + c) * 2] = mq.x; s_ch[(j * cw + c) * 2 + 1] = mq.y;
+          }
+          named_bar_sync(1, nthr);
+          const int cpg = p.gn_C / 32;
+          for (int t = etid; t < nimg * cw; t += nthr) {
+            const int j = t / cw, c = t - j * cw;
+            const int ch = col0 + cbase + c;
+            const float2 mr = gn_group_from_channels(s_ch + (size_t)(j * cw + (c / cpg) * cpg) * 2, cpg, (float)HW, p.gn_eps);
+            const float* f = p.gn_film ? p.gn_film + (long long)min(n0 + j, p.Nimg - 1) * p.gn_film_sN : nullptr;
+            float a, b;
+            gn_fold_affine(mr.x, mr.y, __ldg(p.gn_gamma + ch), __ldg(p.gn_beta + ch), f ? f + ch : nullptr,
+                           f ? f + p.gn_C + ch : nullptr, a, b);
+            s_ab[(j * cw + c) * 2] = a; s_ab[(j * cw + c) * 2 + 1] = b;
+          }
+          named_bar_sync(1, nthr);
+          const int upr = cw >> 3;
+          for (int u = etid; u < kConvBM * upr; u += nthr) {
+            const int rr = u / upr, cu = u - rr * upr;
+            const int lw = rr % p.bw, lh = (rr / p.bw) % p.bh, ln = rr / (p.bw * p.bh);
+            const int w = w0 + lw, h = h0 + lh, n = n0 + ln;
+            const int col = col0 + cbase + cu * 8;
+            if (w >= p.Wout || h >= p.Hout || n >= p.Nimg || col >= p.Cout) continue;
+            float a[8], b[8];
+#pragma unroll
+            for (int k = 0; k < 8; ++k) {
+              a[k] = s_ab[(ln * cw + cu * 8 + k) * 2];
+              b[k] = s_ab[(ln * cw + cu * 8 + k) * 2 + 1];
+            }
+            const uint4 x = *reinterpret_cast<const uint4*>(s_out + (size_t)rr * cw + cu * 8);
+            *reinterpret_cast<uint4*>(p.gn_out + n * p.gn_sN + h * p.gn_sH + w * p.gn_sW + col) = gn_apply8(x, a, b, p.gn_silu);
           }
         }
       }
diff --git a/resshift_b200/csrc/engine.cu b/resshift_b200/csrc/engine.cu
--- a/resshift_b200/csrc/engine.cu
+++ b/resshift_b200/csrc/engine.cu
@@ -289,6 +289,7 @@
   float* out_f32 = nullptr;
   bool bound = false;
   int launches = 0;
+  int gn_folded = 0;
   int branches = 1;
   std::vector<cudaStream_t> side;
   std::vector<cudaEvent_t> ev;
@@ -369,6 +370,7 @@
   const bool fuse_swin_attn = env_int("RS_SWIN_FUSE", 1) != 0 && !env_is("RS_CONV_IMPL", "simt") && !env_is("RS_ATTN_IMPL", "simt");
   const int fuse_swin_min_pairs = env_int("RS_SWIN_FUSE_MIN_PAIRS", 96);
   const bool fuse_stats = env_int("RS_GN_FUSE", 1) && !env_is("RS_CONV_EPI", "direct") && !env_is("RS_CONV_IMPL", "simt");
+  const bool gn_epilogue = env_int("RS_GN_EPILOGUE", 1) != 0 && fuse_stats;
   Builder(rs_plan& p) : P(p), E(*p.e), cur(&p.ops) {}
   int list_id() const { return cur == &P.fe_ops ? 0 : 1; }
   std::vector<Op>& list(int id) { return id == 0 ? P.fe_ops : P.ops; }
@@ -400,7 +402,8 @@
     cur->push_back(op);
     if (out && !out_f32 && out->tens >= 0) note_writer(*out, cout);
   }
-  void gn(const View& in, const std::string& name, const View& out, int silu, int film_off, float eps = 1e-5f) {
+  void gn(const View& in, const std::string& name, const View& out, int silu, int film_off, float eps = 1e-5f, bool raw_dead = false) {
+    if (gn_epilogue && P.vq_which < 0 && fold_gn(in, name, out, silu, film_off, eps, raw_dead)) return;
     Op op; op.kind = OP_GN;
     op.gn.in = in; op.gn.out = out; op.gn.silu = silu; op.gn.film_off = film_off; op.gn.eps = eps;
     op.gn.film_n0 = cur_batch0;
@@ -422,6 +425,30 @@
     for (const Writer& w : prod)
       list(w.list)[w.op].stat_dst.push_back({list_id(), (int)cur->size() - 1, w.c0 - in.c0, w.n0 - in.n0});
   }
+  bool fold_gn(const View& in, const std::string& name, const View& out, int silu, int film_off, float eps, bool raw_dead) {
+    if (P.branches != 1 || cur->empty()) return false;
+    const std::vector<Writer> prod = covering_writers(in);
+    if (prod.size() != 1 || prod[0].list != list_id() || prod[0].op != (int)cur->size() - 1 || prod[0].win_slots) return false;
+    Op& c = cur->back();
+    ConvDesc& d = c.conv;
+    if (c.kind != OP_CONV || c.to_f32 || !d.has_out || !d.allow_split || c.split_tens >= 0 || d.gn_fold || d.Cout != in.C ||
+        !conv_gn_epilogue_ok(d.in.N, d.in.H, d.in.W, d.in.C, d.Cout, d.ksize, d.stride))
+      return false;
+    const int i = opi() - 1;
+    c.g_name = name;
+    c.gn.in = in; c.gn.out = out; c.gn.silu = silu; c.gn.film_off = film_off; c.gn.film_n0 = cur_batch0; c.gn.eps = eps;
+    d.gn_fold = true; d.gn_raw = !raw_dead; d.gn_out = out; d.gn_silu = silu; d.gn_eps = eps;
+    P.touch(out, i);
+    Tensor& raw = P.tensors[in.tens];
+    if (raw_dead && c.stat_dst.empty() && raw.first == i && raw.last == i) {
+      d.out = out;
+      raw.first = 1 << 30; raw.last = -1;
+    } else {
+      d.gn_raw = true;
+    }
+    ++P.gn_folded;
+    return true;
+  }
   void attn(const View& qkv, const View& out, const std::string& blk, int shift) {
     Op op; op.kind = OP_ATTN; op.a_in = qkv; op.a_out = out; op.a_shift = shift;
     op.w_name = blk + ".attn.relative_position_bias_table";
@@ -492,7 +519,7 @@
     View h1 = P.make_view(x.N, x.H, x.W, cout);
     conv(t1, p + ".in_layers.2", 3, 1, cout, &h1, nullptr, ACT_NONE);
     View t2 = P.make_view(x.N, x.H, x.W, cout);
-    gn(h1, p + ".out_layers.0", t2, 1, E.film_row_of.at(p));
+    gn(h1, p + ".out_layers.0", t2, 1, E.film_row_of.at(p), 1e-5f, true);
     if (x.C != cout) {
       conv(x, p + ".skip_connection", 1, 1, cout, &out, nullptr, ACT_NONE);
       conv(t2, p + ".out_layers.3", 3, 1, cout, &out, &out, ACT_NONE);
@@ -802,6 +829,11 @@
       d.partial = op.split_tens >= 0 ? reinterpret_cast<float*>(P.ws + P.tensors[op.split_tens].off) : nullptr;
       if (d.in.C < d.ipad && d.in.ld >= d.ipad && d.in.tens == P.xin.tens) d.in.C = d.ipad;
       if (d.in.C < d.ipad && P.fe_in.tens >= 0 && d.in.tens == P.fe_in.tens) d.in.C = d.ipad;
+      if (d.gn_fold) {
+        resolve(P, d.gn_out);
+        d.gn_gamma = E.at<float>(op.g_name + ".weight"); d.gn_beta = E.at<float>(op.g_name + ".bias");
+        RS_CHECK(d.gn_gamma && d.gn_beta, "missing GroupNorm parameters " + op.g_name);
+      }
       int rc = conv_finalize(d); if (rc) return rc;
       P.launches += (d.prm.splitk > 1 && !d.prm.splitk_cluster) ? 2 : 1;
     } else if (op.kind == OP_GN) {
@@ -929,7 +961,15 @@
     if (op_skipped(op)) { if (prof) { cudaEventRecord(prof->get(), st); prof->kind.push_back((int)op.kind); cudaEventRecord(prof->get(), st); } continue; }
     if (prof) { cudaEventRecord(prof->get(), st); prof->kind.push_back((int)op.kind); }
     switch (op.kind) {
-      case OP_CONV: rc = conv_launch(op.conv, st); break;
+      case OP_CONV:
+        if (op.conv.gn_fold && op.gn.film_off >= 0) {
+          ConvDesc d = op.conv;
+          d.prm.gn_film = film_base + op.gn.film_off + (long long)op.gn.film_n0 * film_sN; d.prm.gn_film_sN = film_sN;
+          rc = conv_launch(d, st);
+        } else {
+          rc = conv_launch(op.conv, st);
+        }
+        break;
       case OP_GN: {
         GnDesc g = op.gn;
         if (g.film_off >= 0) { g.film = film_base + g.film_off + (long long)g.film_n0 * film_sN; g.film_sN = film_sN; }
@@ -1088,6 +1128,7 @@
 void rs_plan_destroy(rs_plan* p) { delete p; }
 size_t rs_plan_workspace_bytes(const rs_plan* p) { return p ? p->workspace_bytes : 0; }
 int rs_plan_num_launches(const rs_plan* p) { return p ? p->launches : 0; }
+int rs_plan_num_gn_folded(const rs_plan* p) { return p ? p->gn_folded : 0; }
 
 int rs_plan_bind(rs_plan* p, void* workspace_dev) {
   RS_CHECK(p && workspace_dev && (reinterpret_cast<uintptr_t>(workspace_dev) & 255) == 0, "workspace must be 256-byte aligned");
@@ -1191,6 +1232,10 @@
       const ConvParams& c = op.conv.prm;
       snprintf(d, desc_stride, "conv%dx%d s%d %dx%d Cin=%d Cout=%d grid=%d BN=%d st=%d %s", op.conv.ksize, op.conv.ksize,
                op.conv.stride, c.Hout, c.Wout, op.conv.in.C, c.Cout, op.conv.grid, c.BN, c.stages, op.w_name.c_str());
+      if (op.conv.gn_fold) {
+        const size_t l = strlen(d);
+        snprintf(d + l, desc_stride - l, " +gn %s", op.g_name.c_str());
+      }
     } else if (op.kind == OP_GN) {
       snprintf(d, desc_stride, "gn %dx%d C=%d fused=%d %s", op.gn.in.H, op.gn.in.W, op.gn.in.C, (int)op.gn.fused, op.g_name.c_str());
     } else if (op.kind == OP_MLP) {
diff --git a/resshift_b200/csrc/gn_stats.cuh b/resshift_b200/csrc/gn_stats.cuh
--- a/resshift_b200/csrc/gn_stats.cuh
+++ b/resshift_b200/csrc/gn_stats.cuh
@@ -231,27 +231,32 @@
   }
 }
 
+__device__ __forceinline__ float2 tile_pair(const float* wstat, int BN, int cc, int bn, int j) {
+  const float m0 = wstat[((size_t)0 * BN + cc) * 2], q0 = wstat[((size_t)0 * BN + cc) * 2 + 1];
+  const float m1 = wstat[((size_t)1 * BN + cc) * 2], q1 = wstat[((size_t)1 * BN + cc) * 2 + 1];
+  if (bn == 1) {
+    float m, q;
+    chan_merge_equal(64.f, m0, q0, m1, q1, m, q);
+    return make_float2(m, q);
+  }
+  return j == 0 ? make_float2(m0, q0) : make_float2(m1, q1);
+}
+
 __device__ __forceinline__ void write_tile_pairs(const float* wstat, int BN, int ncols, int col0, int bn, int n0, int Nimg, int slot,
                                                  int slots, const GnSink& s0, const GnSink& s1, int tid, int nthreads) {
   for (int cc = tid; cc < ncols; cc += nthreads) {
-    const float m0 = wstat[((size_t)0 * BN + cc) * 2], q0 = wstat[((size_t)0 * BN + cc) * 2 + 1];
-    const float m1 = wstat[((size_t)1 * BN + cc) * 2], q1 = wstat[((size_t)1 * BN + cc) * 2 + 1];
+    const float2 p0 = tile_pair(wstat, BN, cc, bn, 0);
+    const float2 p1 = bn == 2 ? tile_pair(wstat, BN, cc, bn, 1) : p0;
 #pragma unroll
     for (int d = 0; d < 2; ++d) {
       const GnSink& s = d == 0 ? s0 : s1;
       if (!s.part) continue;
       const size_t ch = (size_t)s.coff + col0 + cc;
       float* dst = s.part + (((size_t)n0 * slots + slot) * s.cstride + ch) * 2;
-      if (bn == 1) {
-        float m, q;
-        chan_merge_equal(64.f, m0, q0, m1, q1, m, q);
-        dst[0] = m; dst[1] = q;
-      } else {
-        dst[0] = m0; dst[1] = q0;
-        if (n0 + 1 < Nimg) {
-          float* dst1 = s.part + (((size_t)(n0 + 1) * slots + slot) * s.cstride + ch) * 2;
-          dst1[0] = m1; dst1[1] = q1;
-        }
+      dst[0] = p0.x; dst[1] = p0.y;
+      if (bn == 2 && n0 + 1 < Nimg) {
+        float* dst1 = s.part + (((size_t)(n0 + 1) * slots + slot) * s.cstride + ch) * 2;
+        dst1[0] = p1.x; dst1[1] = p1.y;
       }
     }
   }
@@ -291,5 +296,26 @@
   return make_float2(pivot + dm, rsqrtf(m2 / (cnt * (float)cpg) + eps));
 }
 
+__device__ __forceinline__ void gn_fold_affine(float mean, float rstd, float gamma, float beta, const float* film_sc,
+                                               const float* film_sh, float& a, float& b) {
+  a = rstd * gamma;
+  b = beta - mean * a;
+  if (film_sc) { const float sc = 1.0f + *film_sc; a *= sc; b = b * sc + *film_sh; }
+}
+__device__ __forceinline__ uint4 gn_apply8(const uint4& raw, const float (&a)[8], const float (&b)[8], int silu) {
+  const __half2* h = reinterpret_cast<const __half2*>(&raw);
+  uint4 o;
+  __half2* oh = reinterpret_cast<__half2*>(&o);
+#pragma unroll
+  for (int j = 0; j < 4; ++j) {
+    float2 f = __half22float2(h[j]);
+    f.x = fmaf(f.x, a[2 * j], b[2 * j]);
+    f.y = fmaf(f.y, a[2 * j + 1], b[2 * j + 1]);
+    if (silu) { f.x = silu_f(f.x); f.y = silu_f(f.y); }
+    oh[j] = __floats2half2_rn(f.x, f.y);
+  }
+  return o;
+}
+
 #endif
 }
diff --git a/resshift_b200/csrc/launch.cuh b/resshift_b200/csrc/launch.cuh
--- a/resshift_b200/csrc/launch.cuh
+++ b/resshift_b200/csrc/launch.cuh
@@ -142,6 +142,10 @@
   SplitKReduceParams red;
   int red_grid_x = 0, red_grid_z = 1; size_t red_smem = 0;
   GnSink sink[2] = {};
+  bool gn_fold = false, gn_raw = true;
+  int gn_silu = 0; float gn_eps = 1e-5f;
+  const float* gn_gamma = nullptr; const float* gn_beta = nullptr;
+  View gn_out;
   ConvParams prm;
   ConvSimtSrc simt;
   int grid = 0; size_t smem = 0;
@@ -243,6 +247,21 @@
   return pick_tile_config(m_tiles, (Cout + 15) / 16 * 16, num_kb, env_int("RS_CONV_BN", 0), sp, false, sp && Cout % 8 == 0);
 }
 
+inline bool conv_gn_epilogue_fits(const TileConfig& tc, int bn, int slots, int Cout, size_t ring_bytes) {
+  if (!(tc.splitk > 1 && tc.cluster_split && tc.cg == 2 && tc.msub == 1 && !tc.persist)) return false;
+  if (!((bn == 2 && slots == 1) || (bn == 1 && slots == 2)) || Cout % 32 != 0) return false;
+  const int cw = tc.BN / tc.splitk;
+  const size_t need = (size_t)kConvBM * (tc.BN * 4 + 16) + (size_t)kConvBM * cw * 2 + ((size_t)8 * cw + 16) * sizeof(float);
+  return cw % (Cout / 32) == 0 && need <= ring_bytes;
+}
+inline bool conv_gn_epilogue_ok(int N, int Hin, int Win, int Cin, int Cout, int ksize, int stride) {
+  const TileConfig tc = conv_preview_config(N, Hin, Win, Cin, Cout, ksize, stride, true);
+  const int Hout = Hin / stride, Wout = Win / stride;
+  const int bw = pow2_floor_div(Wout, kConvBM), bh = pow2_floor_div(Hout, kConvBM / bw);
+  const size_t ring = (size_t)tc.stages * (kConvBM * kConvBK * 2 + (tc.BN / 2) * kConvBK * 2);
+  return tc.BN > 0 && conv_gn_epilogue_fits(tc, kConvBM / (bw * bh), (Wout / bw) * (Hout / bh), Cout, ring);
+}
+
 inline int conv_finalize(ConvDesc& d) {
   ConvParams& p = d.prm;
   std::memset(&p, 0, sizeof(p));
@@ -370,7 +389,17 @@
   if (p.splitk > 1 && p.splitk_cluster) {
     fill_sinks(p.sink);
     RS_CHECK(cg == 2 && d.Cout % 8 == 0 && (BN / p.splitk) % 8 == 0, "cluster split-K configuration");
-  } else if (p.splitk > 1) {
+  }
+  if (d.gn_fold) {
+    RS_CHECK(conv_gn_epilogue_fits(tc, p.bn, p.gn_slots, d.Cout, (size_t)stages * stage_bytes),
+             "GroupNorm epilogue: the tile configuration does not keep images and groups together");
+    RS_CHECK(d.gn_out.H == Hout && d.gn_out.W == Wout && d.gn_out.N == N && d.gn_out.C == d.Cout && d.gn_out.ld % 8 == 0 &&
+             (reinterpret_cast<uintptr_t>(d.gn_out.ptr) & 15) == 0 && d.gn_gamma && d.gn_beta, "GroupNorm epilogue arguments");
+    p.gn_fold = 1; p.gn_raw = d.gn_raw ? 1 : 0; p.gn_silu = d.gn_silu; p.gn_C = d.Cout; p.gn_eps = d.gn_eps;
+    p.gn_gamma = d.gn_gamma; p.gn_beta = d.gn_beta;
+    p.gn_out = d.gn_out.ptr; p.gn_sN = d.gn_out.sN(); p.gn_sH = d.gn_out.sH(); p.gn_sW = d.gn_out.sW();
+  }
+  if (p.splitk > 1 && !p.splitk_cluster) {
     SplitKReduceParams& r = d.red;
     std::memset(&r, 0, sizeof(r));
     r.partial = d.partial; r.S = p.splitk; r.N = N; r.HW = Hout * Wout; r.C = d.Cout;
diff --git a/resshift_b200/csrc/norm_act.cuh b/resshift_b200/csrc/norm_act.cuh
--- a/resshift_b200/csrc/norm_act.cuh
+++ b/resshift_b200/csrc/norm_act.cuh
@@ -211,10 +211,7 @@
     const float* f = p.film ? p.film + n * p.film_sN + c0 : nullptr;
     for (int cc = threadIdx.x; cc < Cs; cc += blockDim.x) {
       const int g = cc / cpg;
-      float a = s_rstd[g] * s_g[cc];
-      float b = s_be[cc] - s_mean[g] * a;
-      if (f) { const float sc = 1.0f + f[cc]; a *= sc; b = b * sc + f[p.C + cc]; }
-      s_a[cc] = a; s_b[cc] = b;
+      gn_fold_affine(s_mean[g], s_rstd[g], s_g[cc], s_be[cc], f ? f + cc : nullptr, f ? f + p.C + cc : nullptr, s_a[cc], s_b[cc]);
     }
   }
   __syncthreads();
@@ -222,20 +219,7 @@
   float a[8], b[8];
 #pragma unroll
   for (int j = 0; j < 8; ++j) { a[j] = s_a[c + j]; b[j] = s_b[c + j]; }
-  auto one = [&](const uint4& raw) {
-    const __half2* h = reinterpret_cast<const __half2*>(&raw);
-    uint4 o;
-    __half2* oh = reinterpret_cast<__half2*>(&o);
-#pragma unroll
-    for (int j = 0; j < 4; ++j) {
-      float2 f = __half22float2(h[j]);
-      f.x = fmaf(f.x, a[2 * j], b[2 * j]);
-      f.y = fmaf(f.y, a[2 * j + 1], b[2 * j + 1]);
-      if (p.silu) { f.x = silu_f(f.x); f.y = silu_f(f.y); }
-      oh[j] = __floats2half2_rn(f.x, f.y);
-    }
-    return o;
-  };
+  auto one = [&](const uint4& raw) { return gn_apply8(raw, a, b, p.silu); };
 #pragma unroll
   for (int u = 0; u < kPre; ++u)
     if (r + u * lanes < r1) *reinterpret_cast<uint4*>(yb + (long long)(r + u * lanes) * p.y_ld) = one(pre[u]);
diff --git a/resshift_b200/models/unet.py b/resshift_b200/models/unet.py
--- a/resshift_b200/models/unet.py
+++ b/resshift_b200/models/unet.py
@@ -117,6 +117,9 @@
     def num_launches(self, batch, height, width) -> int:
         return _lib.lib.rs_plan_num_launches(self.plan(batch, height, width).handle)
 
+    def num_gn_folded(self, batch, height, width) -> int:
+        return _lib.lib.rs_plan_num_gn_folded(self.plan(batch, height, width).handle)
+
     @torch.no_grad()
     def forward(self, x, timesteps, lq=None, mask=None):
         if lq is None:
```

New measurement: 281.7 (median of 6 runs). No clear change (+0.5%).
